# sp-uhh/guided-vae-nmf

Hardware: AMD Instinct MI355X
Metric: STFT-frames/sec through VAE-NMF reconstruct loop; SI-SDR parity vs ref (higher is better)
Workload: dtype bf16; 1 GPU; 64-utterance batch per GPU, M1 reconstruct, 512-pt STFT (F=257, 501 frames/utt), NMF rank 8, 100 EM iters, MH 60/30 per E-step + 105/75 Wiener chain; utterances_total=64, utterances_rank0=64, parallelism=utterance-shard x1 (np.array_split, no collective in the loop)

## Files before the change

### guided-vae-nmf_amd/csrc/chain.hip

```cpp
#include "common.h"

#ifdef VN_STAMP
__device__ long long g_wc_stamp[32];
#define WC_STAMP_DECL long long _t_prev = (long long)__builtin_amdgcn_s_memtime(); long long _st_acc[8] = {0, 0, 0, 0, 0, 0, 0, 0}; int _st_cnt[8] = {0, 0, 0, 0, 0, 0, 0, 0};
#define WC_STAMP(slot) do { long long _t = (long long)__builtin_amdgcn_s_memtime(); _st_acc[slot] += _t - _t_prev; _st_cnt[slot] += 1; _t_prev = _t; } while (0)
#define WC_STAMP_FLUSH do { if (blockIdx.x == 0 && threadIdx.x == 0) { for (int _i = 0; _i < 8; ++_i) { g_wc_stamp[_i] += _st_acc[_i]; g_wc_stamp[16 + _i] += _st_cnt[_i]; } } } while (0)
#else
#define WC_STAMP_DECL
#define WC_STAMP(slot)
#define WC_STAMP_FLUSH
#endif
namespace {

constexpr int WT_FRAMES = 16;
constexpr unsigned WC_OOB = 0xF0000000u;
constexpr int WC_PF = 1;
constexpr int WC_PFL = 2;
constexpr int WC_ST_AUX = 0;

struct WcArgs {
  const __bf16 *w1f, *w2f, *w3f;
  const float *b1, *b2, *b3;
  int NT3;
  int Tm;
  int F, Fs;
  const float *X2, *W, *Ht, *g, *B1, *Vb;
  float *Z, *Zs, *acc_out;
  void* VsS;
  unsigned VsS_bytes;
  int32_t* src;
  int Rs;
  const int32_t *wt_utt, *wt_n0, *wt_cnt;
  int n_wtiles;
  const int32_t* frame_off;
  const uint64_t* utt_seed;
  const float *eps, *u;
  int Kp, NT, n_utts, Rcap, nsamples, burnin, rng_mode, update_Z;
  int n_hi_lds;
  int b1_lds;
  uint32_t call;
  float sd;
  float sd_hi;
  int one_hidden;
};

template <bool SPLIT>
struct WcLds {
  static constexpr int PARTS = SPLIT ? 2 : 1;
  static constexpr int W1 = 0;
  static constexpr int W2 = W1 + NT_H * PARTS * 1024;
  static constexpr int B1 = W2 + NT_H * NK_H * PARTS * 1024;
  static constexpr int B2 = B1 + HID * 4;
  static constexpr int B3 = B2 + HID * 4;
  static constexpr int W3 = B3 + 640 * 4;
  static constexpr int fixed_bytes = W3;
};

typedef __attribute__((ext_vector_type(4))) unsigned u32x4;
typedef __attribute__((ext_vector_type(2))) unsigned u32x2;

typedef __attribute__((ext_vector_type(2))) __bf16 bf16x2;
__device__ __forceinline__ unsigned pk2(float a, float b) { return __builtin_bit_cast(unsigned, bf16x2{(__bf16)a, (__bf16)b}); }
// ... 62 lines not shown
  x2 = xv;
  vb = v;
}

struct WcFrame {
  int utt, nrow;
  bool fvalid;
  bool keeps;
};
__device__ __forceinline__ WcFrame wc_frame(const WcArgs& a, int wt, int c, bool writer) {
  WcFrame fr;
  const int n0 = a.wt_n0[wt], cnt = a.wt_cnt[wt];
  fr.utt = a.wt_utt[wt];
  fr.fvalid = c < cnt;
  fr.keeps = fr.fvalid && writer;
  fr.nrow = n0 + (fr.fvalid ? c : cnt - 1);
  return fr;
}
__device__ __forceinline__ void wc_load_z(const WcRes& R, const WcFrame& fr, int q, float (&z)[8]) {
  const unsigned zo = ((unsigned)fr.nrow * LAT + 4u * (unsigned)q) * 4u;
  const f32x4 lo = __builtin_bit_cast(f32x4, __builtin_amdgcn_raw_buffer_load_b128(R.z_rs, zo, 0, 0));
  const f32x4 hi = __builtin_bit_cast(f32x4, __builtin_amdgcn_raw_buffer_load_b128(R.z_rs, zo + 64u, 0, 0));
#pragma unroll
  for (int t = 0; t < 4; ++t) { z[t] = lo[t]; z[4 + t] = hi[t]; }
}
__device__ __forceinline__ void wc_store_z(const WcArgs& a, const WcRes& R, const WcFrame& fr, unsigned rp_off, const float (&z)[8]) {
  if (a.update_Z) {
    const unsigned zo = fr.keeps ? rp_off : WC_OOB;
    __builtin_amdgcn_raw_buffer_store_b128(__builtin_bit_cast(u32x4, f32x4{z[0], z[1], z[2], z[3]}), R.z_rs, zo, 0, 0);
    __builtin_amdgcn_raw_buffer_store_b128(__builtin_bit_cast(u32x4, f32x4{z[4], z[5], z[6], z[7]}), R.z_rs, zo + 64u, 0, 0);
  }
}

template <int MAXT, bool EXACT, bool SPLIT, bool STORE, int NWAVES, bool LOL, bool HIALL, bool M2, int GT>
__global__ __launch_bounds__(NWAVES * 64, NWAVES / 4) void wchain_kernel(const WcArgs a) {
  extern __shared__ __attribute__((aligned(16))) char smem[];
  using L = WcLds<SPLIT>;
  constexpr int PARTS = L::PARTS;
  using store_t = typename std::conditional<SPLIT, float, __bf16>::type;
  const int NT3 = EXACT ? MAXT : a.NT3;
  const int n_hi = HIALL ? NT3 - GT : a.n_hi_lds;

  {
    const int nthr = NWAVES * 64;
    auto stage = [&](char* dst, const __bf16* srcp, int nblk) {
      for (int e = threadIdx.x; e < nblk * PARTS * 64; e += nthr) {
        const int chunk = e & 63, pb = e >> 6, b = pb / PARTS, part = pb - b * PARTS;
        *reinterpret_cast<f32x4*>(dst + (size_t)e * 16) =
            *reinterpret_cast<const f32x4*>(reinterpret_cast<const char*>(srcp) + ((size_t)(b * 2 + part) * 64 + chunk) * 16);
      }
    };
    stage(smem + L::W1, a.w1f, NT_H);
    stage(smem + L::W2, a.w2f, NT_H * NK_H);
    for (int e = threadIdx.x; e < n_hi * NK_H * 64; e += nthr) {
      const int chunk = e & 63, b = (e >> 6) + GT * NK_H;
      *reinterpret_cast<f32x4*>(smem + L::W3 + (size_t)e * 16) =
          *reinterpret_cast<const f32x4*>(reinterpret_cast<const char*>(a.w3f) + ((size_t)(b * 2) * 64 + chunk) * 16);
    }
    if (SPLIT && LOL)
      for (int e = threadIdx.x; e < NT3 * NK_H * 64; e += nthr) {
        const int chunk = e & 63, b = e >> 6;
        *reinterpret_cast<f32x4*>(smem + L::W3 + (size_t)n_hi * NK_H * 1024 + (size_t)e * 16) =
            *reinterpret_cast<const f32x4*>(reinterpret_cast<const char*>(a.w3f) + ((size_t)(b * 2 + 1) * 64 + chunk) * 16);
      }
    float* b1s = reinterpret_cast<float*>(smem + L::B1);
    float* b2s = reinterpret_cast<float*>(smem + L::B2);
    float* b3s = reinterpret_cast<float*>(smem + L::B3);
    for (int i = threadIdx.x; i < HID; i += nthr) { b1s[i] = a.b1[i]; b2s[i] = a.b2[i]; }
    for (int i = threadIdx.x; i < 16 * NT3; i += nthr) b3s[i] = a.b3[i];
  }
  __syncthreads();

  const int lane = threadIdx.x & 63, q = lane >> 4, c = lane & 15;
  const unsigned l16 = (unsigned)lane * 16u;
  const float* b1l = reinterpret_cast<const float*>(smem + L::B1);
  const float* b2l = reinterpret_cast<const float*>(smem + L::B2);
  const float* b3l = reinterpret_cast<const float*>(smem + L::B3);
  const char* w3lo_lds = smem + L::W3 + (size_t)n_hi * NK_H * 1024;
  const char* w3g = reinterpret_cast<const char*>(a.w3f);
  const int Tm = EXACT ? ((MAXT - 1) & ~1) : a.Tm;
  auto tile_on = [&](int t) { return EXACT || t < NT3; };
  auto tile_on3 = [&](int n, int t) { return n != MAXT || EXACT || t < NT3; };

  const WcRes R = wc_resources<STORE, M2>(a);

  const int wave = __builtin_amdgcn_readfirstlane(threadIdx.x >> 6);
  for (int wt = wave * (int)gridDim.x + (int)blockIdx.x; wt < a.n_wtiles; wt += (int)gridDim.x * NWAVES) {
    const WcFrame fr = wc_frame(a, wt, c, true);
    const int nrow = fr.nrow;
    const float gn = a.g[nrow];
    f32x4 x2[MAXT], vb[MAXT];
    {
      const unsigned rowF = (unsigned)nrow * (unsigned)a.Fs;
      const unsigned uF = (unsigned)fr.utt * (unsigned)a.Fs;
      int qo = q;
      asm volatile("" : "+v"(qo));
      auto bin0o = [&](int t) { return (!SPLIT && t < Tm) ? 32 * (t >> 1) + 8 * qo + 4 * (t & 1) : 16 * t + 4 * qo; };
#pragma unroll
      for (int t = 0; t < MAXT; ++t) {
        x2[t] = f32x4{0, 0, 0, 0};
        vb[t] = f32x4{1, 1, 1, 1};
        if (tile_on(t)) {
          const int f0 = bin0o(t);
          wc_tile_consts(a, R, rowF, uF, nrow, f0, x2[t], vb[t]);
        }
      }
    }
    constexpr bool B1L = M2 && NWAVES == 8;
    f32x4 b1r[(M2 && !B1L) ? NT_H : 1];
    char* b1stash = smem + a.b1_lds + wave * (NT_H * 512) + lane * 8;
    if (M2) {
#pragma unroll
      for (int t = 0; t < NT_H; ++t) {
        const f32x4 v = __builtin_bit_cast(f32x4, __builtin_amdgcn_raw_buffer_load_b128(R.b1in_rs, ((unsigned)nrow * HID + 4u * (unsigned)q) * 4u + 64u * (unsigned)t, 0, 0));
        if (B1L) *reinterpret_cast<u32x2*>(b1stash + t * 512) = u32x2{pk2(v[0], v[1]), pk2(v[2], v[3])};
        else b1r[(M2 && !B1L) ? t : 0] = v;
      }
    }
    float z[8];
    wc_load_z(R, fr, q, z);
    const unsigned fbase = STORE ? (fr.fvalid ? (unsigned)nrow * (unsigned)(a.Rs * a.Fs) * (unsigned)sizeof(store_t) : WC_OOB) : 0u;
    const unsigned zs_off = fr.fvalid ? ((unsigned)nrow * (unsigned)a.Rcap * LAT + 4u * q) * 4u : WC_OOB;
    const unsigned fr_off = (fr.fvalid && q == 0) ? (unsigned)nrow * 4u : WC_OOB;
    const unsigned rp_off = ((unsigned)nrow * LAT + 4u * q) * 4u;
    int cur_src = a.nsamples;
    Xs128 st0, st1;
    if (a.rng_mode == VAENMF_RNG_DEVICE) {
      const uint32_t floc = (uint32_t)(nrow - a.frame_off[fr.utt]);
      int qs = q;
      asm volatile("" : "+v"(qs));
      st0 = xs_seed(a.utt_seed[fr.utt], floc, (uint32_t)qs, a.call);
      st1 = xs_seed(a.utt_seed[fr.utt], floc, (uint32_t)(4 + qs), a.call);
    }

    WC_STAMP_DECL
    auto energy = [&](const float (&zz)[8], int slot, auto dost) -> double {
      constexpr bool DOST = STORE && decltype(dost)::value;
      const unsigned voff = DOST ? fbase + (unsigned)slot * (unsigned)a.Fs * (unsigned)sizeof(store_t) : 0u;
      u32x4 bh[NK_H], bl[NK_H], ch[NK_H], cl[NK_H];
      auto put = [&](u32x4 (&dh)[NK_H], u32x4 (&dl)[NK_H], int t, const f32x4 h) {
        dh[t >> 1][2 * (t & 1)] = pk2(h[0], h[1]);
        dh[t >> 1][2 * (t & 1) + 1] = pk2(h[2], h[3]);
        if (SPLIT) {
          dl[t >> 1][2 * (t & 1)] = pk2(h[0] - bf_lo(dh[t >> 1][2 * (t & 1)]), h[1] - bf_hi(dh[t >> 1][2 * (t & 1)]));
          dl[t >> 1][2 * (t & 1) + 1] = pk2(h[2] - bf_lo(dh[t >> 1][2 * (t & 1) + 1]), h[3] - bf_hi(dh[t >> 1][2 * (t & 1) + 1]));
        }
      };
      auto run_layer = [&](auto nks_c, auto ntiles_c, auto pfl_c, auto frag, auto frag_lo, auto frag_lo_pro, auto bias, auto bop, auto epi) {
        constexpr int NKS = decltype(nks_c)::value, N = decltype(ntiles_c)::value;
        constexpr int PF = WC_PF, NB = PF + 1;
        constexpr int PFL = SPLIT ? decltype(pfl_c)::value : 0, NBL = PFL + 1;
        bf16x8 wh[NB][NKS], wl[NBL][NKS];
        f32x4 acc[2], bq[NB];
#pragma unroll
        for (int p = 0; p < PFL; ++p)
          if (p < N) {
#pragma unroll
            for (int s = 0; s < NKS; ++s) frag_lo_pro(p, s, wl[p % NBL][s]);
          }
#pragma unroll
        for (int p = 0; p < PF; ++p)
          if (p < N) {
#pragma unroll
            for (int s = 0; s < NKS; ++s) frag(p, s, wh[p % NB][s]);
            bq[p % NB] = bias(p);
          }
#pragma unroll
        for (int t = 0; t <= N; ++t) {
          if (SPLIT && t + PFL < N && tile_on3(N, t + PFL)) {
#pragma unroll
            for (int s = 0; s < NKS; ++s) frag_lo(t + PFL, s, wl[(t + PFL) % NBL][s]);
// ... 78 lines not shown
      WC_STAMP(2);
      double e = 0.0;
      f32x2 pl2 = {0.f, 0.f}, px2 = {0.f, 0.f};
      unsigned pk_even0 = 0, pk_even1 = 0;
      run_layer(std::integral_constant<int, NK_H>{}, std::integral_constant<int, MAXT>{}, std::integral_constant<int, (SPLIT && !LOL) ? WC_PFL : WC_PF>{},
                [&](int t, int s, bf16x8& hi) {
                  if (GT > 0 && t < GT) hi = gfr[t < GT ? t : 0][s];
                  else if (HIALL || t - GT < n_hi) hi = *reinterpret_cast<const bf16x8*>(smem + L::W3 + ((t - GT) * NK_H + s) * 1024 + l16);
                  else hi = *reinterpret_cast<const bf16x8*>(w3g + (size_t)((t * NK_H + s) * 2) * 1024 + l16);
                },
                [&](int t, int s, bf16x8& lo) {
                  if (LOL) lo = *reinterpret_cast<const bf16x8*>(w3lo_lds + (t * NK_H + s) * 1024 + l16);
                  else lo = *reinterpret_cast<const bf16x8*>(w3g + (size_t)((t * NK_H + s) * 2 + 1) * 1024 + l16);
                },
                [&](int t, int s, bf16x8& lo) {
                  if (LOL) lo = *reinterpret_cast<const bf16x8*>(w3lo_lds + (t * NK_H + s) * 1024 + l16);
                  else if (t < NHOIST) lo = lo_pre[t < NHOIST ? t : 0][s];
                  else lo = *reinterpret_cast<const bf16x8*>(w3g + (size_t)((t * NK_H + s) * 2 + 1) * 1024 + l16);
                },
                [&](int t) { return *reinterpret_cast<const f32x4*>(b3l + 16 * t + 4 * q); },
                [&](int s, bf16x8& hi, bf16x8& lo) { hi = __builtin_bit_cast(bf16x8, bh[s]); lo = SPLIT ? __builtin_bit_cast(bf16x8, bl[s]) : hi; },
                [&](int t, const f32x4 acc) {
                  f32x4 ev;
#pragma unroll
                  for (int j = 0; j < 4; ++j) ev[j] = fast_exp(acc[j]);
                  {
                    const f32x2 g2 = {gn, gn};
                    const f32x2 v0 = g2 * ev.lo + vb[t].lo, v1 = g2 * ev.hi + vb[t].hi;
                    const f32x2 pp = v0 * v1;
                    pl2 += f32x2{fast_log2(pp[0]), fast_log2(pp[1])};
                    const f32x2 rc = {fast_rcp(pp[0]), fast_rcp(pp[1])};
                    px2 = (x2[t].lo * v1 + x2[t].hi * v0) * rc + px2;
                  }
                  if (DOST) {
                    if (SPLIT) {
                      __builtin_amdgcn_raw_buffer_store_b128(__builtin_bit_cast(u32x4, ev), R.vrs, voff + 16u * q + 64u * t, 0, WC_ST_AUX);
                    } else {
                      const unsigned p0 = pk2(ev[0], ev[1]), p1 = pk2(ev[2], ev[3]);
                      if (t < Tm) {
                        if ((t & 1) == 0) { pk_even0 = p0; pk_even1 = p1; }
                        else __builtin_amdgcn_raw_buffer_store_b128(u32x4{pk_even0, pk_even1, p0, p1}, R.vrs, voff + 16u * q + 64u * (t >> 1), 0, WC_ST_AUX);
                      } else {
                        __builtin_amdgcn_raw_buffer_store_b64(u32x2{p0, p1}, R.vrs, voff + 8u * q + 32u * t, 0, WC_ST_AUX);
                      }
                    }
                  }
                  if ((t & 1) == 1) {
                    e += (double)((pl2[0] + pl2[1]) * LN2_F + (px2[0] + px2[1]));
                    pl2 = px2 = f32x2{0.f, 0.f};
                  }
                });
      e += (double)((pl2[0] + pl2[1]) * LN2_F + (px2[0] + px2[1]));
      WC_STAMP(3);
      return sum_rows4_d(e);
    };

    double Ecur = 0.0;
    __builtin_amdgcn_s_waitcnt(0x0F70);
    const int n_it = vn_chain_passes<STORE>(a.nsamples, a.burnin);
    for (int it = -1; it < n_it; ++it) {
      asm volatile("" ::: "memory");
      const VnChainPass ps = vn_chain_pass<STORE>(it, a.nsamples, a.burnin);
      const bool re = ps.re, step = ps.step;
      const int m = ps.m, slot = ps.slot;
      float zp[8];
      float lu = 0.f;
      if (step) {
// ... 22 lines not shown
      }
      WC_STAMP(0);
      double Ep;
      if (STORE && slot >= 0) Ep = energy(zp, slot, std::true_type{});
      else Ep = energy(zp, slot, std::false_type{});
      WC_STAMP(5);
      if (re) continue;
      float pr = 0.f;
#pragma unroll
      for (int j = 0; j < 8; ++j) pr += z[j] * z[j] - zp[j] * zp[j];
      pr = sum_rows4(pr);
      lu = sum_rows4(lu);
      WC_STAMP(6);
      const float accp = (float)(Ecur - Ep) + 0.5f * pr;
      const bool ok = m < 0 || lu < accp;
      if (a.acc_out && m >= 0) __builtin_amdgcn_raw_buffer_store_b32(__builtin_bit_cast(unsigned, accp), R.acc_rs, fr_off + (unsigned)m * (unsigned)a.NT * 4u, 0, 0);
#pragma unroll
      for (int j = 0; j < 8; ++j) z[j] = ok ? zp[j] : z[j];
      Ecur = ok ? Ep : Ecur;
      WC_STAMP(7);
      if (m >= a.burnin) {
        const unsigned r = (unsigned)(m - a.burnin);
        if (STORE) {
          cur_src = ok ? (int)r : cur_src;
          __builtin_amdgcn_raw_buffer_store_b32((unsigned)cur_src, R.src_rs, fr_off + r * (unsigned)a.NT * 4u, 0, 0);
        }
        const unsigned zo = zs_off + r * (LAT * 4u);
        __builtin_amdgcn_raw_buffer_store_b128(__builtin_bit_cast(u32x4, f32x4{z[0], z[1], z[2], z[3]}), R.zs_rs, zo, 0, 0);
        __builtin_amdgcn_raw_buffer_store_b128(__builtin_bit_cast(u32x4, f32x4{z[4], z[5], z[6], z[7]}), R.zs_rs, zo + 64u, 0, 0);
      }
      WC_STAMP(4);
    }
    WC_STAMP_FLUSH;
    wc_store_z(a, R, fr, rp_off, z);
  }
}


template <int MAXT, bool STORE, bool M2>
__global__ __launch_bounds__(256, 1) void wchain4_kernel(const WcArgs a) {
  extern __shared__ __attribute__((aligned(16))) char smem[];
  constexpr int NP = (MAXT - 1) / 2;
  constexpr int PPW = NP / 4, NOWN = 2 * PPW + 1;
  constexpr bool B1BF = MAXT == 17;
  static_assert(NP % 4 == 0, "pairs must split over four wavefronts");
  u32x4* xh1 = reinterpret_cast<u32x4*>(smem);
  u32x4* xh2 = xh1 + 4 * 64;
  float* exl = reinterpret_cast<float*>(xh2 + 4 * 64);

  const int lane = threadIdx.x & 63, q = lane >> 4, c = lane & 15;
  const unsigned l16 = (unsigned)lane * 16u;
  const int wave = __builtin_amdgcn_readfirstlane(threadIdx.x >> 6);
  auto tile_of = [&](int i) { return i < 2 * PPW ? 2 * (wave + 4 * (i >> 1)) + (i & 1) : MAXT - 1; };
  auto own = [&](int i) { return i < 2 * PPW || wave == 0; };

  bf16x8 w1r[2], w2r[2][NK_H], w3r[NOWN][NK_H];
  f32x4 bias1[2], bias2[2], bias3[NOWN];
  {
    const char* w1g = reinterpret_cast<const char*>(a.w1f);
    const char* w2g = reinterpret_cast<const char*>(a.w2f);
    const char* w3g = reinterpret_cast<const char*>(a.w3f);
#pragma unroll
    for (int i = 0; i < 2; ++i) {
      const int t = 2 * wave + i;
      w1r[i] = *reinterpret_cast<const bf16x8*>(w1g + (size_t)(t * 2) * 1024 + l16);
#pragma unroll
      for (int s = 0; s < NK_H; ++s) w2r[i][s] = *reinterpret_cast<const bf16x8*>(w2g + (size_t)((t * NK_H + s) * 2) * 1024 + l16);
      bias1[i] = *reinterpret_cast<const f32x4*>(a.b1 + 16 * t + 4 * q);
      bias2[i] = *reinterpret_cast<const f32x4*>(a.b2 + 16 * t + 4 * q);
    }
#pragma unroll
    for (int i = 0; i < NOWN; ++i) {
      const int t = tile_of(i);
#pragma unroll
      for (int s = 0; s < NK_H; ++s) w3r[i][s] = *reinterpret_cast<const bf16x8*>(w3g + (size_t)((t * NK_H + s) * 2) * 1024 + l16);
      bias3[i] = *reinterpret_cast<const f32x4*>(a.b3 + 16 * t + 4 * q);
    }
  }

  const WcRes R = wc_resources<STORE, M2>(a);

  for (int wt = blockIdx.x; wt < a.n_wtiles; wt += (int)gridDim.x) {
    const WcFrame fr = wc_frame(a, wt, c, wave == 0);
    const int nrow = fr.nrow;
    const float gn = a.g[nrow];
    f32x4 x2[NOWN], vb[NOWN];
    {
      const unsigned rowF = (unsigned)nrow * (unsigned)a.Fs, uF = (unsigned)fr.utt * (unsigned)a.Fs;
#pragma unroll
      for (int i = 0; i < NOWN; ++i) {
        x2[i] = f32x4{0, 0, 0, 0};
        vb[i] = f32x4{1, 1, 1, 1};
        if (own(i)) {
          const int t = tile_of(i);
          const int f0 = t < MAXT - 1 ? 32 * (t >> 1) + 8 * q + 4 * (t & 1) : 16 * t + 4 * q;
          wc_tile_consts(a, R, rowF, uF, nrow, f0, x2[i], vb[i]);
        }
      }
    }
    f32x4 b1r[2];
    b1r[0] = bias1[0]; b1r[1] = bias1[1];
    if (M2) {
#pragma unroll
      for (int i = 0; i < 2; ++i) {
        const f32x4 v = __builtin_bit_cast(f32x4, __builtin_amdgcn_raw_buffer_load_b128(R.b1in_rs, ((unsigned)nrow * HID + 4u * (unsigned)q) * 4u + 64u * (unsigned)(2 * wave + i), 0, 0));
        if (B1BF) {
          const unsigned w0 = pk2(v[0], v[1]), w1 = pk2(v[2], v[3]);
          b1r[i] = f32x4{bf_lo(w0), bf_hi(w0), bf_lo(w1), bf_hi(w1)};
        } else b1r[i] = v;
      }
    }
    float z[8];
    wc_load_z(R, fr, q, z);
    const unsigned fbase = STORE ? (fr.fvalid ? (unsigned)nrow * (unsigned)(a.Rs * a.Fs) * 2u : WC_OOB) : 0u;
    const unsigned zs_off = fr.keeps ? ((unsigned)nrow * (unsigned)a.Rcap * LAT + 4u * q) * 4u : WC_OOB;
    const unsigned fr_off = (fr.keeps && q == 0) ? (unsigned)nrow * 4u : WC_OOB;
    const unsigned rp_off = ((unsigned)nrow * LAT + 4u * q) * 4u;
    int cur_src = a.nsamples;
    Xs128 st0, st1;
    if (a.rng_mode == VAENMF_RNG_DEVICE) {
      const uint32_t floc = (uint32_t)(nrow - a.frame_off[fr.utt]);
      st0 = xs_seed(a.utt_seed[fr.utt], floc, (uint32_t)q, a.call);
      st1 = xs_seed(a.utt_seed[fr.utt], floc, (uint32_t)(4 + q), a.call);
    }

    auto energy = [&](const float (&zz)[8], int slot, auto dost) -> double {
      constexpr bool DOST = STORE && decltype(dost)::value;
      const unsigned voff = DOST ? fbase + (unsigned)slot * (unsigned)a.Fs * 2u : 0u;
      u32x4 bh[NK_H], ch[NK_H];
      u32x4 mine;
      auto put2 = [&](int i, const f32x4 h) { mine[2 * i] = pk2(h[0], h[1]); mine[2 * i + 1] = pk2(h[2], h[3]); };
      auto exchange = [&](u32x4* xh, u32x4 (&dst)[NK_H]) {
        xh[wave * 64 + lane] = mine;
        __syncthreads();
#pragma unroll
        for (int s2 = 0; s2 < NK_H; ++s2) dst[s2] = xh[s2 * 64 + lane];
      };
      {
        const bf16x8 zin = __builtin_bit_cast(bf16x8, u32x4{pk2(zz[0], zz[1]), pk2(zz[2], zz[3]), pk2(zz[4], zz[5]), pk2(zz[6], zz[7])});
        f32x4 ac[2];
#pragma unroll
        for (int i = 0; i < 2; ++i) ac[i] = __builtin_amdgcn_mfma_f32_16x16x32_bf16(w1r[i], zin, b1r[i], 0, 0, 0);
#pragma unroll
        for (int i = 0; i < 2; ++i) put2(i, tanh4(ac[i]));
      }
      exchange(xh1, ch);
      if (a.one_hidden) {
#pragma unroll
        for (int s = 0; s < NK_H; ++s) bh[s] = ch[s];
      } else {
        f32x4 ac[2];
#pragma unroll
        for (int i = 0; i < 2; ++i) {
          ac[i] = bias2[i];
#pragma unroll
          for (int s = 0; s < NK_H; ++s) ac[i] = __builtin_amdgcn_mfma_f32_16x16x32_bf16(w2r[i][s], __builtin_bit_cast(bf16x8, ch[s]), ac[i], 0, 0, 0);
        }
#pragma unroll
        for (int i = 0; i < 2; ++i) put2(i, tanh4(ac[i]));
        exchange(xh2, bh);
      }
      f32x2 pl2 = {0.f, 0.f}, px2 = {0.f, 0.f};
      float pv[PPW + 1];
#pragma unroll
      for (int j = 0; j <= PPW; ++j) pv[j] = 0.f;
      unsigned pk_even0 = 0, pk_even1 = 0;
      auto mm3 = [&](int i) {
        f32x4 ac = bias3[i];
#pragma unroll
        for (int s = 0; s < NK_H; ++s) ac = __builtin_amdgcn_mfma_f32_16x16x32_bf16(w3r[i][s], __builtin_bit_cast(bf16x8, bh[s]), ac, 0, 0, 0);
        return ac;
      };
      auto epi = [&](int i, const f32x4 acc) {
        f32x4 ev;
#pragma unroll
        for (int j = 0; j < 4; ++j) ev[j] = fast_exp(acc[j]);
        {
          const f32x2 g2 = {gn, gn};
          const f32x2 v0 = g2 * ev.lo + vb[i].lo, v1 = g2 * ev.hi + vb[i].hi;
          const f32x2 pp = v0 * v1;
          pl2 += f32x2{fast_log2(pp[0]), fast_log2(pp[1])};
          const f32x2 rc = {fast_rcp(pp[0]), fast_rcp(pp[1])};
          px2 = (x2[i].lo * v1 + x2[i].hi * v0) * rc + px2;
        }
        if (DOST) {
          const unsigned p0 = pk2(ev[0], ev[1]), p1 = pk2(ev[2], ev[3]);
          const unsigned t = (unsigned)tile_of(i);
          if (i < 2 * PPW) {
            if ((i & 1) == 0) { pk_even0 = p0; pk_even1 = p1; }
            else __builtin_amdgcn_raw_buffer_store_b128(u32x4{pk_even0, pk_even1, p0, p1}, R.vrs, voff + 16u * q + 64u * (t >> 1), 0, WC_ST_AUX);
          } else {
            __builtin_amdgcn_raw_buffer_store_b64(u32x2{p0, p1}, R.vrs, voff + 8u * q + 32u * t, 0, WC_ST_AUX);
          }
        }
        if ((i & 1) == 1 || i == 2 * PPW) {
          pv[i >> 1] = (pl2[0] + pl2[1]) * LN2_F + (px2[0] + px2[1]);
          pl2 = px2 = f32x2{0.f, 0.f};
        }
      };
      {
        f32x4 acn = mm3(0);
#pragma unroll
        for (int i = 0; i < NOWN; ++i) {
          const f32x4 acc = acn;
          if (i + 1 < NOWN && own(i + 1)) acn = mm3(i + 1);
          if (own(i)) epi(i, acc);
        }
      }
      float* ex = exl + lane;
#pragma unroll
      for (int j = 0; j < PPW; ++j) ex[(wave + 4 * j) * 64] = pv[j];
      if (wave == 0) ex[NP * 64] = pv[PPW];
      __syncthreads();
      double e = 0.0;
#pragma unroll
      for (int p = 0; p <= NP; ++p) e += (double)ex[p * 64];
      return sum_rows4_d(e);
    };

    double Ecur = 0.0;
    __builtin_amdgcn_s_waitcnt(0x0F70);
    const int n_it = vn_chain_passes<STORE>(a.nsamples, a.burnin);
    for (int it = -1; it < n_it; ++it) {
// ... 22 lines not shown
          for (int t = 0; t < 8; ++t) asm volatile("" : "+v"(zp[t]));
          asm volatile("" : "+v"(lu));
        }
      } else {
#pragma unroll
        for (int t = 0; t < 8; ++t) zp[t] = z[t];
      }
      double Ep;
      if (STORE && slot >= 0) Ep = energy(zp, slot, std::true_type{});
      else Ep = energy(zp, slot, std::false_type{});
      if (re) continue;
      float pr = 0.f;
#pragma unroll
      for (int j = 0; j < 8; ++j) pr += z[j] * z[j] - zp[j] * zp[j];
      pr = sum_rows4(pr);
      lu = sum_rows4(lu);
      const float accp = (float)(Ecur - Ep) + 0.5f * pr;
      const bool ok = m < 0 || lu < accp;
      if (a.acc_out && m >= 0) __builtin_amdgcn_raw_buffer_store_b32(__builtin_bit_cast(unsigned, accp), R.acc_rs, fr_off + (unsigned)m * (unsigned)a.NT * 4u, 0, 0);
#pragma unroll
      for (int j = 0; j < 8; ++j) z[j] = ok ? zp[j] : z[j];
      Ecur = ok ? Ep : Ecur;
      if (m >= a.burnin) {
        const unsigned r = (unsigned)(m - a.burnin);
        if (STORE) {
          cur_src = ok ? (int)r : cur_src;
          __builtin_amdgcn_raw_buffer_store_b32((unsigned)cur_src, R.src_rs, fr_off + r * (unsigned)a.NT * 4u, 0, 0);
        }
        const unsigned zo = zs_off + r * (LAT * 4u);
        __builtin_amdgcn_raw_buffer_store_b128(__builtin_bit_cast(u32x4, f32x4{z[0], z[1], z[2], z[3]}), R.zs_rs, zo, 0, 0);
        __builtin_amdgcn_raw_buffer_store_b128(__builtin_bit_cast(u32x4, f32x4{z[4], z[5], z[6], z[7]}), R.zs_rs, zo + 64u, 0, 0);
      }
    }
    wc_store_z(a, R, fr, rp_off, z);
  }
}

}

namespace {

template <typename Go>
int wc_by_m2_store(const WcArgs& a, Go&& go) {
  if (a.B1) return a.VsS ? go(std::true_type{}, std::true_type{}) : go(std::true_type{}, std::false_type{});
  return a.VsS ? go(std::false_type{}, std::true_type{}) : go(std::false_type{}, std::false_type{});
}
template <int MAXT, bool EXACT, bool SPLIT, int NW1, bool LOL, int GT = 0>
int wc_launch_s(const WcArgs& a, int nwt, int n_sms, size_t lds, hipStream_t st) {
  int grid = nwt;
  if (grid > n_sms) grid = n_sms;
  const int cap = vn_switches().grid_cap;
  if (cap > 0 && cap < grid) grid = cap;
  return wc_by_m2_store(a, [&](auto m2, auto store) -> int {
    auto* fn = wchain_kernel<MAXT, EXACT, SPLIT, decltype(store)::value, NW1, LOL, true, decltype(m2)::value, GT>;
    if (int e = vn_ensure_dyn_lds((const void*)fn, VN_LDS_LIMIT)) return e;
    hipLaunchKernelGGL(fn, dim3(grid), dim3(NW1 * 64), lds, st, a);
    return 0;
  });
}
template <int MAXT>
int wc_launch4(const WcArgs& a, hipStream_t st) {
  const size_t lds4 = 2 * 4 * 64 * 16 + 20 * 64 * 4;
  return wc_by_m2_store(a, [&](auto m2, auto store) -> int {
    hipLaunchKernelGGL((wchain4_kernel<MAXT, decltype(store)::value, decltype(m2)::value>), dim3(a.n_wtiles), dim3(256), lds4, st, a);
    return 0;
  });
}

}

bool vn_wchain_supported(const vaenmf_plan* p) {
  if (p->NT3c > 17 && !(p->NT3c == 33 && p->cfg.precision == VAENMF_PREC_BF16)) return false;
  return !vn_switches().team_chain;
}

extern "C" int vaenmf_wchain_addressable(int64_t NT, int32_t Rcap, int32_t steps, int32_t Fs, int32_t Kp, int32_t n_utt, int32_t replay) {
  const uint64_t lim = 0xE0000000ull;
  const uint64_t nt = (uint64_t)(NT > 0 ? NT : 0), S = (uint64_t)(steps > 0 ? steps : 0);
  if (nt * (uint64_t)Rcap * LAT * 4 >= lim) return 0;
  if (nt * (uint64_t)Fs * 4 >= lim) return 0;
  if (nt * (uint64_t)HID * 4 >= lim) return 0;
  if ((uint64_t)n_utt * (uint64_t)Fs * (uint64_t)Kp * 4 >= lim) return 0;
  if (nt * (uint64_t)Kp * 4 >= lim) return 0;
  if (nt * S * 4 >= lim) return 0;
  if (replay && nt * S * LAT * 4 >= lim) return 0;
  return 1;
}
bool vn_wchain_fits(const vaenmf_plan* p, const VnChainCall& cc) {
  return vaenmf_wchain_addressable(p->NT, cc.Rcap, cc.nsamples + cc.burnin, p->Fs, p->Kp, p->n_utt, cc.eps != nullptr) != 0;
}

int vn_launch_wchain(vaenmf_plan* p, const VnChainCall& cc, hipStream_t st) {
  VN_REQUIRE(vn_wchain_fits(p, cc), "wave chain: a buffer of this batch (%d frames) passes the kernel's 32-bit byte offsets", p->NT);
  const bool split = p->cfg.precision == VAENMF_PREC_BF16X3;
  WcArgs a = {};
  a.w1f = p->w1f; a.w2f = p->w2f; a.w3f = p->w3c; a.b1 = p->b1; a.b2 = p->b2; a.b3 = p->b3c;
  a.NT3 = p->NT3c; a.Tm = split ? 0 : ((p->NT3c - 1) & ~1); a.F = p->cfg.F; a.Fs = p->Fs;
  a.X2 = cc.X2; a.W = cc.W; a.Ht = cc.Ht; a.g = cc.g; a.B1 = cc.B1; a.Vb = p->Vb_ext;
  a.Z = cc.Z; a.Zs = cc.Zs; a.acc_out = cc.acc_out;
  a.VsS = cc.VsS; a.VsS_bytes = (unsigned)cc.VsS_bytes; a.src = cc.src; a.Rs = cc.Rs;
  a.wt_utt = p->d_wt_utt; a.wt_n0 = p->d_wt_n0; a.wt_cnt = p->d_wt_cnt; a.n_wtiles = p->n_wtiles;
  a.frame_off = p->d_frame_off; a.utt_seed = p->d_utt_seed; a.eps = cc.eps; a.u = cc.u;
  a.Kp = p->Kp; a.NT = p->NT; a.n_utts = p->n_utt; a.Rcap = cc.Rcap; a.nsamples = cc.nsamples; a.burnin = cc.burnin;
  a.rng_mode = cc.rng_mode; a.update_Z = cc.update_Z; a.call = cc.call; a.sd = cc.sd; a.sd_hi = cc.sd_hi; a.one_hidden = cc.one_hidden;
  a.n_hi_lds = p->NT3c;
  const size_t fixed = split ? WcLds<true>::fixed_bytes : WcLds<false>::fixed_bytes;
  constexpr int GT33 = 4;
  const size_t w3hi = (size_t)(p->NT3c == 33 ? p->NT3c - GT33 : p->NT3c) * NK_H * 1024;
  const bool lol = split && p->NT3c <= 5;
  constexpr int NW_BF16 = 8, NW_X3 = 4;
  const int nwaves = (split || p->NT3c == 33) ? 4 : NW_BF16;
  a.b1_lds = (int)(fixed + w3hi * (lol ? 2 : 1));
  const size_t lds = (size_t)a.b1_lds + ((cc.B1 && nwaves == 8) ? (size_t)nwaves * NT_H * 512 : 0);
  VN_REQUIRE(lds <= (size_t)VN_LDS_LIMIT, "wave chain: %zu bytes of LDS needed", lds);
  if (!split && (p->NT3c == 17 || p->NT3c == 33) && p->n_wtiles <= p->n_sms && vn_switches().wchain4) {
    const int rc4 = p->NT3c == 17 ? wc_launch4<17>(a, st) : wc_launch4<33>(a, st);
    if (rc4) return rc4;
    VN_CHECK_HIP(hipGetLastError());
    p->last_chain_kernel = 2;
    return 0;
  }
  int rc;
  if (p->NT3c == 33)     rc = wc_launch_s<33, true, false, 4, false, GT33>(a, p->n_wtiles, p->n_sms, lds, st);
  else if (p->NT3c == 17) rc = split ? wc_launch_s<17, true, true, NW_X3, false>(a, p->n_wtiles, p->n_sms, lds, st) : wc_launch_s<17, true, false, NW_BF16, false>(a, p->n_wtiles, p->n_sms, lds, st);
  else if (p->NT3c == 5) rc = split ? wc_launch_s<5, true, true, NW_X3, true>(a, p->n_wtiles, p->n_sms, lds, st)   : wc_launch_s<5, true, false, NW_BF16, false>(a, p->n_wtiles, p->n_sms, lds, st);
  else if (p->NT3c < 5)  rc = split ? wc_launch_s<5, false, true, NW_X3, true>(a, p->n_wtiles, p->n_sms, lds, st)  : wc_launch_s<5, false, false, NW_BF16, false>(a, p->n_wtiles, p->n_sms, lds, st);
  else                   rc = split ? wc_launch_s<17, false, true, NW_X3, false>(a, p->n_wtiles, p->n_sms, lds, st) : wc_launch_s<17, false, false, NW_BF16, false>(a, p->n_wtiles, p->n_sms, lds, st);
  if (rc) return rc;
  VN_CHECK_HIP(hipGetLastError());
  p->last_chain_kernel = 1;
  return 0;
}

#ifdef VN_STAMP
extern "C" int vaenmf_debug_stamps_wc(long long* out32, int reset) {
  long long h[32];
  if (hipMemcpyFromSymbol(h, HIP_SYMBOL(g_wc_stamp), sizeof(h)) != hipSuccess) return -2;
  for (int i = 0; i < 32; ++i) out32[i] = h[i];
  if (reset) { long long z[32] = {0}; (void)hipMemcpyToSymbol(HIP_SYMBOL(g_wc_stamp), z, sizeof(z)); }
  return 0;
}
#endif
```

### guided-vae-nmf_amd/csrc/common.h

```cpp
#pragma once
#include <hip/hip_runtime.h>
#include <stdint.h>
#include <string>
#include <type_traits>
#include <vector>
#include "../../include/vaenmf.h"

typedef __attribute__((ext_vector_type(8))) __bf16 bf16x8;
typedef __attribute__((ext_vector_type(4))) __bf16 bf16x4;
typedef __attribute__((ext_vector_type(4))) float f32x4;

void vaenmf_set_error(const char* fmt, ...);
#define VN_CHECK_HIP(expr)                                                         \
  do {                                                                             \
    hipError_t _e = (expr);                                                        \
    if (_e != hipSuccess) {                                                        \
      vaenmf_set_error("%s failed: %s (%s:%d)", #expr, hipGetErrorString(_e), __FILE__, __LINE__); \
      return -2;                                                                   \
    }                                                                              \
  } while (0)
#define VN_REQUIRE(cond, ...)                \
  do {                                       \
    if (!(cond)) {                           \
      vaenmf_set_error(__VA_ARGS__);         \
      return -1;                             \
    }                                        \
  } while (0)

constexpr int VN_COST_CHUNK = 25;
constexpr int MAX_TILE_FRAMES = 64;
constexpr int LAT = 32;
constexpr int HID = 128;
constexpr int NK_H = HID / 32;
constexpr int NT_H = HID / 16;
constexpr int VN_LDS_LIMIT = 160 * 1024;

struct VnEmGraphs {
  using Key = std::vector<uint64_t>;
  struct Graph {
    Key key; hipGraphExec_t exec; uint64_t used;
    int chain_kernel, w_fused;
  };
  hipStream_t cap_stream = nullptr;
  std::vector<Graph> cache;
  std::vector<Key> seen;
  uint64_t tick = 0;
  bool off = false;
  int last = 0;
  Graph* find(const Key& key);
  bool first_seen(const Key& key);
  Graph* insert(const Key& key, hipGraphExec_t exec, int chain_kernel, int w_fused);
  void release();
};

struct vaenmf_plan {
  vaenmf_config cfg;
  int Fs, Kp, NT3;
  int Fm;
  float* w3n;
  int geom;
  int nwaves;
  int tile_frames;
  __bf16 *w1f, *w2f, *w3f;
  float *b1, *b2, *b3;
  float* w1y;
  int Dy;
  int Lz;
  bool wide = false;
  int Lp = LAT;
  bool one_hidden;
  bool have_weights;
  const float* Vb_ext;
  int n_utt, NT, n_tiles;
  int32_t *d_frame_off;
  int32_t *d_tile_utt, *d_tile_n0, *d_tile_cnt;
  int32_t *d_frame_utt;
  int32_t *d_frame_loc;
  __bf16* w3c;
  float* b3c;
  int NT3c;
  int32_t *d_wt_utt, *d_wt_n0, *d_wt_cnt;
  int n_wtiles;
  int32_t *d_t64_n0 = nullptr, *d_t64_cnt = nullptr, *d_t64_first = nullptr, *d_t64_g0 = nullptr;
  int n_t64 = 0;
  float* wpart64 = nullptr;
  size_t wpart16_groups = 0;
  float* wpart16 = nullptr;
  int last_chain_kernel = 0;
  int last_w_fused = 0;
  int Rcap_store;
  int last_m_step_path;
  uint64_t* d_utt_seed;
  std::vector<int32_t> h_frame_off;
  float *A1, *P;
  float* normW;
  float* wpart;
  double* cost_frames;
  bool store_on;
  void* VsS;
  int32_t* src;
  size_t VsS_cap, src_cap;
  int store_R, store_Rs;
  int n_sms;
  bool prof_on;
  std::vector<hipEvent_t> prof_ev;
  std::vector<int> prof_kind;
  size_t prof_used;
  VnEmGraphs graphs;
  static constexpr int SEED_RING = 8;
  uint64_t* h_seed_ring = nullptr;
  hipEvent_t seed_ev[SEED_RING] = {};
  bool seed_ev_used[SEED_RING] = {};
  int seed_pos = 0;
};

struct VnChainCall {
  const float *X2, *W, *Ht, *g, *B1;
  float *Z, *Zs, *acc_out;
  const float *eps, *u;
  void* VsS; size_t VsS_bytes; int32_t* src; int Rs;
  int Rcap, nsamples, burnin, rng_mode, update_Z;
  uint32_t call;
  float sd;
  float sd_hi;
  int one_hidden;
};

struct VnSwitches {
  bool wchain4;
  bool team_chain;
  bool wfused;
  bool wgroup;
  int wfused_grid;
  int grid_cap;
  bool keep_zs;
};

VnSwitches vn_switches();
int vn_ensure_dyn_lds(const void* fn, int bytes);
extern long long g_vn_dev_allocs;
bool vn_wchain_supported(const vaenmf_plan* p);
bool vn_wchain_fits(const vaenmf_plan* p, const VnChainCall& cc);
int vn_launch_wchain(vaenmf_plan* p, const VnChainCall& cc, hipStream_t st);
int vn_launch_tchain(vaenmf_plan* p, const VnChainCall& cc, hipStream_t st);
int vn_launch_widechain(vaenmf_plan* p, const VnChainCall& cc, hipStream_t st);
int vn_launch_wide_rng_fill(vaenmf_plan* p, uint32_t call, int S, float* eps_out, float* u_out, hipStream_t st);
int vn_launch_w_update(const vaenmf_plan* p, float* W, const float* Ht, hipStream_t st);
int vn_launch_w_update_tiles(const vaenmf_plan* p, float* W, hipStream_t st, bool groups);
int vn_launch_cost_reduce(const vaenmf_plan* p, const double* cost_frames, size_t stride, int n_it, int R, double* cost, int niter,
                          int it0, hipStream_t st);

inline int check_bound(const vaenmf_plan* p) {
  VN_REQUIRE(p != nullptr, "null plan");
  VN_REQUIRE(p->have_weights, "decoder weights not set (vaenmf_set_decoder_weights)");
  VN_REQUIRE(p->NT > 0, "no batch bound (vaenmf_bind_batch)");
  return 0;
}

enum { VN_K_CHAIN = 0, VN_K_WSTATS = 1, VN_K_WUPDATE = 2, VN_K_HG = 3, VN_K_WF = 4, VN_K_NKINDS = 5 };
struct ProfScope {
  vaenmf_plan* p; hipStream_t st; size_t idx; bool on;
  ProfScope(vaenmf_plan* p_, int kind, hipStream_t st_) : p(p_), st(st_), idx(0), on(false) {
    if (p && p->prof_on && p->prof_used + 2 <= p->prof_ev.size()) {
      on = true; idx = p->prof_used; p->prof_used += 2; p->prof_kind[idx / 2] = kind;
      (void)hipEventRecord(p->prof_ev[idx], st);
    }
  }
  ~ProfScope() { if (on) (void)hipEventRecord(p->prof_ev[idx + 1], st); }
};

#if defined(__HIPCC__)
__device__ __forceinline__ float fast_tanh(float xs) {
  float e = __builtin_amdgcn_exp2f(xs);
  return 1.0f - 2.0f * __builtin_amdgcn_rcpf(e + 1.0f);
}
// ... 137 lines not shown
```

### guided-vae-nmf_amd/csrc/driver.hip

```cpp
#include "common.h"
#include <cstring>

extern "C" int vaenmf_mh_chain(vaenmf_plan* p, const float* X2, const float* W, const float* Ht, const float* g,
                               float* Z, int32_t update_Z, const float* B1, float* Zs, int32_t Rcap, int32_t nsamples,
                               int32_t burnin, float var_rw, const vaenmf_rng* rng, float* acc_out, void* stream) {
  if (int e = check_bound(p)) return e;
  VN_REQUIRE(rng != nullptr, "rng is null");
  VN_REQUIRE(nsamples >= 1 && burnin >= 0 && nsamples <= Rcap, "bad sample counts (nsamples=%d burnin=%d Rcap=%d)", nsamples, burnin, Rcap);
  VN_REQUIRE(rng->mode == VAENMF_RNG_DEVICE || (rng->eps && rng->u), "replay mode needs eps and u buffers");
  hipStream_t st = (hipStream_t)stream;
  const bool split = p->cfg.precision == VAENMF_PREC_BF16X3;
  VnChainCall cc = {};
  cc.X2 = X2; cc.W = W; cc.Ht = Ht; cc.g = g; cc.B1 = B1; cc.Z = Z; cc.Zs = Zs; cc.acc_out = acc_out;
  cc.eps = rng->eps; cc.u = rng->u;
  cc.Rcap = Rcap; cc.nsamples = nsamples; cc.burnin = burnin; cc.rng_mode = rng->mode; cc.update_Z = update_Z;
  cc.call = rng->call; cc.sd = sqrtf(var_rw); cc.sd_hi = p->Lz > 16 ? cc.sd : 0.f; cc.one_hidden = p->one_hidden ? 1 : 0;
  p->store_R = p->store_Rs = 0;
  if (p->store_on) {
    const int Rs = nsamples + 1;
    const size_t esz = split ? sizeof(float) : sizeof(__bf16);
    const size_t need_v = (size_t)(p->NT + 1) * Rs * p->Fs * esz, need_s = (size_t)p->NT * Rs;
    VN_REQUIRE(need_v < 0xE0000000ull, "sample store: %d frames x %d slots x %d bins exceeds the 32-bit byte offsets of "
               "the chain kernel; bind a smaller batch or switch the store off", p->NT, Rs, p->Fs);
    VN_REQUIRE(need_v <= p->VsS_cap && need_s <= p->src_cap, "sample store too small for %d frames x %d samples: call "
               "vaenmf_sample_store(plan, max_samples) after vaenmf_bind_batch (no allocation happens in vaenmf_mh_chain)", p->NT, nsamples);
    cc.VsS = p->VsS; cc.VsS_bytes = need_v; cc.src = p->src; cc.Rs = Rs;
  }
  const bool use_wchain = !p->wide && vn_wchain_supported(p) && vn_wchain_fits(p, cc);
  VN_REQUIRE(p->wide || use_wchain || Zs != nullptr, "vaenmf_mh_chain: Zs may be NULL only where the wave-private chain kernels run (vaenmf_wchain_addressable)");
  {
    ProfScope ps(p, VN_K_CHAIN, st);
    if (int e = p->wide ? vn_launch_widechain(p, cc, st) : use_wchain ? vn_launch_wchain(p, cc, st) : vn_launch_tchain(p, cc, st)) return e;
  }
  if (p->store_on) { p->store_R = nsamples; p->store_Rs = nsamples + 1; }
  return 0;
}

extern "C" int vaenmf_sample_store(vaenmf_plan* p, int32_t max_samples) {
  VN_REQUIRE(p != nullptr, "null plan");
  VN_REQUIRE(max_samples >= 0, "max_samples = %d", max_samples);
  p->store_R = p->store_Rs = 0;
  p->store_on = max_samples > 0;
  if (!p->store_on) return 0;
  const size_t esz = p->cfg.precision == VAENMF_PREC_BF16X3 ? sizeof(float) : sizeof(__bf16);
  const size_t frames = (size_t)(p->NT > 0 ? p->NT : p->cfg.max_frames) + 1, Rs = (size_t)max_samples + 1;
  size_t need_v = frames * Rs * p->Fs * esz, need_s = frames * Rs;
  if (need_v >= 0xE0000000ull) need_v = 0xE0000000ull - 16;
  if (need_v > p->VsS_cap) {
    if (p->VsS) VN_CHECK_HIP(hipFree(p->VsS));
    p->VsS = nullptr; p->VsS_cap = 0;
    VN_CHECK_HIP(hipMalloc(&p->VsS, need_v));
    ++g_vn_dev_allocs;
    p->VsS_cap = need_v;
  }
  if (need_s > p->src_cap) {
    if (p->src) VN_CHECK_HIP(hipFree(p->src));
    p->src = nullptr; p->src_cap = 0;
    VN_CHECK_HIP(hipMalloc(&p->src, need_s * sizeof(int32_t)));
    ++g_vn_dev_allocs;
    p->src_cap = need_s;
  }
  p->Rcap_store = max_samples;
  return 0;
}

namespace {
template <typename ST>
__global__ void store_gather_kernel(const ST* __restrict__ VsS, const int32_t* __restrict__ src, int NT, int R, int Rs, int Fs,
                                    float* __restrict__ out) {
  const int n = blockIdx.x / R, r = blockIdx.x - n * R;
  const ST* row = VsS + ((size_t)n * Rs + src[(size_t)r * NT + n]) * Fs;
  for (int f = threadIdx.x; f < Fs; f += blockDim.x) out[((size_t)n * R + r) * Fs + f] = (float)row[f];
}
}

extern "C" int vaenmf_sample_store_gather(vaenmf_plan* p, float* Vs_out, void* stream) {
  VN_REQUIRE(p != nullptr && p->store_R > 0, "the sample store is empty (vaenmf_sample_store(plan, 1), then vaenmf_mh_chain)");
  VN_REQUIRE(Vs_out != nullptr, "null output");
  if (p->cfg.precision == VAENMF_PREC_BF16X3)
    hipLaunchKernelGGL(store_gather_kernel<float>, dim3((unsigned)(p->NT * p->store_R)), dim3(64), 0, (hipStream_t)stream,
                       reinterpret_cast<const float*>(p->VsS), p->src, p->NT, p->store_R, p->store_Rs, p->Fs, Vs_out);
  else
    hipLaunchKernelGGL(store_gather_kernel<__bf16>, dim3((unsigned)(p->NT * p->store_R)), dim3(64), 0, (hipStream_t)stream,
                       reinterpret_cast<const __bf16*>(p->VsS), p->src, p->NT, p->store_R, p->store_Rs, p->Fs, Vs_out);
  VN_CHECK_HIP(hipGetLastError());
  return 0;
}

extern "C" int vaenmf_set_noise_psd(vaenmf_plan* p, const float* Vb) {
  VN_REQUIRE(p != nullptr, "null plan");
  p->Vb_ext = Vb;
  return 0;
}

namespace {
constexpr size_t MAX_GRAPHS = 4, MAX_SEEN = 8;

struct EmCall {
  const float* X2; float *W, *Ht, *g, *Z; const float* B1; float* Zs;
  int32_t Rcap, niter, nsE, biE, nsWF, biWF; float var_rw;
  const float* X; float *S_hat, *N_hat; double* cost;
};

VnEmGraphs::Key em_graph_key(const vaenmf_plan* p, const EmCall& c, bool stored, const VnSwitches& sw) {
  auto u64 = [](const void* q) { return (uint64_t)(uintptr_t)q; };
  uint32_t vbits;
  memcpy(&vbits, &c.var_rw, 4);
  uint64_t fo_hash = 1469598103934665603ull;
  for (int32_t v : p->h_frame_off) { fo_hash ^= (uint64_t)(uint32_t)v; fo_hash *= 1099511628211ull; }
  return {fo_hash,
      u64(c.X2), u64(c.W), u64(c.Ht), u64(c.g), u64(c.Z), u64(c.B1), u64(c.Zs), u64(c.X), u64(c.S_hat), u64(c.N_hat), u64(c.cost),
      (uint64_t)c.Rcap, (uint64_t)c.niter, (uint64_t)c.nsE, (uint64_t)c.biE, (uint64_t)c.nsWF, (uint64_t)c.biWF, (uint64_t)vbits, (uint64_t)stored,
      (uint64_t)p->NT, (uint64_t)p->n_utt, (uint64_t)p->n_wtiles, (uint64_t)p->n_tiles, u64(p->VsS), u64(p->src), u64(p->Vb_ext),
      (uint64_t)p->VsS_cap, (uint64_t)p->Rcap_store, u64(p->w1f), u64(p->w2f), u64(p->w3f), u64(p->w3c), u64(p->b3c), u64(p->b1),
      u64(p->d_wt_utt), u64(p->d_wt_n0), u64(p->d_wt_cnt), u64(p->d_frame_off), u64(p->d_frame_utt), u64(p->d_frame_loc), u64(p->d_tile_utt),
      u64(p->d_tile_n0), u64(p->d_tile_cnt), u64(p->d_utt_seed), u64(p->A1), u64(p->P), u64(p->normW), u64(p->wpart), u64(p->cost_frames), u64(p->w3n), u64(p->w1y), u64(p->b2), u64(p->b3),
      u64(p->wpart64), u64(p->wpart16), u64(p->d_t64_n0), u64(p->d_t64_cnt), u64(p->d_t64_first), u64(p->d_t64_g0), (uint64_t)p->n_t64,
      (uint64_t)p->cfg.precision, (uint64_t)p->cfg.K, (uint64_t)p->cfg.F,
      (uint64_t)sw.wchain4, (uint64_t)sw.team_chain, (uint64_t)sw.wfused, (uint64_t)sw.wgroup, (uint64_t)(uint32_t)sw.wfused_grid,
      (uint64_t)(uint32_t)sw.grid_cap,
      (uint64_t)sw.keep_zs};
}
}

VnEmGraphs::Graph* VnEmGraphs::find(const Key& key) {
  for (auto& gph : cache)
    if (gph.key == key) return &gph;
  return nullptr;
}

bool VnEmGraphs::first_seen(const Key& key) {
  for (auto& k : seen) if (k == key) return false;
  if (seen.size() >= MAX_SEEN) seen.erase(seen.begin());
  seen.push_back(key);
  return true;
}

VnEmGraphs::Graph* VnEmGraphs::insert(const Key& key, hipGraphExec_t exec, int chain_kernel, int w_fused) {
  if (cache.size() >= MAX_GRAPHS) {
    size_t lru = 0;
    for (size_t i = 1; i < cache.size(); ++i) if (cache[i].used < cache[lru].used) lru = i;
    (void)hipGraphExecDestroy(cache[lru].exec);
    cache.erase(cache.begin() + lru);
  }
  cache.push_back({key, exec, 0, chain_kernel, w_fused});
  return &cache.back();
}

void VnEmGraphs::release() {
  for (auto& gph : cache) if (gph.exec) (void)hipGraphExecDestroy(gph.exec);
  cache.clear();
  if (cap_stream) (void)hipStreamDestroy(cap_stream);
  cap_stream = nullptr;
}

static int em_run_body(vaenmf_plan* p, const EmCall& c, bool stored, void* stream) {
  hipStream_t st = (hipStream_t)stream;
  vaenmf_rng rng = {VAENMF_RNG_DEVICE, 0, nullptr, nullptr};
  const size_t cstride = (size_t)p->cfg.max_frames;
  float* Zs_e = (stored && !vn_switches().keep_zs &&
                 (p->wide || (vn_wchain_supported(p) &&
                              vaenmf_wchain_addressable(p->NT, c.Rcap, c.nsE + c.biE, p->Fs, p->Kp, p->n_utt, 0)))) ? nullptr : c.Zs;
  for (int it = 0; it < c.niter; ++it) {
    rng.call = (uint32_t)it;
    double* cf = p->cost_frames + (size_t)(it % VN_COST_CHUNK) * cstride;
    if (int e = vaenmf_mh_chain(p, c.X2, c.W, c.Ht, c.g, c.Z, 1, c.B1, Zs_e, c.Rcap, c.nsE, c.biE, c.var_rw, &rng, nullptr, stream)) return e;
    if (int e = stored ? vaenmf_m_step_stored(p, c.X2, c.W, c.Ht, c.g, cf, stream)
                       : vaenmf_m_step(p, c.X2, c.W, c.Ht, c.g, c.Zs, c.Rcap, c.nsE, c.B1, cf, stream)) return e;
    if (c.cost && ((it + 1) % VN_COST_CHUNK == 0 || it + 1 == c.niter)) {
      const int it0 = it - it % VN_COST_CHUNK;
      if (int e2 = vn_launch_cost_reduce(p, p->cost_frames, cstride, it - it0 + 1, c.nsE, c.cost, c.niter, it0, st)) return e2;
    }
  }
  rng.call = (uint32_t)c.niter;
  if (int e = vaenmf_mh_chain(p, c.X2, c.W, c.Ht, c.g, c.Z, 0, c.B1, c.Zs, c.Rcap, c.nsWF, c.biWF, c.var_rw, &rng, nullptr, stream)) return e;
  if (stored) return vaenmf_wiener_stored(p, c.W, c.Ht, c.g, c.X, c.S_hat, c.N_hat, nullptr, nullptr, stream);
  return vaenmf_wiener(p, c.X2, c.W, c.Ht, c.g, c.Zs, c.Rcap, c.nsWF, c.B1, c.X, c.S_hat, c.N_hat, nullptr, nullptr, stream);
}

static int em_graph_launch(vaenmf_plan* p, VnEmGraphs::Graph& gph, const EmCall& c, bool stored, hipStream_t st) {
  VN_CHECK_HIP(hipGraphLaunch(gph.exec, st));
  gph.used = ++p->graphs.tick;
  if (stored) { p->store_R = c.nsWF; p->store_Rs = c.nsWF + 1; }
  p->last_chain_kernel = gph.chain_kernel;
  p->last_w_fused = gph.w_fused;
  p->graphs.last = 1;
  return 0;
}

static hipGraphExec_t em_graph_capture(vaenmf_plan* p, const EmCall& c, bool stored) {
  VnEmGraphs& G = p->graphs;
  auto fail = [&]() { (void)hipGetLastError(); G.off = true; return (hipGraphExec_t) nullptr; };
  if (!G.cap_stream && hipStreamCreateWithFlags(&G.cap_stream, hipStreamNonBlocking) != hipSuccess) return fail();
  if (hipStreamBeginCapture(G.cap_stream, hipStreamCaptureModeThreadLocal) != hipSuccess) return fail();
  hipGraph_t graph = nullptr;
  const int rc = em_run_body(p, c, stored, (void*)G.cap_stream);
  const hipError_t ec = hipStreamEndCapture(G.cap_stream, &graph);
  hipGraphExec_t exec = nullptr;
  const bool ok = rc == 0 && ec == hipSuccess && graph && hipGraphInstantiate(&exec, graph, nullptr, nullptr, 0) == hipSuccess && exec;
  if (graph) (void)hipGraphDestroy(graph);
  return ok ? exec : fail();
}

extern "C" int vaenmf_em_run(vaenmf_plan* p, const float* X2, float* W, float* Ht, float* g, float* Z, const float* B1,
                             float* Zs, int32_t Rcap, int32_t niter, int32_t nsE, int32_t biE, int32_t nsWF, int32_t biWF,
                             float var_rw, const float* X, float* S_hat, float* N_hat, double* cost, void* stream) {
  if (int e = check_bound(p)) return e;
  VN_REQUIRE(nsE <= Rcap && nsWF <= Rcap, "Rcap=%d too small for nsE=%d / nsWF=%d", Rcap, nsE, nsWF);
  const EmCall c = {X2, W, Ht, g, Z, B1, Zs, Rcap, niter, nsE, biE, nsWF, biWF, var_rw, X, S_hat, N_hat, cost};
  const size_t esz = p->cfg.precision == VAENMF_PREC_BF16X3 ? sizeof(float) : sizeof(__bf16);
  auto fits = [&](int ns) { return (size_t)(p->NT + 1) * (ns + 1) * p->Fs * esz < 0xE0000000ull; };
  const bool want = p->store_on, stored = want && fits(nsE) && fits(nsWF);
  VN_REQUIRE(!p->wide || want, "vaenmf_em_run on a wide decoder plan streams the sample store: switch it on with vaenmf_sample_store first");
  VN_REQUIRE(!p->wide || stored, "vaenmf_em_run on a wide decoder plan: the sample store of %d frames passes the 32-bit offsets of the "
             "streaming kernels and there is no decoding path for wide decoders; bind a smaller batch", p->NT);
  p->store_on = stored;
  p->last_m_step_path = stored ? 1 : 2;
  struct Restore { vaenmf_plan* p; bool v; ~Restore() { p->store_on = v; } } restore{p, want};
  auto eager = [&]() { return em_run_body(p, c, stored, stream); };

  static const bool graphs_on = []() { const char* e = getenv("VAENMF_GRAPH"); return !(e && e[0] == '0'); }();
  VnEmGraphs& G = p->graphs;
  G.last = 0;
  if (!graphs_on || G.off || p->prof_on) return eager();
  const VnEmGraphs::Key key = em_graph_key(p, c, stored, vn_switches());
  if (VnEmGraphs::Graph* gph = G.find(key)) return em_graph_launch(p, *gph, c, stored, (hipStream_t)stream);
  if (G.first_seen(key)) return eager();
  const hipGraphExec_t exec = em_graph_capture(p, c, stored);
  if (!exec) return eager();
  return em_graph_launch(p, *G.insert(key, exec, p->last_chain_kernel, p->last_w_fused), c, stored, (hipStream_t)stream);
}
```

### guided-vae-nmf_amd/csrc/engine.hip

```cpp
#include "common.h"

namespace {

constexpr int TEAM_COLS = 32;

struct DecW {
  const __bf16 *w1f, *w2f, *w3f;
  const float *b1, *b2, *b3;
  const float* w3n;
  int NT3;
  int F;
  int Fm;
  int Lz;
  int one_hidden;
};

template <int NTEAM, bool SPLIT>
struct LdsMap {
  static constexpr int PARTS = SPLIT ? 2 : 1;
  static constexpr bool ALIAS = SPLIT;
  static constexpr int ACT = 2 * NK_H * PARTS * 1024;
  static constexpr int ACT_TEAM = ALIAS ? ACT : 2 * ACT;
  static constexpr int W1B = NT_H * 1 * PARTS * 1024;
  static constexpr int W2B = NT_H * NK_H * PARTS * 1024;
// ... 251 lines not shown
  d.nyq = dw.Fm != dw.F;
  d.nyqbuf = reinterpret_cast<float*>(smem + M::nyq) + d.team * 8 * 2 * 16;
#pragma unroll
  for (int ti = 0; ti < NT_H / NW; ++ti)
    d.wn[ti] = d.nyq ? *reinterpret_cast<const f32x4*>(dw.w3n + 16 * (d.w + NW * ti) + 4 * ((threadIdx.x & 63) >> 4)) : f32x4{0, 0, 0, 0};
  stage_weights<M::PARTS>(smem + M::w1, dw.w1f, NT_H);
  stage_weights<M::PARTS>(smem + M::w2, dw.w2f, NT_H * NK_H);
  if (W3LDS) stage_weights<M::PARTS>(smem + w3_lds_off, dw.w3f, dw.NT3 * NK_H);
  float* b2 = reinterpret_cast<float*>(smem + M::b2);
  float* b3 = reinterpret_cast<float*>(smem + M::b3);
  for (int i = threadIdx.x; i < HID; i += blockDim.x) b2[i] = dw.b2[i];
  for (int i = threadIdx.x; i < Fs; i += blockDim.x) b3[i] = dw.b3[i];
  return d;
}

__device__ __forceinline__ double shfl_xor_d(double v, int m) { return __shfl_xor(v, m, 64); }

#ifdef VN_STAMP
__device__ long long* g_stamp_buf = nullptr;
__device__ long long g_stamp_store[64];
#define VN_STAMP_DECL long long _t_prev = (long long)__builtin_amdgcn_s_memtime(); const bool _st_on = blockIdx.x == 0 && threadIdx.x == 0;
#define VN_STAMP_AT(slot) do { long long _t = (long long)__builtin_amdgcn_s_memtime(); if (_st_on) { g_stamp_store[slot] += _t - _t_prev; g_stamp_store[32 + slot] += 1; } _t_prev = _t; } while (0)
#else
#define VN_STAMP_DECL
#define VN_STAMP_AT(slot)
#endif

struct ChainArgs {
  DecW dw;
  const float *X2, *W, *Ht, *g, *B1;
  const float* Vb;
  float *Z, *Zs, *acc_out;
  void* VsS;
  int32_t* src;
  int Rs;
  const int32_t *tile_utt, *tile_n0, *tile_cnt, *frame_off;
  const uint64_t* utt_seed;
  const float *eps, *u;
  int Fs, Kp, NT, Rcap, nsamples, burnin, rng_mode, update_Z;
  int w3_lds_off;
  uint32_t call;
  float sd;
};

struct ChainX {
  float eps[TEAM_COLS][LAT];
  float u[TEAM_COLS];
  double epart[2][8][TEAM_COLS];
};

template <int NW, int NTEAM, int MT, bool SPLIT, bool W3LDS, bool STORE>
__global__ __launch_bounds__(NW * NTEAM * 64) void mh_chain_kernel(const ChainArgs a) {
  constexpr int MAXT = MT;
  extern __shared__ __attribute__((aligned(16))) char smem[];
  using M = LdsMap<NTEAM, SPLIT>;
  constexpr int TPW = NT_H / NW;
  const DecW& dw = a.dw;
  const Dec<NW, NTEAM, MT, SPLIT, W3LDS> d = dec_setup<NW, NTEAM, MT, SPLIT, W3LDS>(smem, dw, a.w3_lds_off, a.Fs);
  ChainX& L = reinterpret_cast<ChainX*>(smem + M::common_end)[d.team];
  const int lane = threadIdx.x & 63, w = d.w, q = lane >> 4, c = lane & 15;
  const int tile = blockIdx.x;
  const int utt = a.tile_utt[tile];
  const int cnt_all = a.tile_cnt[tile];
  int cnt = cnt_all - TEAM_COLS * d.team;
  cnt = cnt < 0 ? 0 : (cnt > TEAM_COLS ? TEAM_COLS : cnt);
  const bool team_on = cnt > 0;
// ... 44 lines not shown
#pragma unroll
    for (int fg = 0; fg < 2; ++fg) {
      x2n[fg] = a.X2[(size_t)nrow[fg] * a.Fs + dw.F - 1];
      float v = 0.f;
      if (a.Vb) v = a.Vb[(size_t)nrow[fg] * a.Fs + dw.F - 1];
      else
        for (int k = 0; k < a.Kp; ++k) v += a.W[((size_t)utt * a.Fs + dw.F - 1) * a.Kp + k] * a.Ht[(size_t)nrow[fg] * a.Kp + k];
      vbn[fg] = v;
    }
  }
  f32x4 bias1[TPW][2];
#pragma unroll
  for (int ti = 0; ti < TPW; ++ti) {
    const int f0 = 16 * (w + NW * ti) + 4 * q;
#pragma unroll
    for (int fg = 0; fg < 2; ++fg)
      bias1[ti][fg] = a.B1 ? *reinterpret_cast<const f32x4*>(a.B1 + (size_t)nrow[fg] * HID + f0)
                           : *reinterpret_cast<const f32x4*>(dw.b1 + f0);
  }
  float z[2][8];
#pragma unroll
  for (int fg = 0; fg < 2; ++fg) {
    const f32x4 lo = *reinterpret_cast<const f32x4*>(a.Z + (size_t)nrow[fg] * LAT + 4 * q);
    const f32x4 hi = *reinterpret_cast<const f32x4*>(a.Z + (size_t)nrow[fg] * LAT + 16 + 4 * q);
#pragma unroll
    for (int t = 0; t < 4; ++t) { z[fg][t] = lo[t]; z[fg][4 + t] = hi[t]; }
  }
  using store_t = typename std::conditional<SPLIT, float, __bf16>::type;
  uint32_t voff[2] = {0u, 0u};
  int cur_src[2] = {a.nsamples, a.nsamples};
  if (STORE) {
#pragma unroll
    for (int fg = 0; fg < 2; ++fg)
      voff[fg] = ((uint32_t)(fvalid[fg] ? nrow[fg] : a.NT) * (uint32_t)(a.Rs * a.Fs) + 4u * q) * (uint32_t)sizeof(store_t);
  }
  const int sid = threadIdx.x - d.team * NW * 64, sfr = sid >> 3, squad = sid & 7;
  const bool srng = sid < TEAM_COLS * 8;
  const bool sval = srng && team_on && sfr < cnt;
  Xs128 st;
  if (sval && a.rng_mode == VAENMF_RNG_DEVICE)
    st = xs_seed(a.utt_seed[utt], (uint32_t)(n0 - a.frame_off[utt] + sfr), (uint32_t)squad, a.call);
  auto draw = [&](int step) {
    if (!srng) return;
    f32x4 e = {0, 0, 0, 0};
    float uu = 0.5f;
    if (sval) {
      if (a.rng_mode == VAENMF_RNG_DEVICE) {
        e = normal4(st);
        if (squad == 0) uu = uniform01(st);
      } else {
        const size_t row = (size_t)step * a.NT + n0 + sfr;
        e = *reinterpret_cast<const f32x4*>(a.eps + row * LAT + 4 * squad);
        if (squad == 0) uu = a.u[row];
        __builtin_amdgcn_s_waitcnt(0x0F70);
      }
    }
    if (4 * squad >= a.dw.Lz) e = f32x4{0, 0, 0, 0};
    *reinterpret_cast<f32x4*>(&L.eps[sfr][4 * squad]) = e;
    if (squad == 0) L.u[sfr] = uu;
  };

  int ecount = 0;
  const float* b3l = reinterpret_cast<const float*>(smem + M::b3);
  const int S = a.nsamples + a.burnin;
  auto energy = [&](const float (&zz)[2][8], double (&E)[2], int next_step, int slot, auto dost) {
    constexpr bool DOST = STORE && decltype(dost)::value;
    char* const vbase = reinterpret_cast<char*>(a.VsS) + (DOST ? (size_t)slot * a.Fs * sizeof(store_t) : 0);
    bf16x8 zhi[2], zlo[2];
    split8<SPLIT>(zz[0], zhi[0], zlo[0]);
    split8<SPLIT>(zz[1], zhi[1], zlo[1]);
    d.hidden(zhi, zlo, bias1, [&]() { if (next_step < S) draw(next_step); });
    double e[2] = {0.0, 0.0};
    d.template out_layer_tiles<false>(
        [&](int i) { return *reinterpret_cast<const f32x4*>(b3l + 16 * (w + NW * i) + 4 * q); },
        [&](int i, const f32x4 acc0, const f32x4 acc1) {
#pragma unroll
          for (int fg = 0; fg < 2; ++fg) {
            const f32x4 acc = fg == 0 ? acc0 : acc1;
            float pl = 0.f, px = 0.f;
            f32x4 ev;
#pragma unroll
            for (int t = 0; t < 4; ++t) ev[t] = fast_exp(acc[t]);
#pragma unroll
            for (int t = 0; t < 4; t += 2) {
              const float v0 = gn[fg] * ev[t] + vb[i][fg][t];
              const float v1 = gn[fg] * ev[t + 1] + vb[i][fg][t + 1];
              const float pp = v0 * v1;
              pl += fast_log2(pp);
              px += (x2[i][fg][t] * v1 + x2[i][fg][t + 1] * v0) * fast_rcp(pp);
            }
            if (DOST) {
              const char* tb = vbase + 16 * (w + NW * i) * sizeof(store_t);
              if (SPLIT) {
                asm volatile("global_store_dwordx4 %0, %1, %2\n\ts_nop 1" :: "v"(voff[fg]), "v"(ev), "s"(tb) : "memory");
              } else {
                const bf16x4 pk = bf16x4{(__bf16)ev[0], (__bf16)ev[1], (__bf16)ev[2], (__bf16)ev[3]};
                asm volatile("global_store_dwordx2 %0, %1, %2" :: "v"(voff[fg]), "v"(pk), "s"(tb) : "memory");
              }
            }
            e[fg] += (double)(pl * LN2_F + px);
          }
        });
    if (d.nyq) {
      const float bn = b3l[dw.F - 1];
#pragma unroll
      for (int fg = 0; fg < 2; ++fg) {
        const float vs = fast_exp(d.nyq_logit(fg, bn));
        const float vx = gn[fg] * vs + vbn[fg];
        const float term = fast_log(vx) + x2n[fg] * fast_rcp(vx);
        e[fg] += (w == 0 && q == 0) ? (double)term : 0.0;
        if (DOST && w == 2 && q == 0) {
          store_t* dst = reinterpret_cast<store_t*>(vbase + (size_t)dw.Fm * sizeof(store_t) + voff[fg]);
          if (SPLIT) {
            *reinterpret_cast<f32x4*>(dst) = f32x4{vs, 0.f, 0.f, 0.f};
#pragma unroll
            for (int j = 1; j < 4; ++j) *reinterpret_cast<f32x4*>(dst + 4 * j) = f32x4{0.f, 0.f, 0.f, 0.f};
          } else {
            bf16x8 t8;
#pragma unroll
            for (int j = 0; j < 8; ++j) t8[j] = (__bf16)0.f;
            bf16x8 h8 = t8;
            h8[0] = (__bf16)vs;
            *reinterpret_cast<bf16x8*>(dst) = h8;
            *reinterpret_cast<bf16x8*>(dst + 8) = t8;
          }
        }
      }
    }
    const int par = ecount & 1;
    ++ecount;
#pragma unroll
    for (int fg = 0; fg < 2; ++fg) {
      e[fg] = sum_rows4_d(e[fg]);
      if (q == 0) L.epart[par][w][16 * fg + c] = e[fg];
    }
    d.team_sync();
#pragma unroll
    for (int fg = 0; fg < 2; ++fg) {
      double s = 0.0;
#pragma unroll
      for (int ww = 0; ww < NW; ++ww) s += L.epart[par][ww][16 * fg + c];
      E[fg] = s;
    }
// ... 704 lines not shown
    default: return launch_decode_one<NW, NTEAM, MT, SPLIT, MODE, 32>(a, grid, lds, st);
  }
}
template <int MODE>
int launch_decode(const vaenmf_plan* p, const DecodeArgs& a, hipStream_t st) {
  const int want = p->n_sms * 2;
  int grid = a.n_tiles < want ? a.n_tiles : want;
  const int cap = vn_switches().grid_cap;
  if (cap > 0 && cap < grid) grid = cap;
  const bool split = p->cfg.precision == VAENMF_PREC_BF16X3;
  const int Kp = (MODE == MODE_STORE) ? 8 : p->Kp;
  switch (p->geom) {
    case 0: return split ? launch_decode_kp<4, 2, 5, true, MODE>(a, Kp, grid, st) : launch_decode_kp<4, 2, 5, false, MODE>(a, Kp, grid, st);
    case 3: return split ? launch_decode_kp<4, 2, 4, true, MODE>(a, Kp, grid, st) : launch_decode_kp<4, 2, 4, false, MODE>(a, Kp, grid, st);
    case 4: return split ? launch_decode_kp<8, 1, 4, true, MODE>(a, Kp, grid, st) : launch_decode_kp<8, 1, 4, false, MODE>(a, Kp, grid, st);
    default: return split ? launch_decode_kp<8, 1, 5, true, MODE>(a, Kp, grid, st) : launch_decode_kp<8, 1, 5, false, MODE>(a, Kp, grid, st);
  }
}

DecodeArgs base_decode_args(const vaenmf_plan* p, const float* Zs, int Rcap, int R, const float* B1) {
  DecodeArgs a = {};
  a.dw = make_decw(p);
  a.Zs = Zs; a.B1 = B1; a.tile_utt = p->d_tile_utt; a.tile_n0 = p->d_tile_n0; a.tile_cnt = p->d_tile_cnt; a.n_tiles = p->n_tiles;
  a.Fs = p->Fs; a.K = p->cfg.K; a.NT = p->NT; a.Rcap = Rcap; a.R = R; a.Vb = p->Vb_ext;
  return a;
}

}

int vn_launch_tchain(vaenmf_plan* p, const VnChainCall& cc, hipStream_t st) {
  ChainArgs a = {};
  a.dw = make_decw(p);
  a.X2 = cc.X2; a.W = cc.W; a.Ht = cc.Ht; a.g = cc.g; a.B1 = cc.B1; a.Z = cc.Z; a.Zs = cc.Zs; a.acc_out = cc.acc_out; a.Vb = p->Vb_ext;
  a.VsS = cc.VsS; a.src = cc.src; a.Rs = cc.Rs;
  a.tile_utt = p->d_tile_utt; a.tile_n0 = p->d_tile_n0; a.tile_cnt = p->d_tile_cnt; a.frame_off = p->d_frame_off;
  a.utt_seed = p->d_utt_seed; a.eps = cc.eps; a.u = cc.u;
  a.Fs = p->Fs; a.Kp = p->Kp; a.NT = p->NT; a.Rcap = cc.Rcap; a.nsamples = cc.nsamples; a.burnin = cc.burnin;
  a.rng_mode = cc.rng_mode; a.call = cc.call; a.sd = cc.sd; a.update_Z = cc.update_Z;
  const bool split = p->cfg.precision == VAENMF_PREC_BF16X3;
  int lrc = 0;
  switch (p->geom) {
    case 0: lrc = split ? launch_chain<4, 2, 5, true>(a, p->n_tiles, st) : launch_chain<4, 2, 5, false>(a, p->n_tiles, st); break;
    case 3: lrc = split ? launch_chain<4, 2, 4, true>(a, p->n_tiles, st) : launch_chain<4, 2, 4, false>(a, p->n_tiles, st); break;
    case 4: lrc = split ? launch_chain<8, 1, 4, true>(a, p->n_tiles, st) : launch_chain<8, 1, 4, false>(a, p->n_tiles, st); break;
    default: lrc = split ? launch_chain<8, 1, 5, true>(a, p->n_tiles, st) : launch_chain<8, 1, 5, false>(a, p->n_tiles, st); break;
  }
  if (lrc) return lrc;
  VN_CHECK_HIP(hipGetLastError());
  p->last_chain_kernel = 0;
  return 0;
}

extern "C" int vaenmf_rng_fill(vaenmf_plan* p, uint32_t call, int32_t S, float* eps_out, float* u_out, void* stream) {
  if (int e = check_bound(p)) return e;
  if (p->wide) return vn_launch_wide_rng_fill(p, call, S, eps_out, u_out, (hipStream_t)stream);
  hipLaunchKernelGGL(rng_fill_kernel, dim3(p->n_tiles), dim3(8 * p->tile_frames), 0, (hipStream_t)stream, p->d_tile_utt, p->d_tile_n0,
                     p->d_tile_cnt, p->d_frame_off, p->d_utt_seed, call, S, p->NT, eps_out, u_out);
  VN_CHECK_HIP(hipGetLastError());
  return 0;
}

extern "C" int vaenmf_decode(vaenmf_plan* p, const float* Zs, int32_t Rcap, int32_t R, const float* B1, float* Vs_out, void* stream) {
  if (int e = check_bound(p)) return e;
  VN_REQUIRE(!p->wide, "%s: a wide decoder plan (z_dim > 32 or a hidden layer of 256 units) has no decoding kernels; run the chain with the sample "
             "store on (vaenmf_sample_store) and use vaenmf_m_step_stored / vaenmf_wiener_stored (vaenmf_sample_store_gather for the variances)", "vaenmf_decode");
  VN_REQUIRE(R >= 1 && R <= Rcap, "bad R=%d (Rcap=%d)", R, Rcap);
  DecodeArgs a = base_decode_args(p, Zs, Rcap, R, B1);
// ... 54 lines not shown
```

### guided-vae-nmf_amd/csrc/plan.hip

```cpp
#include <stdarg.h>
#include <stdio.h>
#include <string.h>
#include <math.h>
#include <stdlib.h>
#include <mutex>
#include <set>
#include <utility>
#include "common.h"
#include <algorithm>

static thread_local char g_err[512] = "";

int vn_ensure_dyn_lds(const void* fn, int bytes) {
  static std::mutex mu;
  static std::set<std::pair<int, const void*>> done;
  int dev = 0;
  VN_CHECK_HIP(hipGetDevice(&dev));
  std::lock_guard<std::mutex> lock(mu);
  if (done.count({dev, fn})) return 0;
  VN_CHECK_HIP(hipFuncSetAttribute(fn, hipFuncAttributeMaxDynamicSharedMemorySize, bytes));
  done.insert({dev, fn});
  return 0;
}

VnSwitches vn_switches() {
  auto env = [](const char* name) { const char* e = getenv(name); return e ? e : ""; };
  VnSwitches s;
  s.wchain4 = env("VAENMF_WCHAIN4")[0] != '0';
  s.team_chain = env("VAENMF_TEAM_CHAIN")[0] == '1';
  s.wfused = env("VAENMF_WFUSED")[0] != '0';
  s.wgroup = env("VAENMF_WGROUP")[0] != '0';
  s.wfused_grid = atoi(env("VAENMF_WFUSED_GRID"));
  s.grid_cap = atoi(env("VAENMF_GRID_CAP"));
  s.keep_zs = env("VAENMF_KEEP_ZS")[0] == '1';
  return s;
}

void vaenmf_set_error(const char* fmt, ...) {
  va_list ap;
  va_start(ap, fmt);
  vsnprintf(g_err, sizeof(g_err), fmt, ap);
  va_end(ap);
}
extern "C" const char* vaenmf_last_error(void) { return g_err; }

long long g_vn_dev_allocs = 0;

namespace {

uint16_t bf16_rne(float v) {
  uint32_t u;
  memcpy(&u, &v, 4);
  if ((u & 0x7F800000u) == 0x7F800000u && (u & 0x007FFFFFu)) return (uint16_t)((u >> 16) | 0x40);
  u += 0x7FFFu + ((u >> 16) & 1u);
  return (uint16_t)(u >> 16);
}
float bf16_to_f(uint16_t h) {
  uint32_t u = (uint32_t)h << 16;
  float v;
  memcpy(&v, &u, 4);
  return v;
}

std::vector<uint16_t> pack_weights(const float* W, int out, int in, int ldw, int ntiles, int nk) {
  std::vector<uint16_t> f((size_t)ntiles * nk * 2 * 64 * 8, 0);
  for (int t = 0; t < ntiles; ++t)
    for (int s = 0; s < nk; ++s)
// ... 34 lines not shown
  VN_REQUIRE(cfg->F >= 1 && cfg->F <= 640, "F=%d out of range (1..640)", cfg->F);
  VN_REQUIRE(cfg->K >= 1 && cfg->K <= 32, "NMF rank K=%d out of range (1..32)", cfg->K);
  VN_REQUIRE(cfg->max_frames >= 1 && cfg->max_utts >= 1, "bad capacities");
  VN_REQUIRE(cfg->precision == VAENMF_PREC_BF16X3 || cfg->precision == VAENMF_PREC_BF16, "bad precision");
  vaenmf_plan* p = new vaenmf_plan();
  memset((void*)&p->cfg, 0, sizeof(p->cfg));
  p->cfg = *cfg;
  p->Fs = (cfg->F + 15) / 16 * 16;
  p->Fm = (cfg->F % 16 == 1 && cfg->F > 16) ? cfg->F - 1 : cfg->F;
  p->NT3 = (p->Fm + 15) / 16;
  p->Kp = cfg->K <= 8 ? 8 : (cfg->K <= 16 ? 16 : 32);
  {
    const char* g = getenv("VAENMF_GEOM");
    int geom = p->NT3 == 16 ? 3 : (p->NT3 <= 20 ? 0 : (p->NT3 == 32 ? 4 : 2));
    if (g && g[0] == '2') geom = p->NT3 == 32 ? 4 : 2;
    p->geom = geom;
    p->nwaves = (geom == 0 || geom == 3) ? 4 : 8;
    p->tile_frames = (geom == 0 || geom == 3) ? 64 : 32;
  }
  p->NT3c = (cfg->F + 15) / 16;
  p->w1f = p->w2f = p->w3f = p->w3c = nullptr;
  p->b1 = p->b2 = p->b3 = p->w1y = p->w3n = p->b3c = nullptr;
  p->d_wt_utt = p->d_wt_n0 = p->d_wt_cnt = nullptr;
  p->n_wtiles = 0; p->Rcap_store = 0; p->last_m_step_path = 0;
  p->Dy = 0;
  p->Lz = cfg->L;
  p->one_hidden = cfg->H2 == 0;
  p->wide = cfg->L > LAT || cfg->H1 != HID || cfg->H2 > HID;
  p->Lp = p->wide ? 128 : LAT;
  const size_t H1 = cfg->H1, H2 = cfg->H2 ? cfg->H2 : HID, Hlast = cfg->H2 ? cfg->H2 : cfg->H1;
  const size_t nk1 = p->Lp / 32, nt3 = p->wide ? p->Fs / 16 : p->NT3;
  p->have_weights = false;
  p->Vb_ext = nullptr;
  p->store_on = false; p->VsS = nullptr; p->src = nullptr; p->VsS_cap = p->src_cap = 0; p->store_R = p->store_Rs = 0;
  p->n_utt = p->NT = p->n_tiles = 0;
  p->prof_on = false;
  p->prof_used = 0;
  int dev = 0;
  hipDeviceProp_t prop;
  VN_CHECK_HIP(hipGetDevice(&dev));
  VN_CHECK_HIP(hipGetDeviceProperties(&prop, dev));
  p->n_sms = prop.multiProcessorCount;
  const size_t NTc = cfg->max_frames, Uc = cfg->max_utts;
  const size_t max_tiles = NTc / 32 + Uc + 1;
  int e = 0;
  e |= dev_alloc(&p->w1f, (H1 / 16) * nk1 * 2 * 64 * 8);
  e |= dev_alloc(&p->w2f, (H2 / 16) * (H1 / 32) * 2 * 64 * 8);
  e |= dev_alloc(&p->w3f, nt3 * (Hlast / 32) * 2 * 64 * 8);
  e |= dev_alloc(&p->b1, H1);
  e |= dev_alloc(&p->b2, H2);
  e |= dev_alloc(&p->b3, p->Fs);
  e |= dev_alloc(&p->w3n, HID);
  e |= dev_alloc(&p->w3c, (size_t)p->NT3c * (HID / 32) * 2 * 64 * 8);
  e |= dev_alloc(&p->b3c, (size_t)p->NT3c * 16);
  const size_t max_wtiles = NTc / 16 + Uc + 1;
  e |= dev_alloc(&p->d_wt_utt, max_wtiles);
  e |= dev_alloc(&p->d_wt_n0, max_wtiles);
  e |= dev_alloc(&p->d_wt_cnt, max_wtiles);
  e |= dev_alloc(&p->d_frame_off, Uc + 1);
  e |= dev_alloc(&p->d_tile_utt, max_tiles);
  e |= dev_alloc(&p->d_tile_n0, max_tiles);
  e |= dev_alloc(&p->d_tile_cnt, max_tiles);
  e |= dev_alloc(&p->d_frame_utt, NTc);
  e |= dev_alloc(&p->d_frame_loc, NTc);
  e |= dev_alloc(&p->d_utt_seed, Uc);
  e |= dev_alloc(&p->A1, NTc * p->Fs);
  e |= dev_alloc(&p->P, NTc * p->Fs);
// ... 15 lines not shown
  return 0;
}

extern "C" void vaenmf_plan_destroy(vaenmf_plan* p) {
  if (!p) return;
  void* ptrs[] = {p->w1f, p->w2f, p->w3f, p->b1, p->b2, p->b3, p->w3n, p->w1y, p->d_frame_off, p->d_tile_utt, p->d_tile_n0,
                  p->d_tile_cnt, p->d_frame_utt, p->d_frame_loc, p->d_utt_seed, p->A1, p->P, p->normW, p->wpart, p->cost_frames,
                  p->VsS, p->src, p->w3c, p->b3c, p->d_wt_utt, p->d_wt_n0, p->d_wt_cnt, p->d_t64_n0, p->d_t64_cnt, p->d_t64_first, p->d_t64_g0,
                  p->wpart64, p->wpart16};
  for (void* q : ptrs)
    if (q) (void)hipFree(q);
  for (hipEvent_t e : p->prof_ev) (void)hipEventDestroy(e);
  p->graphs.release();
  if (p->h_seed_ring) (void)hipHostFree(p->h_seed_ring);
  for (int i = 0; i < vaenmf_plan::SEED_RING; ++i) if (p->seed_ev[i]) (void)hipEventDestroy(p->seed_ev[i]);
  delete p;
}

extern "C" int vaenmf_plan_query(const vaenmf_plan* p, int32_t what) {
  if (!p) return -1;
  switch (what) {
    case VAENMF_Q_FS: return p->Fs;
    case VAENMF_Q_KP: return p->Kp;
    case VAENMF_Q_TILES: return p->n_tiles;
    case VAENMF_Q_NT: return p->NT;
    case VAENMF_Q_NUTT: return p->n_utt;
    case VAENMF_Q_MSTEP_PATH: return p->last_m_step_path;
    case VAENMF_Q_WTILES: return p->n_wtiles;
    case VAENMF_Q_EM_GRAPH: return p->graphs.last;
    case VAENMF_Q_DEV_ALLOCS: return (int)g_vn_dev_allocs;
    case VAENMF_Q_W_FUSED: return p->last_w_fused;
    case VAENMF_Q_CHAIN_KERNEL: return p->last_chain_kernel;
    case VAENMF_Q_LP: return p->Lp;
    default: return -1;
  }
}

static int set_weights_wide(vaenmf_plan* p, const float* W1, int in1, const float* b1, const float* W2, const float* b2,
                            const float* W3, const float* b3) {
  const int Lz = p->Lz, H1 = p->cfg.H1, H2 = p->cfg.H2, HL = H2 ? H2 : H1, F = p->cfg.F, Dy = in1 - Lz;
  const double C2 = 2.0 * 1.4426950408889634, C1 = 1.4426950408889634;
  auto scaled = [](const float* src, size_t n, double c) {
    std::vector<float> v(n);
    for (size_t i = 0; i < n; ++i) v[i] = (float)((double)src[i] * c);
    return v;
  };
  const std::vector<float> W1s = scaled(W1, (size_t)H1 * in1, C2), b1s = scaled(b1, H1, C2);
  const std::vector<float> W3s = scaled(W3, (size_t)F * HL, C1), b3s = scaled(b3, F, C1);
  int e = 0;
  const std::vector<uint16_t> f1 = pack_weights(W1s.data(), H1, Lz, in1, H1 / 16, p->Lp / 32);
  e |= upload((uint16_t*)p->w1f, f1.data(), f1.size());
  e |= upload(p->b1, b1s.data(), (size_t)H1);
  if (!p->one_hidden) {
    const std::vector<float> W2s = scaled(W2, (size_t)H2 * H1, C2), b2s = scaled(b2, H2, C2);
    const std::vector<uint16_t> f2 = pack_weights(W2s.data(), H2, H1, H1, H2 / 16, H1 / 32);
    e |= upload((uint16_t*)p->w2f, f2.data(), f2.size());
    e |= upload(p->b2, b2s.data(), (size_t)H2);
  }
  const std::vector<uint16_t> f3 = pack_weights(W3s.data(), F, HL, HL, p->Fs / 16, HL / 32);
  std::vector<float> b3p(p->Fs, -200.f);
  memcpy(b3p.data(), b3s.data(), sizeof(float) * F);
  e |= upload((uint16_t*)p->w3f, f3.data(), f3.size());
  e |= upload(p->b3, b3p.data(), b3p.size());
  if (p->w1y) { (void)hipFree(p->w1y); p->w1y = nullptr; }
  p->Dy = Dy;
  if (Dy > 0) {
// ... 204 lines not shown
```

### guided-vae-nmf_amd/csrc/stream.hip

```cpp
#include "common.h"

namespace {

typedef __attribute__((ext_vector_type(4))) unsigned u32x4;
typedef __attribute__((ext_vector_type(2))) unsigned u32x2;

constexpr int ST_WAVES = 4;
constexpr int ROW_AUX = 2;

struct StreamArgs {
  const void* VsS;
  const int32_t* src;
  const float *X2, *W, *normW, *Vb, *X;
  float *Ht, *g, *A1, *P, *S_hat, *N_hat, *WFs, *WFn;
  double* cost_frames;
  const int32_t* frame_utt;
  int NT, R, Rs, F, Fm, Fs, K;
  int gains_only;
  int store_f32;
  int w_blk_lds;
  int n_sms;
  const int32_t *t64_n0, *t64_cnt;
  int n_t64;
  float* wpart64;
};

__device__ __forceinline__ float wave_sum(float v) { return sum_rows4(sum_row16(v)); }
__device__ __forceinline__ float vn_uniform(float v) { return __builtin_bit_cast(float, __builtin_amdgcn_readfirstlane(__builtin_bit_cast(int, v))); }
__device__ __forceinline__ float read_lane(const float& v, int l) { return __builtin_bit_cast(float, __builtin_amdgcn_readlane(__builtin_bit_cast(int, v), l)); }

template <int NCH, int KP, typename ST, bool TAIL = false>
struct FrameCtx {
  const StreamArgs& a;
  int lane;
  bool cv[NCH];
  int f0[NCH];
  int nb[NCH];
  unsigned fo[NCH];
  bool has_x;
  static constexpr bool WPRIV = KP <= 8;
  float* wl;
  float wx;
  float nw;
  int wutt, blk_utt, xutt;
  bool in_lds;
  __device__ FrameCtx(const StreamArgs& a_, float* wl_) : a(a_), wl(wl_) {
    lane = threadIdx.x & 63;
#pragma unroll
    for (int c = 0; c < NCH; ++c) {
      f0[c] = 256 * c + 4 * lane; cv[c] = f0[c] < a.Fm; fo[c] = cv[c] ? (unsigned)f0[c] : 0u;
      nb[c] = TAIL ? a.Fm - f0[c] : 0;
    }
    has_x = a.F != a.Fm;
    wutt = -1;
    blk_utt = -1;
    xutt = -1;
    wx = 0.f;
    nw = 1.f;
    in_lds = false;
  }
  __device__ __forceinline__ bool ok(int c, int t) const { return TAIL ? t < nb[c] : cv[c]; }
  __device__ __forceinline__ void pad_bins(f32x4 (&v)[NCH], float pad) const {
    if constexpr (TAIL) {
#pragma unroll
      for (int c = 0; c < NCH; ++c)
#pragma unroll
        for (int t = 1; t < 4; ++t) v[c][t] = ok(c, t) ? v[c][t] : pad;
    }
  }
  __device__ __forceinline__ float nwk(int k) const { return read_lane(nw, k); }
  __device__ __forceinline__ float wxk(int k) const { return read_lane(wx, k); }
  __device__ __forceinline__ void stage_block_w() {
    if (WPRIV || !a.w_blk_lds) return;
    const int wpb = blockDim.x >> 6, nw = gridDim.x * wpb, per = (a.NT + nw - 1) / nw;
    const int n_first = blockIdx.x * wpb * per;
    if (n_first < a.NT) {
      blk_utt = a.frame_utt[n_first];
      const f32x4* src = reinterpret_cast<const f32x4*>(a.W + (size_t)blk_utt * a.Fs * KP);
      for (int e = threadIdx.x; e < a.Fs * KP / 4; e += blockDim.x) put_t(e, src[e]);
    }
    __syncthreads();
  }
  __device__ __forceinline__ void set_utt(int utt, const float* normW = nullptr) {
    if (utt != xutt) {
      xutt = utt;
      unsigned lo = (unsigned)lane;
      asm volatile("" : "+v"(lo));
      const unsigned lk = lo < (unsigned)KP ? lo : 0u;
      wx = (has_x && lo < (unsigned)KP) ? (a.W + ((size_t)utt * a.Fs + a.F - 1) * KP)[lk] : 0.f;
      if (normW) nw = lo < (unsigned)KP ? (normW + (size_t)utt * KP)[lk] : 1.f;
      __builtin_amdgcn_s_waitcnt(0x0F70);
    }
    if (!WPRIV) { in_lds = utt == blk_utt; return; }
// ... 119 lines not shown
  __device__ __forceinline__ void store_row(float* dst, const f32x4 (&v)[NCH], float vx) const {
#pragma unroll
    for (int c = 0; c < NCH; ++c)
      if (cv[c]) *reinterpret_cast<f32x4*>(dst + fo[c]) = v[c];
    if (a.Fm + lane < a.Fs) dst[a.Fm + lane] = (lane == 0 && has_x) ? vx : 0.f;
  }
};

typedef float f32x2 __attribute__((ext_vector_type(2)));
__device__ __forceinline__ f32x2 rcp2(const f32x2 x) { return f32x2{fast_rcp(x[0]), fast_rcp(x[1])}; }
__device__ __forceinline__ f32x2 log2_2(const f32x2 x) { return f32x2{fast_log2(x[0]), fast_log2(x[1])}; }
__device__ __forceinline__ void wstat_term(const f32x4 v, const f32x4 vb, const f32x2 g2, f32x4& a1, f32x4& a2) {
  const f32x2 q0 = rcp2(g2 * v.lo + vb.lo), q1 = rcp2(g2 * v.hi + vb.hi);
  a1.lo += q0; a1.hi += q1;
  a2.lo = q0 * q0 + a2.lo; a2.hi = q1 * q1 + a2.hi;
}

constexpr int row_batch_rows(int elt, int nch, int div) { return (elt == 2 ? 32 : 16) / nch / div; }
template <int NCH, typename ST, int DIV = 1, int RT = 0, int RBX = 0>
struct RowBatch {
  static constexpr int RB = RBX > 0 ? RBX : row_batch_rows((int)sizeof(ST), NCH, DIV);
  static_assert(RT <= RB, "RT");
  __device__ __forceinline__ bool on(int r) const { return RT > 0 ? r < RT : r < nr; }
  using raw_t = typename std::conditional<sizeof(ST) == 4, f32x4, bf16x4>::type;
  raw_t raw[RB][NCH];
  unsigned xbits;
  int nr;
  template <typename FC>
  static __device__ __forceinline__ int load_slots(const FC& fc, const int32_t* scol, int r0, int R) {
    const int nr_ = R - r0 < RB ? R - r0 : RB;
    return *reinterpret_cast<const int32_t*>(reinterpret_cast<const char*>(scol) + (unsigned)(r0 + (fc.lane < nr_ ? fc.lane : 0)) * (unsigned)fc.a.NT * 4u);
  }
  template <typename FC>
  __device__ __forceinline__ void load_rows(const FC& fc, const ST* base, int sl, int r0, int R) {
    nr = RT > 0 ? RT : (R - r0 < RB ? R - r0 : RB);
#pragma unroll
    for (int r = 0; r < RB; ++r)
      if (r == 0 || on(r)) {
        const ST* row = base + (size_t)__builtin_amdgcn_readlane(sl, r) * fc.a.Fs;
#pragma unroll
        for (int c = 0; c < NCH; ++c) raw[r][c] = __builtin_nontemporal_load(reinterpret_cast<const raw_t*>(row + fc.fo[c]));
      }
    if (fc.has_x) {
      if constexpr (sizeof(ST) == 2) xbits = reinterpret_cast<const unsigned short*>(base)[(size_t)sl * fc.a.Fs + fc.a.F - 1];
      else xbits = reinterpret_cast<const unsigned*>(base)[(size_t)sl * fc.a.Fs + fc.a.F - 1];
    } else xbits = 0u;
  }
  template <typename FC>
  __device__ __forceinline__ void load(const FC& fc, const ST* base, const int32_t* scol, int r0, int R) {
    load_rows(fc, base, load_slots(fc, scol, r0, R), r0, R);
  }
  template <typename FC>
  __device__ __forceinline__ void load_rows_buf(const FC& fc, __amdgpu_buffer_rsrc_t rs, unsigned frame_off, int sl, int R, int r0 = 0) {
    nr = RT > 0 ? RT : (R - r0 < RB ? R - r0 : RB);
    const unsigned rowb = (unsigned)fc.a.Fs * (unsigned)sizeof(ST);
    if (fc.has_x) {
      const unsigned o = frame_off + (unsigned)sl * rowb + (unsigned)(fc.a.F - 1) * (unsigned)sizeof(ST);
      if constexpr (sizeof(ST) == 2) xbits = (unsigned)__builtin_amdgcn_raw_buffer_load_b16(rs, o, 0, 0);
      else xbits = (unsigned)__builtin_amdgcn_raw_buffer_load_b32(rs, o, 0, 0);
    } else xbits = 0u;
#pragma unroll
    for (int r = 0; r < RB; ++r)
      if (r == 0 || on(r)) {
        const unsigned so = frame_off + (unsigned)__builtin_amdgcn_readlane(sl, r) * rowb;
#pragma unroll
        for (int c = 0; c < NCH; ++c) {
          const unsigned vo = (unsigned)(fc.cv[c] ? fc.f0[c] : 0) * (unsigned)sizeof(ST);
          if constexpr (sizeof(ST) == 2) raw[r][c] = __builtin_bit_cast(raw_t, __builtin_amdgcn_raw_buffer_load_b64(rs, vo, so, 0));
          else raw[r][c] = __builtin_bit_cast(raw_t, __builtin_amdgcn_raw_buffer_load_b128(rs, vo, so, 0));
        }
      }
  }
  template <typename FN>
  __device__ __forceinline__ void for_rows(FN f) const {
    constexpr int CH = 1;
#pragma unroll
    for (int r0 = 0; r0 < RB; r0 += CH) {
      if (RT > 0 ? r0 + CH <= RT : r0 + CH <= nr) {
#pragma unroll
        for (int r = r0; r < r0 + CH && r < RB; ++r) f(r);
      } else {
#pragma unroll
        for (int r = r0; r < r0 + CH && r < RB; ++r)
          if (on(r)) f(r);
      }
    }
  }
  __device__ __forceinline__ float x() const {
    if constexpr (sizeof(ST) == 2) return __builtin_bit_cast(float, xbits << 16);
    else return __builtin_bit_cast(float, xbits);
// ... 2 lines not shown
#pragma unroll
    for (int r = 0; r < RB; ++r)
#pragma unroll
      for (int c = 0; c < NCH; ++c) asm volatile("" : "+v"(raw[r][c]));
  }
  __device__ __forceinline__ void get(int r, f32x4 (&v)[NCH]) const {
#pragma unroll
    for (int c = 0; c < NCH; ++c) v[c] = f32x4{(float)raw[r][c][0], (float)raw[r][c][1], (float)raw[r][c][2], (float)raw[r][c][3]};
  }
  template <typename FC>
  __device__ __forceinline__ float xmask(const FC& fc) const { return (fc.has_x && fc.lane < nr) ? 1.f : 0.f; }
};

__device__ __forceinline__ void wave_frames(int NT, int& n_beg, int& n_end) {
  const int wpb = blockDim.x >> 6;
  const int gw = blockIdx.x * wpb + (threadIdx.x >> 6), nw = gridDim.x * wpb;
  const int per = (NT + nw - 1) / nw;
  n_beg = __builtin_amdgcn_readfirstlane(gw * per);
  n_end = n_beg + per < NT ? n_beg + per : NT;
}

template <int NCH, int KP, typename ST>
__global__ __launch_bounds__(256, (KP <= 8 && NCH == 1) ? ST_WAVES : 2) void wstats_stream_kernel(const StreamArgs a) {
  extern __shared__ __attribute__((aligned(16))) float wlds[];
  FrameCtx<NCH, KP, ST> fc(a, wlds + (KP <= 8 ? (size_t)(threadIdx.x >> 6) * a.Fs * KP : 0));
  fc.stage_block_w();
  using RBt = RowBatch<NCH, ST>;
  int n_beg, n_end;
  wave_frames(a.NT, n_beg, n_end);
  using Half = RowBatch<NCH, ST, 2>;
  constexpr int HB = Half::RB;
  if (a.R <= 2 * HB) {
    Half h0, h1;
    auto base_of = [&](int n) { return reinterpret_cast<const ST*>(a.VsS) + (size_t)n * a.Rs * a.Fs; };
    const int R0 = a.R < HB ? a.R : HB;
    if (n_beg < n_end) {
      h0.load(fc, base_of(n_beg), a.src + n_beg, 0, R0);
      if (a.R > HB) h1.load(fc, base_of(n_beg), a.src + n_beg, HB, a.R); else h1.nr = 0, h1.xbits = 0u;
    }
    for (int n = n_beg; n < n_end; ++n) {
      const int utt = a.frame_utt[n];
      fc.set_utt(utt);
      const float gn = a.g[n];
      float h[KP];
#pragma unroll
      for (int k = 0; k < KP; k += 4) {
        const f32x4 hv = *reinterpret_cast<const f32x4*>(a.Ht + (size_t)n * KP + k);
#pragma unroll
        for (int t = 0; t < 4; ++t) h[k + t] = vn_uniform(hv[t]);
      }
      f32x4 vb[NCH], x2[NCH], a1[NCH], a2[NCH];
      float vbx, x2x, a1x = 0.f, a2x = 0.f;
      fc.noise_var(utt, h, vb, vbx);
      fc.load_x2(n, x2, x2x);
#pragma unroll
      for (int c = 0; c < NCH; ++c) a1[c] = a2[c] = f32x4{0.f, 0.f, 0.f, 0.f};
      auto consume = [&](const Half& hb) {
#pragma unroll
        for (int r = 0; r < HB; ++r)
          if (r < hb.nr) {
            f32x4 v[NCH];
            hb.get(r, v);
#pragma unroll
            for (int c = 0; c < NCH; ++c) {
              const f32x2 g2 = {gn, gn};
              const f32x2 q0 = rcp2(g2 * v[c].lo + vb[c].lo), q1 = rcp2(g2 * v[c].hi + vb[c].hi);
              a1[c].lo += q0; a1[c].hi += q1;
              a2[c].lo = q0 * q0 + a2[c].lo; a2[c].hi = q1 * q1 + a2[c].hi;
            }
          }
        const float q = fast_rcp(gn * hb.x() + vbx) * hb.xmask(fc);
        a1x += wave_sum(q);
        a2x += wave_sum(q * q);
      };
      consume(h0);
      if (n + 1 < n_end) h0.load(fc, base_of(n + 1), a.src + n + 1, 0, R0);
      if (a.R > HB) {
        consume(h1);
        if (n + 1 < n_end) h1.load(fc, base_of(n + 1), a.src + n + 1, HB, a.R);
      }
#pragma unroll
      for (int c = 0; c < NCH; ++c)
#pragma unroll
        for (int t = 0; t < 4; ++t) a2[c][t] *= x2[c][t];
      fc.store_row(a.A1 + (size_t)n * a.Fs, a1, a1x);
      fc.store_row(a.P + (size_t)n * a.Fs, a2, a2x * x2x);
    }
    return;
  }
  for (int n = n_beg; n < n_end; ++n) {
    const ST* base = reinterpret_cast<const ST*>(a.VsS) + (size_t)n * a.Rs * a.Fs;
    const int32_t* srow = a.src + n;
    RBt rb;
    rb.load(fc, base, srow, 0, a.R);
    const int utt = a.frame_utt[n];
    fc.set_utt(utt);
    const float gn = a.g[n];
    float h[KP];
#pragma unroll
    for (int k = 0; k < KP; k += 4) {
      const f32x4 hv = *reinterpret_cast<const f32x4*>(a.Ht + (size_t)n * KP + k);
#pragma unroll
      for (int t = 0; t < 4; ++t) h[k + t] = vn_uniform(hv[t]);
    }
    f32x4 vb[NCH], x2[NCH], a1[NCH], a2[NCH];
    float vbx, x2x, a1x = 0.f, a2x = 0.f;
    fc.noise_var(utt, h, vb, vbx);
    fc.load_x2(n, x2, x2x);
#pragma unroll
    for (int c = 0; c < NCH; ++c) a1[c] = a2[c] = f32x4{0.f, 0.f, 0.f, 0.f};
    for (int r0 = 0; r0 < a.R; r0 += RBt::RB) {
      if (r0 > 0) rb.load(fc, base, srow, r0, a.R);
#pragma unroll
      for (int r = 0; r < RBt::RB; ++r)
        if (r < rb.nr) {
          f32x4 v[NCH];
          rb.get(r, v);
#pragma unroll
          for (int c = 0; c < NCH; ++c) {
            const f32x2 g2 = {gn, gn};
            const f32x2 q0 = rcp2(g2 * v[c].lo + vb[c].lo), q1 = rcp2(g2 * v[c].hi + vb[c].hi);
            a1[c].lo += q0; a1[c].hi += q1;
            a2[c].lo = q0 * q0 + a2[c].lo; a2[c].hi = q1 * q1 + a2[c].hi;
          }
        }
      const float q = fast_rcp(gn * rb.x() + vbx) * rb.xmask(fc);
      a1x += wave_sum(q);
      a2x += wave_sum(q * q);
    }
#pragma unroll
    for (int c = 0; c < NCH; ++c)
#pragma unroll
      for (int t = 0; t < 4; ++t) a2[c][t] *= x2[c][t];
    fc.store_row(a.A1 + (size_t)n * a.Fs, a1, a1x);
    fc.store_row(a.P + (size_t)n * a.Fs, a2, a2x * x2x);
  }
}

template <int NCH, int KP, typename ST, int RT = 0, bool TAIL = false>
__global__ __launch_bounds__(256, (KP <= 8 && NCH == 1 && sizeof(ST) == 2) ? ST_WAVES : 2) void hg_stream_kernel(const StreamArgs a) {
  extern __shared__ __attribute__((aligned(16))) float wlds[];
  FrameCtx<NCH, KP, ST, TAIL> fc(a, wlds + (KP <= 8 ? (size_t)(threadIdx.x >> 6) * a.Fs * KP : 0));
  fc.stage_block_w();
  using RBt = RowBatch<NCH, ST, 1, RT, ((sizeof(ST) == 2 && NCH == 2 && KP <= 16) || (sizeof(ST) == 4 && NCH == 1 && KP <= 8)) ? 32 : 0>;
  int n_beg, n_end;
  wave_frames(a.NT, n_beg, n_end);
  const bool one = a.R <= RBt::RB;
  for (int n = n_beg; n < n_end; ++n) {
    const ST* base = reinterpret_cast<const ST*>(a.VsS) + (size_t)n * a.Rs * a.Fs;
    const int32_t* srow = a.src + n;
    RBt rb;
    const int utt = a.frame_utt[n];
    const float gn = a.g[n];
    const int sl = RBt::load_slots(fc, srow, 0, a.R);
    f32x4 vb[NCH], x2[NCH];
    float vbx, x2x;
    fc.load_x2(n, x2, x2x);
    float hs[KP];
    if (a.gains_only) {
      fc.ext_var(n, vb, vbx);
    } else {
#pragma unroll
      for (int k = 0; k < KP; k += 4) {
        const f32x4 hv = *reinterpret_cast<const f32x4*>(a.Ht + (size_t)n * KP + k);
#pragma unroll
        for (int t = 0; t < 4; ++t) hs[k + t] = hv[t];
      }
    }
    fc.set_utt(utt, a.gains_only ? nullptr : a.normW);
    rb.load_rows(fc, base, sl, 0, a.R);
    const f32x2 gn2 = {gn, gn};
    if (!a.gains_only) {
#pragma unroll
      for (int k = 0; k < KP; ++k) hs[k] = vn_uniform(hs[k] * fc.nwk(k));
      fc.noise_var(utt, hs, vb, vbx);
      f32x4 a1[NCH], a2[NCH];
      float a1x = 0.f, a2x = 0.f;
#pragma unroll
      for (int c = 0; c < NCH; ++c) a1[c] = a2[c] = f32x4{0.f, 0.f, 0.f, 0.f};
      for (int r0 = 0; r0 < a.R; r0 += RBt::RB) {
        if (r0 > 0) rb.load(fc, base, srow, r0, a.R);
        auto row1 = [&](int r) {
          f32x4 v[NCH];
          rb.get(r, v);
#pragma unroll
          for (int c = 0; c < NCH; ++c) wstat_term(v[c], vb[c], gn2, a1[c], a2[c]);
        };
        rb.for_rows(row1);
        const float q = fast_rcp(gn * rb.x() + vbx) * rb.xmask(fc);
        a1x += wave_sum(q);
        a2x += wave_sum(q * q);
      }
#pragma unroll
      for (int c = 0; c < NCH; ++c)
#pragma unroll
        for (int t = 0; t < 4; ++t) {
          a2[c][t] = fc.ok(c, t) ? a2[c][t] * x2[c][t] : 0.f;
          a1[c][t] = fc.ok(c, t) ? a1[c][t] : 0.f;
        }
      const bool lead = fc.lane == 0 && fc.has_x;
      a2x = lead ? a2x * x2x : 0.f;
      a1x = lead ? a1x : 0.f;
      float hn[KP];
#pragma unroll
      for (int k = 0; k < KP; ++k) {
        float nu, de;
        fc.w_dot(utt, k, a2, a1, a2x, a1x, nu, de);
        nu = wave_sum(nu);
        de = wave_sum(de);
        hn[k] = vn_uniform(k < a.K ? hs[k] * __builtin_amdgcn_sqrtf(nu * fast_rcp(de)) : 0.f);
      }
      if (fc.lane == 0) {
#pragma unroll
        for (int k = 0; k < KP; k += 4)
          *reinterpret_cast<f32x4*>(a.Ht + (size_t)n * KP + k) = f32x4{hn[k], hn[k + 1], hn[k + 2], hn[k + 3]};
      }
      fc.noise_var(utt, hn, vb, vbx);
    }
    float nu = 0.f, de = 0.f;
    if (one) rb.repack();
    {
      f32x4 ng[NCH], dg[NCH];
      float ngx = 0.f, dgx = 0.f;
#pragma unroll
      for (int c = 0; c < NCH; ++c) ng[c] = dg[c] = f32x4{0.f, 0.f, 0.f, 0.f};
      for (int r0 = 0; r0 < a.R; r0 += RBt::RB) {
        if (!one) rb.load(fc, base, srow, r0, a.R);
        auto row2 = [&](int r) {
          f32x4 v[NCH];
          rb.get(r, v);
#pragma unroll
          for (int c = 0; c < NCH; ++c) {
            const f32x2 q0 = rcp2(gn2 * v[c].lo + vb[c].lo), q1 = rcp2(gn2 * v[c].hi + vb[c].hi);
            const f32x2 vq0 = v[c].lo * q0, vq1 = v[c].hi * q1;
            dg[c].lo += vq0; dg[c].hi += vq1;
            ng[c].lo = vq0 * q0 + ng[c].lo; ng[c].hi = vq1 * q1 + ng[c].hi;
          }
        };
        rb.for_rows(row2);
        const float q = fast_rcp(gn * rb.x() + vbx), vq = rb.x() * q * rb.xmask(fc);
        dgx += wave_sum(vq);
        ngx += wave_sum(vq * q);
      }
#pragma unroll
      for (int c = 0; c < NCH; ++c)
        if (fc.cv[c]) {
#pragma unroll
          for (int t = 0; t < 4; ++t)
            if (!TAIL || fc.ok(c, t)) { nu += x2[c][t] * ng[c][t]; de += dg[c][t]; }
        }
      if (fc.lane == 0 && fc.has_x) { nu += x2x * ngx; de += dgx; }
      nu = wave_sum(nu);
      de = wave_sum(de);
    }
    const float gnew = gn * __builtin_amdgcn_sqrtf(nu * fast_rcp(de));
    if (fc.lane == 0) a.g[n] = gnew;
    const f32x2 gw2 = {gnew, gnew};
    if (one) rb.repack();
    f32x4 cl[NCH], cx[NCH];
    float clx = 0.f, cxx = 0.f;
#pragma unroll
    for (int c = 0; c < NCH; ++c) cl[c] = cx[c] = f32x4{0.f, 0.f, 0.f, 0.f};
    for (int r0 = 0; r0 < a.R; r0 += RBt::RB) {
      if (!one) rb.load(fc, base, srow, r0, a.R);
#pragma unroll
      for (int r = 0; r < RBt::RB; r += 2) {
        if (rb.on(r + 1)) {
          f32x4 v0[NCH], v1[NCH];
          rb.get(r, v0);
          rb.get(r + 1, v1);
#pragma unroll
          for (int c = 0; c < NCH; ++c) {
            const f32x2 xa0 = gw2 * v0[c].lo + vb[c].lo, xa1 = gw2 * v1[c].lo + vb[c].lo;
            const f32x2 xb0 = gw2 * v0[c].hi + vb[c].hi, xb1 = gw2 * v1[c].hi + vb[c].hi;
            const f32x2 pa = xa0 * xa1, pb = xb0 * xb1;
            cl[c].lo += log2_2(pa); cl[c].hi += log2_2(pb);
            cx[c].lo = (xa0 + xa1) * rcp2(pa) + cx[c].lo; cx[c].hi = (xb0 + xb1) * rcp2(pb) + cx[c].hi;
          }
        } else if (rb.on(r)) {
          f32x4 v0[NCH];
          rb.get(r, v0);
#pragma unroll
          for (int c = 0; c < NCH; ++c) {
            const f32x2 xa = gw2 * v0[c].lo + vb[c].lo, xb = gw2 * v0[c].hi + vb[c].hi;
            cl[c].lo += log2_2(xa); cl[c].hi += log2_2(xb);
            cx[c].lo += rcp2(xa); cx[c].hi += rcp2(xb);
          }
        }
      }
      const float xm = rb.xmask(fc), x0 = gnew * rb.x() + vbx;
      clx += wave_sum(fast_log2(x0) * xm);
      cxx += wave_sum(fast_rcp(x0) * xm);
    }
    float cs = 0.f;
#pragma unroll
    for (int c = 0; c < NCH; ++c)
      if (fc.cv[c]) {
#pragma unroll
        for (int t = 0; t < 4; ++t)
          if (!TAIL || fc.ok(c, t)) cs += cl[c][t] * LN2_F + x2[c][t] * cx[c][t];
      }
    if (fc.lane == 0 && fc.has_x) cs += clx * LN2_F + x2x * cxx;
    const double cd = sum_rows4_d((double)sum_row16(cs));
    if (fc.lane == 0) a.cost_frames[n] = cd;
  }
}

template <int NCH, int KP, typename ST, bool TAIL = false>
__global__ __launch_bounds__(256, (KP <= 8 && NCH == 1) ? ST_WAVES : 2) void wf_stream_kernel(const StreamArgs a) {
  extern __shared__ __attribute__((aligned(16))) float wlds[];
  FrameCtx<NCH, KP, ST, TAIL> fc(a, wlds + (KP <= 8 ? (size_t)(threadIdx.x >> 6) * a.Fs * KP : 0));
  fc.stage_block_w();
  using RBt = RowBatch<NCH, ST>;
  int n_beg, n_end;
  wave_frames(a.NT, n_beg, n_end);
  const float invR = 1.0f / (float)a.R;
  for (int n = n_beg; n < n_end; ++n) {
    const ST* base = reinterpret_cast<const ST*>(a.VsS) + (size_t)n * a.Rs * a.Fs;
    const int32_t* srow = a.src + n;
    RBt rb;
    rb.load(fc, base, srow, 0, a.R);
    const int utt = a.frame_utt[n];
    fc.set_utt(utt);
    const float gn = a.g[n];
    f32x4 vb[NCH];
    float vbx;
    if (a.Vb) {
      fc.ext_var(n, vb, vbx);
    } else {
      float h[KP];
#pragma unroll
      for (int k = 0; k < KP; k += 4) {
        const f32x4 hv = *reinterpret_cast<const f32x4*>(a.Ht + (size_t)n * KP + k);
#pragma unroll
        for (int t = 0; t < 4; ++t) h[k + t] = vn_uniform(hv[t]);
      }
      fc.noise_var(utt, h, vb, vbx);
    }
    f32x4 ws[NCH], wn[NCH];
    float wsx = 0.f, wnx = 0.f;
#pragma unroll
    for (int c = 0; c < NCH; ++c) ws[c] = wn[c] = f32x4{0.f, 0.f, 0.f, 0.f};
    for (int r0 = 0; r0 < a.R; r0 += RBt::RB) {
      if (r0 > 0) rb.load(fc, base, srow, r0, a.R);
#pragma unroll
      for (int r = 0; r < RBt::RB; ++r)
        if (r < rb.nr) {
          f32x4 v[NCH];
          rb.get(r, v);
#pragma unroll
          for (int c = 0; c < NCH; ++c) {
            const f32x2 g2 = {gn, gn};
            const f32x2 s0 = g2 * v[c].lo, s1 = g2 * v[c].hi;
            const f32x2 q0 = rcp2(s0 + vb[c].lo), q1 = rcp2(s1 + vb[c].hi);
            ws[c].lo = s0 * q0 + ws[c].lo; ws[c].hi = s1 * q1 + ws[c].hi;
            wn[c].lo = vb[c].lo * q0 + wn[c].lo; wn[c].hi = vb[c].hi * q1 + wn[c].hi;
          }
        }
      const float sc = gn * rb.x(), q = fast_rcp(sc + vbx) * rb.xmask(fc);
      wsx += wave_sum(sc * q);
      wnx += wave_sum(vbx * q);
    }
#pragma unroll
    for (int c = 0; c < NCH; ++c)
      if (fc.cv[c]) {
        const size_t o = (size_t)n * a.Fs + fc.f0[c];
#pragma unroll
        for (int t = 0; t < 4; ++t) {
          const float ms = (!TAIL || fc.ok(c, t)) ? ws[c][t] * invR : 0.f, mn = (!TAIL || fc.ok(c, t)) ? wn[c][t] * invR : 0.f;
          const float xr = a.X[2 * (o + t)], xi = a.X[2 * (o + t) + 1];
          a.S_hat[2 * (o + t)] = ms * xr;  a.S_hat[2 * (o + t) + 1] = ms * xi;
          a.N_hat[2 * (o + t)] = mn * xr;  a.N_hat[2 * (o + t) + 1] = mn * xi;
          if (a.WFs) a.WFs[o + t] = ms;
          if (a.WFn) a.WFn[o + t] = mn;
        }
      }
    if (a.Fm + fc.lane < a.Fs) {
// ... 1 lines not shown
      const bool lead = fc.lane == 0 && fc.has_x;
      const float ms = lead ? wsx * invR : 0.f, mn = lead ? wnx * invR : 0.f;
      const float xr = a.X[2 * o], xi = a.X[2 * o + 1];
      a.S_hat[2 * o] = ms * xr;  a.S_hat[2 * o + 1] = ms * xi;
      a.N_hat[2 * o] = mn * xr;  a.N_hat[2 * o + 1] = mn * xi;
      if (a.WFs) a.WFs[o] = ms;
      if (a.WFn) a.WFn[o] = mn;
    }
  }
}

template <int NCH, int KP>
struct FrameSmall {
  f32x4 x2[NCH];
  float x2x, g;
  float hl;
  int utt;
  __device__ __forceinline__ void get_h(float (&h)[KP]) const {
#pragma unroll
    for (int k = 0; k < KP; ++k) h[k] = read_lane(hl, k);
  }
};

template <int NCH, int KP, typename ST, int RT>
__global__ __launch_bounds__(256, 2) void wstats_stream2_kernel(const StreamArgs a) {
  extern __shared__ __attribute__((aligned(16))) float wlds[];
  FrameCtx<NCH, KP, ST> fc(a, wlds + (KP <= 8 ? (size_t)(threadIdx.x >> 6) * a.Fs * KP : 0));
  fc.stage_block_w();
  using RBt = RowBatch<NCH, ST, 1, RT>;
  using FS = FrameSmall<NCH, KP>;
  int n_beg, n_end;
  wave_frames(a.NT, n_beg, n_end);
  if (n_beg >= n_end) return;
  __amdgpu_buffer_rsrc_t vrs = __builtin_amdgcn_make_buffer_rsrc(const_cast<void*>(a.VsS), 0, (int)((unsigned)a.NT * (unsigned)(a.Rs * a.Fs) * (unsigned)sizeof(ST)), 0x00020000);
  auto request = [&](int n, RBt& rb, FS& s, int sl) {
    s.utt = a.frame_utt[n];
    s.g = a.g[n];
    s.hl = a.Ht[(size_t)n * KP + (fc.lane < KP ? fc.lane : 0)];
    fc.load_x2(n, s.x2, s.x2x);
    rb.load_rows_buf(fc, vrs, (unsigned)n * (unsigned)(a.Rs * a.Fs) * (unsigned)sizeof(ST), sl, a.R);
  };
  auto compute = [&](int n, RBt& rb, const FS& s) {
    fc.set_utt(s.utt);
    f32x4 vb[NCH], a1[NCH], a2[NCH];
    float vbx, a1x = 0.f, a2x = 0.f;
    float h[KP];
    s.get_h(h);
    fc.noise_var(s.utt, h, vb, vbx);
#pragma unroll
    for (int c = 0; c < NCH; ++c) a1[c] = a2[c] = f32x4{0.f, 0.f, 0.f, 0.f};
#pragma unroll
    for (int r = 0; r < RBt::RB; ++r) {
      constexpr int ROWGRP = 6;
      if (RT > 0 && (r % ROWGRP) == 0) __builtin_amdgcn_sched_barrier(0);
      if (rb.on(r)) {
        f32x4 v[NCH];
        rb.get(r, v);
#pragma unroll
        for (int c = 0; c < NCH; ++c) wstat_term(v[c], vb[c], f32x2{s.g, s.g}, a1[c], a2[c]);
      }
    }
    const float q = fast_rcp(s.g * rb.x() + vbx) * rb.xmask(fc);
    a1x = wave_sum(q);
    a2x = wave_sum(q * q);
#pragma unroll
    for (int c = 0; c < NCH; ++c)
#pragma unroll
      for (int t = 0; t < 4; ++t) a2[c][t] *= s.x2[c][t];
    fc.store_row(a.A1 + (size_t)n * a.Fs, a1, a1x);
    fc.store_row(a.P + (size_t)n * a.Fs, a2, a2x * s.x2x);
  };
  auto slots = [&](int n) { return n < n_end ? RBt::load_slots(fc, a.src + n, 0, a.R) : 0; };
  RBt rbA, rbB;
  FS sA, sB;
  int sl1 = slots(n_beg + 1);
  request(n_beg, rbA, sA, slots(n_beg));
  for (int n = n_beg; n < n_end; n += 2) {
    int sl2 = 0, sl3 = 0;
    if (n + 1 < n_end) { request(n + 1, rbB, sB, sl1); sl2 = slots(n + 2); }
    compute(n, rbA, sA);
    if (n + 1 < n_end) {
      if (n + 2 < n_end) { request(n + 2, rbA, sA, sl2); sl3 = slots(n + 3); }
      compute(n + 1, rbB, sB);
    }
    sl1 = sl3;
  }
}

template <int KP>
struct RotSmall {
  f32x4 x2;
  float pk;
  __device__ __forceinline__ float lane_f(int l) const { return read_lane(pk, l); }
  __device__ __forceinline__ int utt() const { return __builtin_amdgcn_readlane(__builtin_bit_cast(int, pk), KP); }
  __device__ __forceinline__ float g() const { return lane_f(KP + 1); }
  __device__ __forceinline__ float x2x() const { return lane_f(KP + 2); }
};

template <int KP, int RT>
struct RotCtx {
  using FC = FrameCtx<1, KP, __bf16>;
  const StreamArgs& a;
  const FC& fc;
  __amdgpu_buffer_rsrc_t vrs;
  unsigned rowb, frameb, voff, xvoff;
  const char* pk_base;
  unsigned pk_stride;
  bf16x4 raw[2][RT];
  unsigned xb[2];
  __device__ RotCtx(const StreamArgs& a_, const FC& fc_) : a(a_), fc(fc_) {
    vrs = __builtin_amdgcn_make_buffer_rsrc(const_cast<void*>(a.VsS), 0, (int)((unsigned)a.NT * (unsigned)(a.Rs * a.Fs) * 2u), 0x00020000);
    rowb = (unsigned)a.Fs * 2u;
    frameb = (unsigned)a.Rs * rowb;
    voff = (unsigned)(fc.cv[0] ? fc.f0[0] : 0) * 2u;
    xvoff = (unsigned)(a.F - 1) * 2u;
    xb[0] = xb[1] = 0u;
    const int l = fc.lane;
    if (l == KP) { pk_base = reinterpret_cast<const char*>(a.frame_utt); pk_stride = 4u; }
    else if (l == KP + 1) { pk_base = reinterpret_cast<const char*>(a.g); pk_stride = 4u; }
    else if (l == KP + 2 && fc.has_x) { pk_base = reinterpret_cast<const char*>(a.X2 + a.F - 1); pk_stride = (unsigned)a.Fs * 4u; }
    else if (a.Ht) { pk_base = reinterpret_cast<const char*>(a.Ht + (l < KP ? l : 0)); pk_stride = (unsigned)KP * 4u; }
    else { pk_base = reinterpret_cast<const char*>(a.g); pk_stride = 4u; }
  }
  __device__ __forceinline__ int slots(int n) const {
    return *reinterpret_cast<const int32_t*>(reinterpret_cast<const char*>(a.src + n) + (unsigned)(fc.lane < RT ? fc.lane : 0) * (unsigned)a.NT * 4u);
  }
  __device__ __forceinline__ void req_small(int n, RotSmall<KP>& s) const {
    s.pk = *reinterpret_cast<const float*>(pk_base + (size_t)n * pk_stride);
    f32x4 x2v[1];
    float unused;
    fc.load_x2(n, x2v, unused);
    s.x2 = x2v[0];
  }
  template <int S>
  __device__ __forceinline__ void req_row(int n, int sl, int r, float after, unsigned vbase) {
    const unsigned so = (unsigned)n * frameb + (unsigned)__builtin_amdgcn_readlane(sl, r) * rowb;
    unsigned vo = vbase;
    asm volatile("" : "+v"(vo) : "v"(after));
    raw[S][r] = __builtin_bit_cast(bf16x4, __builtin_amdgcn_raw_buffer_load_b64(vrs, vo, so, ROW_AUX));
  }
  template <int S>
  __device__ __forceinline__ void req_x(int n, int sl, bool on) {
    if (fc.has_x) xb[S] = (unsigned)__builtin_amdgcn_raw_buffer_load_b16(vrs, on ? (unsigned)sl * rowb + xvoff : 0xF0000000u, (unsigned)n * frameb, 0);
  }
  template <int S>
  __device__ __forceinline__ f32x4 row(int r) const {
    return f32x4{(float)raw[S][r][0], (float)raw[S][r][1], (float)raw[S][r][2], (float)raw[S][r][3]};
  }
  template <int S>
  __device__ __forceinline__ float x() const { return __builtin_bit_cast(float, xb[S] << 16); }
  __device__ __forceinline__ float xmask() const { return (fc.has_x && fc.lane < RT) ? 1.f : 0.f; }
};

template <int KP>
__device__ __forceinline__ void rot_h(float hl, float (&h)[KP]) {
#pragma unroll
  for (int k = 0; k < KP; ++k) h[k] = read_lane(hl, k);
}

constexpr int WF_TILE = 64, WF_WFR = 16;
template <int KP>
__host__ __device__ constexpr int wf_acc_floats() { return 2 * KP * 256 + 128; }
template <int KP, int RT>
__global__ __launch_bounds__(256, 2) void wstats_fused_kernel(const StreamArgs a) {
  extern __shared__ __attribute__((aligned(16))) float wlds[];
  const int wave = __builtin_amdgcn_readfirstlane(threadIdx.x >> 6);
  FrameCtx<1, KP, __bf16> fc(a, wlds);
  float* acc_all = wlds + (size_t)a.Fs * KP;
  float* acc = acc_all + (size_t)wave * wf_acc_floats<KP>();
  RotCtx<KP, RT> rc(a, fc);
  const unsigned l4 = (unsigned)fc.lane * 4u;
  for (int tile = blockIdx.x; tile < a.n_t64; tile += gridDim.x) {
    const int t_n0 = a.t64_n0[tile], t_cnt = a.t64_cnt[tile];
    const int utt = a.frame_utt[t_n0];
    __syncthreads();
    if (utt != fc.wutt) {
// ... 98 lines not shown
}

template <int KP, int RT, typename ST>
__global__ __launch_bounds__(256, 2) void wstats_group_kernel(const StreamArgs a, const int32_t* __restrict__ wt_n0,
                                                              const int32_t* __restrict__ wt_cnt, int n_groups, float* __restrict__ part16) {
  extern __shared__ __attribute__((aligned(16))) float wlds[];
  const int wave = __builtin_amdgcn_readfirstlane(threadIdx.x >> 6);
  FrameCtx<1, KP, ST> fc(a, wlds);
  float* acc = wlds + (size_t)a.Fs * KP;
  using RBt = RowBatch<1, ST, 1, RT, (sizeof(ST) == 4 ? 32 : 0)>;
  const unsigned l4 = (unsigned)fc.lane * 4u;
  for (int grp = blockIdx.x; grp < n_groups; grp += gridDim.x) {
    const int g_n0 = wt_n0[grp], g_cnt = wt_cnt[grp];
    const int utt = a.frame_utt[g_n0];
    __syncthreads();
    if (utt != fc.wutt) {
      const f32x4* src = reinterpret_cast<const f32x4*>(a.W + (size_t)utt * a.Fs * KP);
      for (int e = threadIdx.x; e < a.Fs * KP / 4; e += 256) fc.put_t(e, src[e]);
      fc.wutt = utt;
    }
    for (int sidx = wave; sidx < 2 * KP; sidx += 4) *reinterpret_cast<f32x4*>(acc + sidx * 256 + l4) = f32x4{0.f, 0.f, 0.f, 0.f};
    if (wave == 0) { acc[2 * KP * 256 + fc.lane] = 0.f; acc[2 * KP * 256 + 64 + fc.lane] = 0.f; }
    __syncthreads();
    const int n_beg = g_n0 + 4 * wave;
    const int n_end = n_beg + 4 < g_n0 + g_cnt ? n_beg + 4 : g_n0 + g_cnt;
    f32x4 A1[4], A2[4];
    float a1xs[4], pxs[4], hls[4];
#pragma unroll
    for (int i = 0; i < 4; ++i) {
      A1[i] = A2[i] = f32x4{0.f, 0.f, 0.f, 0.f};
      a1xs[i] = pxs[i] = hls[i] = 0.f;
      const int n = n_beg + i;
      if (n < n_end) {
        const ST* base = reinterpret_cast<const ST*>(a.VsS) + (size_t)n * a.Rs * a.Fs;
        const int sl = RBt::load_slots(fc, a.src + n, 0, RT);
        const float gn = a.g[n];
        f32x4 x2[1];
        float x2x;
        fc.load_x2(n, x2, x2x);
        float h[KP];
#pragma unroll
        for (int k = 0; k < KP; k += 4) {
          const f32x4 hv = *reinterpret_cast<const f32x4*>(a.Ht + (size_t)n * KP + k);
#pragma unroll
          for (int t = 0; t < 4; ++t) h[k + t] = vn_uniform(hv[t]);
        }
        hls[i] = fc.lane < KP ? a.Ht[(size_t)n * KP + (fc.lane < KP ? fc.lane : 0)] : 0.f;
        fc.set_utt(utt);
        RBt rb;
        rb.load_rows(fc, base, sl, 0, RT);
        f32x4 vb[1], a1, a2;
        float vbx;
        fc.noise_var(utt, h, vb, vbx);
        a1 = a2 = f32x4{0.f, 0.f, 0.f, 0.f};
        const f32x2 g2 = {gn, gn};
        auto row1 = [&](int r) {
          f32x4 v[1];
          rb.get(r, v);
          wstat_term(v[0], vb[0], g2, a1, a2);
        };
        rb.for_rows(row1);
        const float q = fast_rcp(gn * rb.x() + vbx) * rb.xmask(fc);
        const float a1x = wave_sum(q), a2x = wave_sum(q * q);
        a2 *= x2[0];
        A1[i] = a1; A2[i] = a2;
        a1xs[i] = a1x;
        pxs[i] = a2x * x2x;
      }
    }
    for (int r = 0; r < 4; ++r) {
      if (wave == r) {
#pragma unroll
        for (int i = 0; i < 4; ++i)
          if (n_beg + i < n_end) {
            float h[KP];
            rot_h<KP>(hls[i], h);
            const f32x4 a1 = A1[i], a2 = A2[i];
#pragma unroll
            for (int k0 = 0; k0 < KP; k0 += 4) {
              f32x4 nv[4], dv[4];
#pragma unroll
              for (int t = 0; t < 4; ++t) {
                nv[t] = *reinterpret_cast<const f32x4*>(acc + (2 * (k0 + t)) * 256 + l4);
// ... 3 lines not shown
              for (int t = 0; t < 4; ++t) {
                const f32x4 hh = {h[k0 + t], h[k0 + t], h[k0 + t], h[k0 + t]};
                *reinterpret_cast<f32x4*>(acc + (2 * (k0 + t)) * 256 + l4) = __builtin_elementwise_fma(a2, hh, nv[t]);
                *reinterpret_cast<f32x4*>(acc + (2 * (k0 + t) + 1) * 256 + l4) = __builtin_elementwise_fma(a1, hh, dv[t]);
              }
            }
            const float hl = hls[i];
            float numx = acc[2 * KP * 256 + fc.lane], denx = acc[2 * KP * 256 + 64 + fc.lane];
            numx = __builtin_fmaf(pxs[i], hl, numx);
            denx = __builtin_fmaf(a1xs[i], hl, denx);
            acc[2 * KP * 256 + fc.lane] = numx;
            acc[2 * KP * 256 + 64 + fc.lane] = denx;
          }
      }
      __syncthreads();
    }
    float* dst = part16 + (size_t)grp * 2 * KP * a.Fs;
    for (int sidx = wave; sidx < 2 * KP; sidx += 4) {
      const f32x4 v = *reinterpret_cast<const f32x4*>(acc + sidx * 256 + l4);
      if (fc.cv[0]) *reinterpret_cast<f32x4*>(dst + (size_t)sidx * a.Fs + fc.f0[0]) = v;
    }
    if (wave == 0 && fc.has_x && fc.lane < KP) {
      dst[(size_t)(2 * fc.lane) * a.Fs + a.F - 1] = acc[2 * KP * 256 + fc.lane];
      dst[(size_t)(2 * fc.lane + 1) * a.Fs + a.F - 1] = acc[2 * KP * 256 + 64 + fc.lane];
    }
  }
}

StreamArgs base_args(const vaenmf_plan* p) {
  StreamArgs a = {};
  a.VsS = p->VsS; a.src = p->src; a.frame_utt = p->d_frame_utt; a.Vb = p->Vb_ext;
  a.store_f32 = p->cfg.precision == VAENMF_PREC_BF16X3;
  a.n_sms = p->n_sms;
  a.NT = p->NT; a.R = p->store_R; a.Rs = p->store_Rs; a.F = p->cfg.F; a.Fm = p->Fm; a.Fs = p->Fs; a.K = p->cfg.K;
  return a;
}

enum { SK_WSTATS, SK_HG, SK_WF };
enum { W_TWO_KERNELS = 0, W_FUSED = 1, W_GROUP = 2 };

struct StreamForm {
  int nch, kp;
  bool f32;
  bool tail;
  int hg_rt;
  bool pipelined;
  int w_path;
};

StreamForm stream_form(const vaenmf_plan* p, const StreamArgs& a) {
  StreamForm f = {};
  const int nch = (p->Fm + 255) / 256;
  f.nch = nch <= 1 ? 1 : (nch == 2 ? 2 : 3);
  f.kp = (p->Kp == 8 || p->Kp == 16) ? p->Kp : 32;
  f.f32 = a.store_f32 != 0;
  f.tail = (a.Fm & 3) != 0;
  const bool small = f.nch == 1 && f.kp == 8;
  if (!f.tail && ((small && (a.R == 30 || a.R == 10)) || (f.nch == 2 && !f.f32 && f.kp == 16 && a.R == 30))) f.hg_rt = a.R;
  f.pipelined = small && a.R <= row_batch_rows(f.f32 ? 4 : 2, 1, 1);
  f.w_path = W_TWO_KERNELS;
  if (!f.f32 && p->Kp == 8 && nch == 1 && (a.R == 30 || a.R == 10) && !a.gains_only && vn_switches().wfused)
    f.w_path = (p->wpart16 && p->n_wtiles <= p->n_sms && vn_switches().wgroup) ? W_GROUP : W_FUSED;
  return f;
}

template <int V> using ic = std::integral_constant<int, V>;
// ... 117 lines not shown
```

### guided-vae-nmf_amd/csrc/wide.hip

```cpp
#include "common.h"

namespace {

constexpr int WD_LP = 128;
constexpr int WD_MAXT = 10;

struct WideArgs {
  const __bf16 *w1f, *w2f, *w3f;
  const float *b1, *b2, *b3;
  int NT1, NT2, NT3;
  int NK1, NK2, NK3;
  int H1, Lz, F, Fs, Kp, NT;
  const float *X2, *W, *Ht, *g, *B1, *Vb;
  float *Z, *Zs, *acc_out;
  void* VsS; int32_t* src; int Rs;
  const int32_t *wt_utt, *wt_n0, *wt_cnt, *frame_off;
  const uint64_t* utt_seed;
  const float *eps, *u;
  int Rcap, nsamples, burnin, rng_mode, update_Z;
  uint32_t call;
  float sd;
};

template <bool SPLIT>
__device__ __forceinline__ void wd_split8(const float (&z)[8], bf16x8& hi, bf16x8& lo) {
#pragma unroll
  for (int j = 0; j < 8; ++j) {
    const __bf16 h = (__bf16)z[j];
    hi[j] = h;
    lo[j] = SPLIT ? (__bf16)(z[j] - (float)h) : (__bf16)0.f;
  }
}

template <bool SPLIT, bool STORE>
__global__ __launch_bounds__(256) void widechain_kernel(const WideArgs a) {
  constexpr int PARTS = SPLIT ? 2 : 1;
  using store_t = typename std::conditional<SPLIT, float, __bf16>::type;
  __shared__ __attribute__((aligned(16))) char zimg[4 * PARTS * 1024];
  __shared__ __attribute__((aligned(16))) char act1[8 * PARTS * 1024];
  __shared__ __attribute__((aligned(16))) char act2[8 * PARTS * 1024];
  __shared__ double epart[4][16];
  __shared__ float ppart[4][16];
  __shared__ float ush[16];

  const int lane = threadIdx.x & 63, q = lane >> 4, c = lane & 15;
  const int w = __builtin_amdgcn_readfirstlane(threadIdx.x >> 6);
  const unsigned lane16 = lane * 16;
  const int tile = blockIdx.x;
// ... 93 lines not shown
#pragma unroll
    for (int i = 0; i < 4; ++i) {
      const int t = w + 4 * i;
      if (t < a.NT1) {
        f32x4 acc = bias1[i];
        for (int s = 0; s < a.NK1; ++s) {
          bf16x8 whi, wlo, ahi, alo;
          wfrag(a.w1f, t, 4, s, whi, wlo);
          afrag(zimg, s, ahi, alo);
          acc = mma3<SPLIT>(whi, wlo, ahi, alo, acc);
        }
        store_act(act1, t, acc);
      }
    }
    __syncthreads();
    if (a.NT2 > 0) {
#pragma unroll
      for (int i = 0; i < 4; ++i) {
        const int t = w + 4 * i;
        if (t < a.NT2) {
          f32x4 acc = bias2[i];
          for (int s = 0; s < a.NK2; ++s) {
            bf16x8 whi, wlo, ahi, alo;
            wfrag(a.w2f, t, a.NK2, s, whi, wlo);
            afrag(act1, s, ahi, alo);
            acc = mma3<SPLIT>(whi, wlo, ahi, alo, acc);
          }
          store_act(act2, t, acc);
        }
      }
      __syncthreads();
    }
    const char* last = a.NT2 > 0 ? act2 : act1;
    char* const vrow = DOST ? reinterpret_cast<char*>(a.VsS) + ((size_t)nrow * a.Rs + slot) * a.Fs * sizeof(store_t) : nullptr;
    double e = 0.0;
#pragma unroll
    for (int i = 0; i < WD_MAXT; ++i) {
      const int t = w + 4 * i;
      if (t < a.NT3) {
        f32x4 acc = *reinterpret_cast<const f32x4*>(a.b3 + 16 * t + 4 * q);
        for (int s = 0; s < a.NK3; ++s) {
          bf16x8 whi, wlo, ahi, alo;
          wfrag(a.w3f, t, a.NK3, s, whi, wlo);
          afrag(last, s, ahi, alo);
          acc = mma3<SPLIT>(whi, wlo, ahi, alo, acc);
        }
        f32x4 ev;
        float pl = 0.f, px = 0.f;
#pragma unroll
        for (int k = 0; k < 4; ++k) {
          ev[k] = fast_exp(acc[k]);
          const float vx = gn * ev[k] + vb[i][k];
          pl += fast_log2(vx);
          px += x2[i][k] * fast_rcp(vx);
        }
        if (DOST && fvalid) {
          store_t* dst = reinterpret_cast<store_t*>(vrow) + 16 * t + 4 * q;
          if (SPLIT) *reinterpret_cast<f32x4*>(dst) = ev;
          else *reinterpret_cast<bf16x4*>(dst) = bf16x4{(__bf16)ev[0], (__bf16)ev[1], (__bf16)ev[2], (__bf16)ev[3]};
        }
        e += (double)(pl * LN2_F + px);
      }
    }
    e = sum_rows4_d(e);
    pr = sum_rows4(pr);
    if (q == 0) { epart[w][c] = e; ppart[w][c] = pr; }
    if (ulane) ush[c] = uu;
    __syncthreads();
    E = ((epart[0][c] + epart[1][c]) + epart[2][c]) + epart[3][c];
    P = ((ppart[0][c] + ppart[1][c]) + ppart[2][c]) + ppart[3][c];
    U = ush[c];
  };

  double Ecur = 0.0;
  int cur_src = a.nsamples;
  const int n_it = vn_chain_passes<STORE>(a.nsamples, a.burnin);
  for (int it = -1; it < n_it; ++it) {
    const VnChainPass ps = vn_chain_pass<STORE>(it, a.nsamples, a.burnin);
    const bool re = ps.re, step = ps.step;
    const int m = ps.m, slot = ps.slot;
    float e8[8] = {0, 0, 0, 0, 0, 0, 0, 0}, uu = 1.f;
    if (step) {
      f32x4 e0 = {0, 0, 0, 0}, e1 = {0, 0, 0, 0};
      if (a.rng_mode == VAENMF_RNG_DEVICE) {
        if (on0) e0 = normal4(st0);
        if (on1) e1 = normal4(st1);
        if (ulane) uu = uniform01(st0);
      } else {
        const size_t row = (size_t)m * a.NT + nrow;
// ... 39 lines not shown
    *reinterpret_cast<f32x4*>(dst + l0) = f32x4{z[0], z[1], z[2], z[3]};
    *reinterpret_cast<f32x4*>(dst + l1) = f32x4{z[4], z[5], z[6], z[7]};
  }
}

__global__ void wide_rng_fill_kernel(const int32_t* wt_utt, const int32_t* wt_n0, const int32_t* wt_cnt, const int32_t* frame_off,
                                     const uint64_t* utt_seed, uint32_t call, int S, int NT, float* eps_out, float* u_out) {
  const int tile = blockIdx.x, sfr = threadIdx.x >> 5, squad = threadIdx.x & 31;
  const int utt = wt_utt[tile], n0 = wt_n0[tile], cnt = wt_cnt[tile];
  if (sfr >= cnt) return;
  Xs128 st = xs_seed(utt_seed[utt], (uint32_t)(n0 - frame_off[utt] + sfr), (uint32_t)squad, call);
  for (int s = 0; s < S; ++s) {
    const f32x4 e = normal4(st);
    const size_t row = (size_t)s * NT + n0 + sfr;
    *reinterpret_cast<f32x4*>(eps_out + row * WD_LP + 4 * squad) = e;
    if (squad == 0) u_out[row] = uniform01(st);
  }
}

}

int vn_launch_widechain(vaenmf_plan* p, const VnChainCall& cc, hipStream_t st) {
  VN_REQUIRE(p->wide, "vn_launch_widechain: not a wide plan");
  WideArgs a = {};
  a.w1f = p->w1f; a.w2f = p->w2f; a.w3f = p->w3f; a.b1 = p->b1; a.b2 = p->b2; a.b3 = p->b3;
  a.H1 = p->cfg.H1; a.Lz = p->Lz;
  a.NT1 = a.H1 / 16; a.NT2 = p->cfg.H2 / 16; a.NT3 = p->Fs / 16;
  a.NK1 = (p->Lz + 31) / 32; a.NK2 = a.H1 / 32; a.NK3 = (p->one_hidden ? a.H1 : p->cfg.H2) / 32;
  VN_REQUIRE(a.NT3 <= 4 * WD_MAXT && a.NT1 <= 16 && a.NT2 <= 16 && a.NK2 <= 8 && a.NK3 <= 8 && a.NK1 <= 4 && p->Lp == WD_LP,
             "wide chain: shape outside the kernel's tiles");
  a.F = p->cfg.F; a.Fs = p->Fs; a.Kp = p->Kp; a.NT = p->NT;
  a.X2 = cc.X2; a.W = cc.W; a.Ht = cc.Ht; a.g = cc.g; a.B1 = cc.B1; a.Vb = p->Vb_ext;
  a.Z = cc.Z; a.Zs = cc.Zs; a.acc_out = cc.acc_out;
  a.VsS = cc.VsS; a.src = cc.src; a.Rs = cc.Rs;
  a.wt_utt = p->d_wt_utt; a.wt_n0 = p->d_wt_n0; a.wt_cnt = p->d_wt_cnt; a.frame_off = p->d_frame_off;
  a.utt_seed = p->d_utt_seed; a.eps = cc.eps; a.u = cc.u;
  a.Rcap = cc.Rcap; a.nsamples = cc.nsamples; a.burnin = cc.burnin; a.rng_mode = cc.rng_mode; a.update_Z = cc.update_Z;
  a.call = cc.call; a.sd = cc.sd;
  const bool split = p->cfg.precision == VAENMF_PREC_BF16X3;
  const dim3 grid(p->n_wtiles), blk(256);
  if (split) {
    if (a.VsS) hipLaunchKernelGGL((widechain_kernel<true, true>), grid, blk, 0, st, a);
    else hipLaunchKernelGGL((widechain_kernel<true, false>), grid, blk, 0, st, a);
  } else {
    if (a.VsS) hipLaunchKernelGGL((widechain_kernel<false, true>), grid, blk, 0, st, a);
    else hipLaunchKernelGGL((widechain_kernel<false, false>), grid, blk, 0, st, a);
  }
  VN_CHECK_HIP(hipGetLastError());
  p->last_chain_kernel = 3;
  return 0;
}

int vn_launch_wide_rng_fill(vaenmf_plan* p, uint32_t call, int S, float* eps_out, float* u_out, hipStream_t st) {
  hipLaunchKernelGGL(wide_rng_fill_kernel, dim3(p->n_wtiles), dim3(16 * 32), 0, st, p->d_wt_utt, p->d_wt_n0, p->d_wt_cnt,
                     p->d_frame_off, p->d_utt_seed, call, S, p->NT, eps_out, u_out);
  VN_CHECK_HIP(hipGetLastError());
  return 0;
}
```

### guided-vae-nmf_amd/vaenmf/_lib.py

```python
import ctypes as C
import os

_HERE = os.path.dirname(os.path.abspath(__file__))
LIB_PATH = os.environ.get("VAENMF_LIB") or os.path.join(_HERE, "libvaenmf.so")

PREC_BF16X3, PREC_BF16 = 0, 1
RNG_REPLAY, RNG_DEVICE = 0, 1
Q_FS, Q_KP, Q_TILES, Q_NT, Q_NUTT, Q_MSTEP_PATH, Q_WTILES, Q_EM_GRAPH, Q_DEV_ALLOCS, Q_W_FUSED, Q_CHAIN_KERNEL, Q_LP = 0, 1, 2, 3, 4, 5, 6, 7, 8, 9, 10, 11
ACT_NONE, ACT_TANH, ACT_RELU, ACT_SIGMOID, ACT_STEP = 0, 1, 2, 3, 4
LABEL_IBM, LABEL_VAD = 0, 1


class Config(C.Structure):
    _fields_ = [("F", C.c_int32), ("K", C.c_int32), ("L", C.c_int32), ("H1", C.c_int32), ("H2", C.c_int32),
                ("max_frames", C.c_int32), ("max_utts", C.c_int32), ("precision", C.c_int32)]


class Rng(C.Structure):
    _fields_ = [("mode", C.c_int32), ("call", C.c_uint32), ("eps", C.c_void_p), ("u", C.c_void_p)]


PAD_REFLECT, PAD_CONSTANT = 0, 1


class StftOpts(C.Structure):
    _fields_ = [("nfft", C.c_int32), ("hop", C.c_int32), ("center", C.c_int32), ("pad_mode", C.c_int32),
                ("window", C.c_void_p)]


_P, _I, _I64, _F, _D = C.c_void_p, C.c_int32, C.c_int64, C.c_float, C.c_double
SIGNATURES = {
    "vaenmf_last_error": (C.c_char_p, []),
    "vaenmf_plan_create": (_I, [C.POINTER(Config), C.POINTER(_P)]),
    "vaenmf_plan_destroy": (None, [_P]),
    "vaenmf_plan_query": (_I, [_P, _I]),
    "vaenmf_set_decoder_weights": (_I, [_P, _P, _I, _P, _P, _P, _P, _P]),
    "vaenmf_bind_batch": (_I, [_P, _I, _P, _P]),
    "vaenmf_bind_batch_async": (_I, [_P, _I, _P, _P, _P]),
    "vaenmf_set_noise_psd": (_I, [_P, _P]),
    "vaenmf_init_nmf": (_I, [_P, _P, _P, _P, C.c_uint64, _F, _P]),
    "vaenmf_layer1_bias": (_I, [_P, _P, _I, _P, _P]),
    "vaenmf_mh_chain": (_I, [_P, _P, _P, _P, _P, _P, _I, _P, _P, _I, _I, _I, _F, C.POINTER(Rng), _P, _P]),
    "vaenmf_sample_store": (_I, [_P, _I]),
    "vaenmf_sample_store_gather": (_I, [_P, _P, _P]),
    "vaenmf_m_step_stored": (_I, [_P, _P, _P, _P, _P, _P, _P]),
    "vaenmf_wiener_stored": (_I, [_P, _P, _P, _P, _P, _P, _P, _P, _P, _P]),
    "vaenmf_rng_fill": (_I, [_P, C.c_uint32, _I, _P, _P, _P]),
    "vaenmf_decode": (_I, [_P, _P, _I, _I, _P, _P, _P]),
    "vaenmf_m_step": (_I, [_P, _P, _P, _P, _P, _P, _I, _I, _P, _P, _P]),
    "vaenmf_wiener": (_I, [_P, _P, _P, _P, _P, _P, _I, _I, _P, _P, _P, _P, _P, _P, _P]),
    "vaenmf_em_run": (_I, [_P, _P, _P, _P, _P, _P, _P, _P, _I, _I, _I, _I, _I, _I, _F, _P, _P, _P, _P, _P]),
    "vaenmf_dense": (_I, [_P, _I, _I, _I, _P, _P, _I, _I, _P, _I, _P]),
    "vaenmf_power_spec": (_I, [_P, _P, _I64, _P]),
    "vaenmf_stft_geometry": (_I, [_I64, _D, _D, _D, _I, C.POINTER(_I), C.POINTER(_I), C.POINTER(_I), C.POINTER(_I)]),
    "vaenmf_stft_batch_ex": (_I, [_P, _I, _P, _P, _P, _P, C.POINTER(StftOpts), _I, _P, _P]),
    "vaenmf_istft_batch_ex": (_I, [_P, _I, _I, _P, _P, C.POINTER(StftOpts), _I, _P, _P, _P]),
    "vaenmf_resample_ratio": (_I, [_I64, _I64, C.POINTER(_I), C.POINTER(_I)]),
    "vaenmf_resample_length": (_I64, [_I64, _I, _I]),
    "vaenmf_resample_taps": (_I, [_I, _I, _I, _D, _P]),
    "vaenmf_resample_batch": (_I, [_P, _I, _P, _P, _I, _I, _I, _D, _P, _P]),
    "vaenmf_segment_count": (_I, [_I, _P, _I, _I, C.POINTER(_I64), C.POINTER(_I64)]),
    "vaenmf_segment_table": (_I, [_I, _P, _I, _I, _I, _P, _P, _P, _P, _P, _P, _P, _P]),
    "vaenmf_gather_rows": (_I, [_P, _P, _I64, _I, _P, _P]),
    "vaenmf_blend_rows": (_I, [_P, _P, _P, _P, _I64, _I, _P, _P]),
    "vaenmf_lorenz_work_bytes": (_I64, [_I, _I, _I, _I]),
    "vaenmf_lorenz_labels": (_I, [_P, _I, _P, _I, _I, _I, _F, _F, _F, _P, _I, _P, _P, _I64, _P]),
    "vaenmf_wiener_mask": (_I, [_P, _P, _I64, _F, _P, _P]),
    "vaenmf_apply_mask": (_I, [_P, _P, _I, _I, _I, _I, _P, _P]),
    "vaenmf_spp_estimate": (_I, [_P, _I, _I, _P, _I, _D, _D, _D, _D, _I, _P, _P, _I, _P]),
    "vaenmf_spp_noise_given": (_I, [_P, _P, _I64, _D, _P, _P]),
    "vaenmf_gram3_batch": (_I, [_P, _P, _P, _I, _P, _P, _P]),
    "vaenmf_profile_enable": (_I, [_P, _I]),
    "vaenmf_profile_read": (_I, [_P, _P, _P]),
    "vaenmf_wchain_addressable": (_I, [_I64, _I, _I, _I, _I, _I, _I]),
    "vaenmf_hbm_read_probe": (_I, [_P, _I64, _I, _P, C.POINTER(_D), _P]),
}

_lib = None


def lib():
    global _lib
    if _lib is None:
        if not os.path.exists(LIB_PATH):
            raise RuntimeError("libvaenmf.so not found at %s -- build it with "
                               "`python -c 'import __graft_entry__ as g; g.build()'`; "
                               "there is no CPU fallback" % LIB_PATH)
        l = C.CDLL(LIB_PATH)
        for name, (res, args) in SIGNATURES.items():
            fn = getattr(l, name)
            fn.restype = res
            fn.argtypes = args
        _lib = l
    return _lib


class VaenmfError(RuntimeError):
    pass


def check(rc):
    if rc != 0:
        raise VaenmfError("libvaenmf: %s (code %d)" % (lib().vaenmf_last_error().decode(), rc))
```

### include/vaenmf.h

```cpp
#ifndef VAENMF_H
#define VAENMF_H

#include <stdint.h>

#ifdef __cplusplus
extern "C" {
#endif

typedef struct vaenmf_plan vaenmf_plan;

enum { VAENMF_PREC_BF16X3 = 0,
       VAENMF_PREC_BF16   = 1 };

enum { VAENMF_RNG_REPLAY = 0,
       VAENMF_RNG_DEVICE = 1 };

enum { VAENMF_Q_FS = 0, VAENMF_Q_KP = 1, VAENMF_Q_TILES = 2, VAENMF_Q_NT = 3, VAENMF_Q_NUTT = 4,
       VAENMF_Q_MSTEP_PATH = 5,
       VAENMF_Q_WTILES = 6,
       VAENMF_Q_EM_GRAPH = 7,
       VAENMF_Q_W_FUSED = 9,
       VAENMF_Q_CHAIN_KERNEL = 10,
       VAENMF_Q_LP = 11,
       VAENMF_Q_DEV_ALLOCS = 8 };

enum { VAENMF_ACT_NONE = 0, VAENMF_ACT_TANH = 1, VAENMF_ACT_RELU = 2, VAENMF_ACT_SIGMOID = 3,
       VAENMF_ACT_STEP = 4 };

typedef struct {
  int32_t F;
  int32_t K;
  int32_t L;
  int32_t H1, H2;
  int32_t max_frames;
  int32_t max_utts;
  int32_t precision;
} vaenmf_config;

typedef struct {
  int32_t  mode;
  uint32_t call;
  const float* eps;
  const float* u;
} vaenmf_rng;

const char* vaenmf_last_error(void);

int  vaenmf_plan_create(const vaenmf_config* cfg, vaenmf_plan** out);
void vaenmf_plan_destroy(vaenmf_plan* p);
int  vaenmf_plan_query(const vaenmf_plan* p, int32_t what);

int vaenmf_set_decoder_weights(vaenmf_plan* p, const float* W1, int32_t in1, const float* b1,
                               const float* W2, const float* b2, const float* W3, const float* b3);

int vaenmf_bind_batch(vaenmf_plan* p, int32_t n_utt, const int32_t* frame_offsets,
                      const uint64_t* utt_seeds);
// ... 6 lines not shown

int vaenmf_set_noise_psd(vaenmf_plan* p, const float* Vb);

int vaenmf_mh_chain(vaenmf_plan* p, const float* X2, const float* W, const float* Ht, const float* g,
                    float* Z, int32_t update_Z, const float* B1, float* Zs, int32_t Rcap,
                    int32_t nsamples, int32_t burnin, float var_rw,
                    const vaenmf_rng* rng, float* acc_out, void* stream);

int vaenmf_wchain_addressable(int64_t NT, int32_t Rcap, int32_t steps, int32_t Fs, int32_t Kp, int32_t n_utt, int32_t replay);

int vaenmf_rng_fill(vaenmf_plan* p, uint32_t call, int32_t S, float* eps_out, float* u_out, void* stream);

int vaenmf_decode(vaenmf_plan* p, const float* Zs, int32_t Rcap, int32_t R, const float* B1,
                  float* Vs_out, void* stream);

int vaenmf_m_step(vaenmf_plan* p, const float* X2, float* W, float* Ht, float* g,
                  const float* Zs, int32_t Rcap, int32_t R, const float* B1,
                  double* cost_frames, void* stream);

int vaenmf_wiener(vaenmf_plan* p, const float* X2, const float* W, const float* Ht, const float* g,
                  const float* Zs, int32_t Rcap, int32_t R, const float* B1,
                  const float* X, float* S_hat, float* N_hat, float* WFs, float* WFn, void* stream);

int vaenmf_em_run(vaenmf_plan* p, const float* X2, float* W, float* Ht, float* g, float* Z,
                  const float* B1, float* Zs, int32_t Rcap, int32_t niter,
                  int32_t nsE, int32_t biE, int32_t nsWF, int32_t biWF, float var_rw,
                  const float* X, float* S_hat, float* N_hat, double* cost, void* stream);

int vaenmf_dense(const float* X, int32_t M, int32_t in, int32_t ldx, const float* Wt, const float* b,
                 int32_t out, int32_t act, float* Y, int32_t ldy, void* stream);

int vaenmf_sample_store(vaenmf_plan* plan, int32_t max_samples);
int vaenmf_sample_store_gather(vaenmf_plan* plan, float* Vs_out, void* stream);
int vaenmf_m_step_stored(vaenmf_plan* plan, const float* X2, float* W, float* Ht, float* g,
                         double* cost_frames, void* stream);
int vaenmf_wiener_stored(vaenmf_plan* plan, const float* W, const float* Ht, const float* g,
                         const float* X, float* S_hat, float* N_hat, float* WFs, float* WFn,
                         void* stream);

int vaenmf_power_spec(const float* X, float* X2, int64_t n, void* stream);

#define VAENMF_PAD_REFLECT 0
#define VAENMF_PAD_CONSTANT 1
typedef struct vaenmf_stft_opts {
  int32_t nfft;
  int32_t hop;
  int32_t center;
  int32_t pad_mode;
  const double* window;
} vaenmf_stft_opts;
int vaenmf_stft_geometry(int64_t n_samples, double fs, double wlen_sec, double hop_percent,
                         int32_t center, int32_t* nfft, int32_t* hop, int32_t* n_frames,
                         int32_t* n_padded);
int vaenmf_stft_batch_ex(const float* wav, int32_t n_frames_total, const int64_t* sample_offsets,
                         const int32_t* frame_offsets, const int32_t* frame_utt,
                         const int32_t* padded_len, const vaenmf_stft_opts* opts, int32_t Fs,
                         float* X, void* stream);
int vaenmf_istft_batch_ex(const float* S, int32_t n_utt, int32_t n_frames_total,
                          const int64_t* sample_offsets, const int32_t* frame_offsets,
                          const vaenmf_stft_opts* opts, int32_t Fs, float* work,
                          float* wav_out, void* stream);

int vaenmf_resample_ratio(int64_t fs_in, int64_t fs_out, int32_t* up, int32_t* down);
int64_t vaenmf_resample_length(int64_t n_in, int32_t up, int32_t down);
int vaenmf_resample_taps(int32_t up, int32_t down, int32_t zeros, double beta, double* h);
int vaenmf_resample_batch(const float* x, int32_t n_utt, const int64_t* in_offsets, const int64_t* out_offsets,
// ... 42 lines not shown
```

Before: 457,400 frames/s.

## Store sample variances in line-aligned rows with the odd Nyquist bin parked separately

Changes the stored sample-variance layout so each row holds F-1 (256 or 512) bins, which keeps rows aligned to cache lines, and moves the odd last bin into a separate per-frame region. Chain kernels collect that last bin in an LDS park area through cross-lane permutes and flush it once per frame with vector stores. The consumer kernels (M-step and Wiener streaming) and the wide kernel are updated to read the new layout. This is meant to remove misaligned and partial-line stores and loads of the sample store, at the cost of extra LDS, a per-frame flush, and more complex addressing.

```diff
diff --git a/guided-vae-nmf_amd/csrc/chain.hip b/guided-vae-nmf_amd/csrc/chain.hip
--- a/guided-vae-nmf_amd/csrc/chain.hip
+++ b/guided-vae-nmf_amd/csrc/chain.hip
@@ -28,6 +28,8 @@
   float *Z, *Zs, *acc_out;
   void* VsS;
   unsigned VsS_bytes;
+  VnStoreLayout lay;
+  int park_lds;
   int32_t* src;
   int Rs;
   const int32_t *wt_utt, *wt_n0, *wt_cnt;
@@ -156,8 +158,45 @@
   }
 }
 
-template <int MAXT, bool EXACT, bool SPLIT, bool STORE, int NWAVES, bool LOL, bool HIALL, bool M2, int GT>
+__device__ __forceinline__ unsigned wc_lane_here() {
+  unsigned l;
+  asm volatile("v_mbcnt_lo_u32_b32 %0, -1, 0\n\tv_mbcnt_hi_u32_b32 %0, -1, %0" : "=&v"(l));
+  return l;
+}
+__device__ __forceinline__ unsigned wc_or_rows4(unsigned a) {
+  auto r = __builtin_amdgcn_permlane16_swap(a, opaque_copy(a), false, false);
+  unsigned x = r[0], y = r[1];
+  asm volatile("" : "+v"(x), "+v"(y));
+  a = x | y;
+  auto r2 = __builtin_amdgcn_permlane32_swap(a, opaque_copy(a), false, false);
+  x = r2[0]; y = r2[1];
+  asm volatile("" : "+v"(x), "+v"(y));
+  return x | y;
+}
+template <typename store_t>
+__device__ __forceinline__ void wc_park(char* area, unsigned xb, int slot, unsigned bits) {
+  const unsigned l = wc_lane_here();
+  const unsigned v = wc_or_rows4(l < 16u ? bits : 0u);
+  char* dst = area + (l & 15u) * xb + (unsigned)slot * (unsigned)sizeof(store_t);
+  if constexpr (sizeof(store_t) == 4) *reinterpret_cast<unsigned*>(dst) = v;
+  else *reinterpret_cast<unsigned short*>(dst) = (unsigned short)v;
+}
+template <typename store_t>
+__device__ __forceinline__ void wc_flush_odd(const WcArgs& a, __amdgpu_buffer_rsrc_t vrs, const char* area, bool fvalid, int nrow) {
+  __builtin_amdgcn_s_waitcnt(0xC07F);
+  __builtin_amdgcn_wave_barrier();
+  const unsigned xb = a.lay.xframe * (unsigned)sizeof(store_t);
+  const unsigned l = wc_lane_here(), q = l >> 4;
+  const char* park = area + (l & 15u) * xb;
+  const unsigned xo = fvalid ? ((unsigned)a.lay.xbase + (unsigned)nrow * a.lay.xframe) * (unsigned)sizeof(store_t) : WC_OOB;
+  for (unsigned j = 16u * (unsigned)q; j < xb; j += 64u)
+    __builtin_amdgcn_raw_buffer_store_b128(*reinterpret_cast<const u32x4*>(park + j), vrs, xo + j, 0, 0);
+  __builtin_amdgcn_wave_barrier();
+}
+
+template <int MAXT, bool EXACT, bool SPLIT, bool STORE, int NWAVES, bool LOL, bool HIALL, bool M2, int GT, bool ALN = false>
 __global__ __launch_bounds__(NWAVES * 64, NWAVES / 4) void wchain_kernel(const WcArgs a) {
+  static_assert(!ALN || (STORE && EXACT && MAXT == 17), "ALN");
   extern __shared__ __attribute__((aligned(16))) char smem[];
   using L = WcLds<SPLIT>;
   constexpr int PARTS = L::PARTS;
@@ -192,6 +231,9 @@
     float* b3s = reinterpret_cast<float*>(smem + L::B3);
     for (int i = threadIdx.x; i < HID; i += nthr) { b1s[i] = a.b1[i]; b2s[i] = a.b2[i]; }
     for (int i = threadIdx.x; i < 16 * NT3; i += nthr) b3s[i] = a.b3[i];
+    if (ALN)
+      for (unsigned e = threadIdx.x * 16u; e < NWAVES * WT_FRAMES * a.lay.xframe * (unsigned)sizeof(store_t); e += nthr * 16u)
+        *reinterpret_cast<u32x4*>(smem + a.park_lds + e) = u32x4{0u, 0u, 0u, 0u};
   }
   __syncthreads();
 
@@ -243,7 +285,9 @@
     }
     float z[8];
     wc_load_z(R, fr, q, z);
-    const unsigned fbase = STORE ? (fr.fvalid ? (unsigned)nrow * (unsigned)(a.Rs * a.Fs) * (unsigned)sizeof(store_t) : WC_OOB) : 0u;
+    const unsigned fbase = STORE ? (fr.fvalid ? (unsigned)nrow * a.lay.frame * (unsigned)sizeof(store_t) : WC_OOB) : 0u;
+    const unsigned xpark = a.lay.xframe * (unsigned)sizeof(store_t);
+    char* const park = smem + (ALN ? a.park_lds + wave * WT_FRAMES * (int)xpark : 0);
     const unsigned zs_off = fr.fvalid ? ((unsigned)nrow * (unsigned)a.Rcap * LAT + 4u * q) * 4u : WC_OOB;
     const unsigned fr_off = (fr.fvalid && q == 0) ? (unsigned)nrow * 4u : WC_OOB;
     const unsigned rp_off = ((unsigned)nrow * LAT + 4u * q) * 4u;
@@ -260,7 +304,7 @@
     WC_STAMP_DECL
     auto energy = [&](const float (&zz)[8], int slot, auto dost) -> double {
       constexpr bool DOST = STORE && decltype(dost)::value;
-      const unsigned voff = DOST ? fbase + (unsigned)slot * (unsigned)a.Fs * (unsigned)sizeof(store_t) : 0u;
+      const unsigned voff = DOST ? fbase + (unsigned)slot * a.lay.row * (unsigned)sizeof(store_t) : 0u;
       u32x4 bh[NK_H], bl[NK_H], ch[NK_H], cl[NK_H];
       auto put = [&](u32x4 (&dh)[NK_H], u32x4 (&dl)[NK_H], int t, const f32x4 h) {
         dh[t >> 1][2 * (t & 1)] = pk2(h[0], h[1]);
@@ -405,7 +449,9 @@
                     const f32x2 rc = {fast_rcp(pp[0]), fast_rcp(pp[1])};
                     px2 = (x2[t].lo * v1 + x2[t].hi * v0) * rc + px2;
                   }
-                  if (DOST) {
+                  if (DOST && ALN && t == MAXT - 1) {
+                    wc_park<store_t>(park, xpark, slot, SPLIT ? __builtin_bit_cast(unsigned, ev[0]) : (pk2(ev[0], ev[1]) & 0xFFFFu));
+                  } else if (DOST) {
                     if (SPLIT) {
                       __builtin_amdgcn_raw_buffer_store_b128(__builtin_bit_cast(u32x4, ev), R.vrs, voff + 16u * q + 64u * t, 0, WC_ST_AUX);
                     } else {
@@ -494,13 +540,15 @@
       WC_STAMP(4);
     }
     WC_STAMP_FLUSH;
+    if (ALN) wc_flush_odd<store_t>(a, R.vrs, park, fr.fvalid, nrow);
     wc_store_z(a, R, fr, rp_off, z);
   }
 }
 
 
-template <int MAXT, bool STORE, bool M2>
+template <int MAXT, bool STORE, bool M2, bool ALN = false>
 __global__ __launch_bounds__(256, 1) void wchain4_kernel(const WcArgs a) {
+  static_assert(!ALN || STORE, "ALN");
   extern __shared__ __attribute__((aligned(16))) char smem[];
   constexpr int NP = (MAXT - 1) / 2;
   constexpr int PPW = NP / 4, NOWN = 2 * PPW + 1;
@@ -541,6 +589,11 @@
   }
 
   const WcRes R = wc_resources<STORE, M2>(a);
+  char* const park = smem + (ALN ? a.park_lds : 0);
+  const unsigned xpark = a.lay.xframe * 2u;
+  if (ALN && wave == 0)
+    for (unsigned e = (unsigned)lane * 16u; e < WT_FRAMES * a.lay.xframe * 2u; e += 1024u)
+      *reinterpret_cast<u32x4*>(smem + a.park_lds + e) = u32x4{0u, 0u, 0u, 0u};
 
   for (int wt = blockIdx.x; wt < a.n_wtiles; wt += (int)gridDim.x) {
     const WcFrame fr = wc_frame(a, wt, c, wave == 0);
@@ -574,7 +627,7 @@
     }
     float z[8];
     wc_load_z(R, fr, q, z);
-    const unsigned fbase = STORE ? (fr.fvalid ? (unsigned)nrow * (unsigned)(a.Rs * a.Fs) * 2u : WC_OOB) : 0u;
+    const unsigned fbase = STORE ? (fr.fvalid ? (unsigned)nrow * a.lay.frame * 2u : WC_OOB) : 0u;
     const unsigned zs_off = fr.keeps ? ((unsigned)nrow * (unsigned)a.Rcap * LAT + 4u * q) * 4u : WC_OOB;
     const unsigned fr_off = (fr.keeps && q == 0) ? (unsigned)nrow * 4u : WC_OOB;
     const unsigned rp_off = ((unsigned)nrow * LAT + 4u * q) * 4u;
@@ -588,7 +641,7 @@
 
     auto energy = [&](const float (&zz)[8], int slot, auto dost) -> double {
       constexpr bool DOST = STORE && decltype(dost)::value;
-      const unsigned voff = DOST ? fbase + (unsigned)slot * (unsigned)a.Fs * 2u : 0u;
+      const unsigned voff = DOST ? fbase + (unsigned)slot * a.lay.row * 2u : 0u;
       u32x4 bh[NK_H], ch[NK_H];
       u32x4 mine;
       auto put2 = [&](int i, const f32x4 h) { mine[2 * i] = pk2(h[0], h[1]); mine[2 * i + 1] = pk2(h[2], h[3]); };
@@ -651,6 +704,8 @@
           if (i < 2 * PPW) {
             if ((i & 1) == 0) { pk_even0 = p0; pk_even1 = p1; }
             else __builtin_amdgcn_raw_buffer_store_b128(u32x4{pk_even0, pk_even1, p0, p1}, R.vrs, voff + 16u * q + 64u * (t >> 1), 0, WC_ST_AUX);
+          } else if (ALN) {
+            wc_park<__bf16>(park, xpark, slot, p0 & 0xFFFFu);
           } else {
             __builtin_amdgcn_raw_buffer_store_b64(u32x2{p0, p1}, R.vrs, voff + 8u * q + 32u * t, 0, WC_ST_AUX);
           }
@@ -739,6 +794,7 @@
         __builtin_amdgcn_raw_buffer_store_b128(__builtin_bit_cast(u32x4, f32x4{z[4], z[5], z[6], z[7]}), R.zs_rs, zo + 64u, 0, 0);
       }
     }
+    if (ALN && wave == 0) wc_flush_odd<__bf16>(a, R.vrs, park, fr.fvalid, nrow);
     wc_store_z(a, R, fr, rp_off, z);
   }
 }
@@ -752,6 +808,23 @@
   if (a.B1) return a.VsS ? go(std::true_type{}, std::true_type{}) : go(std::true_type{}, std::false_type{});
   return a.VsS ? go(std::false_type{}, std::true_type{}) : go(std::false_type{}, std::false_type{});
 }
+constexpr int WC_GT33 = 4;
+
+struct WcLdsPlan { int nwaves; bool lol; size_t b1_lds, park_lds, total; };
+WcLdsPlan wc_lds_plan(const vaenmf_plan* p, bool m2, size_t xframe_bytes) {
+  const bool split = p->cfg.precision == VAENMF_PREC_BF16X3;
+  WcLdsPlan l;
+  const size_t fixed = split ? WcLds<true>::fixed_bytes : WcLds<false>::fixed_bytes;
+  const int gt = p->NT3c == 33 ? WC_GT33 : 0;
+  const size_t w3hi = (size_t)(p->NT3c - gt) * NK_H * 1024;
+  l.lol = split && p->NT3c <= 5;
+  l.nwaves = (split || p->NT3c == 33) ? 4 : 8;
+  l.b1_lds = fixed + w3hi * (l.lol ? 2 : 1);
+  l.park_lds = l.b1_lds + ((m2 && l.nwaves == 8) ? (size_t)l.nwaves * NT_H * 512 : 0);
+  l.total = l.park_lds + (size_t)l.nwaves * WT_FRAMES * xframe_bytes;
+  return l;
+}
+
 template <int MAXT, bool EXACT, bool SPLIT, int NW1, bool LOL, int GT = 0>
 int wc_launch_s(const WcArgs& a, int nwt, int n_sms, size_t lds, hipStream_t st) {
   int grid = nwt;
@@ -759,16 +832,29 @@
   const int cap = vn_switches().grid_cap;
   if (cap > 0 && cap < grid) grid = cap;
   return wc_by_m2_store(a, [&](auto m2, auto store) -> int {
-    auto* fn = wchain_kernel<MAXT, EXACT, SPLIT, decltype(store)::value, NW1, LOL, true, decltype(m2)::value, GT>;
-    if (int e = vn_ensure_dyn_lds((const void*)fn, VN_LDS_LIMIT)) return e;
-    hipLaunchKernelGGL(fn, dim3(grid), dim3(NW1 * 64), lds, st, a);
-    return 0;
+    auto go = [&](auto* fn) -> int {
+      if (int e = vn_ensure_dyn_lds((const void*)fn, VN_LDS_LIMIT)) return e;
+      hipLaunchKernelGGL(fn, dim3(grid), dim3(NW1 * 64), lds, st, a);
+      return 0;
+    };
+    if constexpr (decltype(store)::value && EXACT && MAXT == 17) {
+      if (a.lay.aligned) return go(wchain_kernel<MAXT, EXACT, SPLIT, true, NW1, LOL, true, decltype(m2)::value, GT, true>);
+    }
+    return go(wchain_kernel<MAXT, EXACT, SPLIT, decltype(store)::value, NW1, LOL, true, decltype(m2)::value, GT>);
   });
 }
 template <int MAXT>
-int wc_launch4(const WcArgs& a, hipStream_t st) {
+int wc_launch4(WcArgs a, hipStream_t st) {
   const size_t lds4 = 2 * 4 * 64 * 16 + 20 * 64 * 4;
   return wc_by_m2_store(a, [&](auto m2, auto store) -> int {
+    if constexpr (decltype(store)::value) {
+      if (a.lay.aligned) {
+        a.park_lds = (int)lds4;
+        hipLaunchKernelGGL((wchain4_kernel<MAXT, true, decltype(m2)::value, true>), dim3(a.n_wtiles), dim3(256),
+                           lds4 + (size_t)WT_FRAMES * a.lay.xframe * 2, st, a);
+        return 0;
+      }
+    }
     hipLaunchKernelGGL((wchain4_kernel<MAXT, decltype(store)::value, decltype(m2)::value>), dim3(a.n_wtiles), dim3(256), lds4, st, a);
     return 0;
   });
@@ -793,6 +879,17 @@
   if (replay && nt * S * LAT * 4 >= lim) return 0;
   return 1;
 }
+static bool wc_runs_wchain4(const vaenmf_plan* p) {
+  return p->cfg.precision != VAENMF_PREC_BF16X3 && (p->NT3c == 17 || p->NT3c == 33) && p->n_wtiles <= p->n_sms && vn_switches().wchain4;
+}
+bool vn_wchain_park_fits(const vaenmf_plan* p, int Rs, bool m2) {
+  if (p->NT3c != 17 && p->NT3c != 33) return true;
+  if (wc_runs_wchain4(p)) return true;
+  if (p->NT3c == 33) return false;
+  const int esz = p->cfg.precision == VAENMF_PREC_BF16X3 ? 4 : 2;
+  const size_t xb = ((size_t)Rs * esz + 63) / 64 * 64;
+  return wc_lds_plan(p, m2, xb).total <= (size_t)VN_LDS_LIMIT;
+}
 bool vn_wchain_fits(const vaenmf_plan* p, const VnChainCall& cc) {
   return vaenmf_wchain_addressable(p->NT, cc.Rcap, cc.nsamples + cc.burnin, p->Fs, p->Kp, p->n_utt, cc.eps != nullptr) != 0;
 }
@@ -805,28 +902,28 @@
   a.NT3 = p->NT3c; a.Tm = split ? 0 : ((p->NT3c - 1) & ~1); a.F = p->cfg.F; a.Fs = p->Fs;
   a.X2 = cc.X2; a.W = cc.W; a.Ht = cc.Ht; a.g = cc.g; a.B1 = cc.B1; a.Vb = p->Vb_ext;
   a.Z = cc.Z; a.Zs = cc.Zs; a.acc_out = cc.acc_out;
-  a.VsS = cc.VsS; a.VsS_bytes = (unsigned)cc.VsS_bytes; a.src = cc.src; a.Rs = cc.Rs;
+  a.VsS = cc.VsS; a.VsS_bytes = (unsigned)cc.VsS_bytes; a.src = cc.src; a.Rs = cc.Rs; a.lay = cc.lay;
   a.wt_utt = p->d_wt_utt; a.wt_n0 = p->d_wt_n0; a.wt_cnt = p->d_wt_cnt; a.n_wtiles = p->n_wtiles;
   a.frame_off = p->d_frame_off; a.utt_seed = p->d_utt_seed; a.eps = cc.eps; a.u = cc.u;
   a.Kp = p->Kp; a.NT = p->NT; a.n_utts = p->n_utt; a.Rcap = cc.Rcap; a.nsamples = cc.nsamples; a.burnin = cc.burnin;
   a.rng_mode = cc.rng_mode; a.update_Z = cc.update_Z; a.call = cc.call; a.sd = cc.sd; a.sd_hi = cc.sd_hi; a.one_hidden = cc.one_hidden;
   a.n_hi_lds = p->NT3c;
-  const size_t fixed = split ? WcLds<true>::fixed_bytes : WcLds<false>::fixed_bytes;
-  constexpr int GT33 = 4;
-  const size_t w3hi = (size_t)(p->NT3c == 33 ? p->NT3c - GT33 : p->NT3c) * NK_H * 1024;
-  const bool lol = split && p->NT3c <= 5;
+  constexpr int GT33 = WC_GT33;
   constexpr int NW_BF16 = 8, NW_X3 = 4;
-  const int nwaves = (split || p->NT3c == 33) ? 4 : NW_BF16;
-  a.b1_lds = (int)(fixed + w3hi * (lol ? 2 : 1));
-  const size_t lds = (size_t)a.b1_lds + ((cc.B1 && nwaves == 8) ? (size_t)nwaves * NT_H * 512 : 0);
-  VN_REQUIRE(lds <= (size_t)VN_LDS_LIMIT, "wave chain: %zu bytes of LDS needed", lds);
-  if (!split && (p->NT3c == 17 || p->NT3c == 33) && p->n_wtiles <= p->n_sms && vn_switches().wchain4) {
+  if (wc_runs_wchain4(p)) {
     const int rc4 = p->NT3c == 17 ? wc_launch4<17>(a, st) : wc_launch4<33>(a, st);
     if (rc4) return rc4;
     VN_CHECK_HIP(hipGetLastError());
     p->last_chain_kernel = 2;
     return 0;
   }
+  const bool aln = cc.VsS && cc.lay.aligned;
+  const WcLdsPlan lp = wc_lds_plan(p, cc.B1 != nullptr, aln ? (size_t)cc.lay.xframe * (split ? 4 : 2) : 0);
+  a.b1_lds = (int)lp.b1_lds;
+  a.park_lds = (int)lp.park_lds;
+  const size_t lds = lp.total;
+  VN_REQUIRE(lds <= (size_t)VN_LDS_LIMIT, "wave chain: %zu bytes of LDS needed", lds);
+  VN_REQUIRE(!aln || p->NT3c == 17, "wave chain: no line-aligned store layout at %d bin tiles", p->NT3c);
   int rc;
   if (p->NT3c == 33)     rc = wc_launch_s<33, true, false, 4, false, GT33>(a, p->n_wtiles, p->n_sms, lds, st);
   else if (p->NT3c == 17) rc = split ? wc_launch_s<17, true, true, NW_X3, false>(a, p->n_wtiles, p->n_sms, lds, st) : wc_launch_s<17, true, false, NW_BF16, false>(a, p->n_wtiles, p->n_sms, lds, st);
diff --git a/guided-vae-nmf_amd/csrc/common.h b/guided-vae-nmf_amd/csrc/common.h
--- a/guided-vae-nmf_amd/csrc/common.h
+++ b/guided-vae-nmf_amd/csrc/common.h
@@ -52,6 +52,28 @@
   Graph* insert(const Key& key, hipGraphExec_t exec, int chain_kernel, int w_fused);
   void release();
 };
+
+struct VnStoreLayout {
+  uint32_t row, frame;
+  uint32_t xslot, xframe;
+  uint64_t xbase;
+  int32_t aligned;
+};
+inline VnStoreLayout vn_store_layout_of(int F, int Fs, int esz, int Rs, size_t frames, bool aligned) {
+  VnStoreLayout l;
+  if (aligned && (F == 257 || F == 513)) {
+    l.row = (uint32_t)(F - 1); l.frame = (uint32_t)Rs * l.row;
+    l.xslot = 1; l.xframe = (uint32_t)(((size_t)Rs * esz + 63) / 64 * 64 / esz);
+    l.xbase = (uint64_t)frames * l.frame; l.aligned = 1;
+  } else {
+    l.row = l.xslot = (uint32_t)Fs; l.frame = l.xframe = (uint32_t)Rs * (uint32_t)Fs;
+    l.xbase = (uint64_t)(F - 1); l.aligned = 0;
+  }
+  return l;
+}
+inline size_t vn_store_bytes(const VnStoreLayout& l, size_t frames, int esz) {
+  return (l.aligned ? frames * ((size_t)l.frame + l.xframe) : frames * (size_t)l.frame) * esz;
+}
 
 struct vaenmf_plan {
   vaenmf_config cfg;
@@ -101,6 +123,7 @@
   int32_t* src;
   size_t VsS_cap, src_cap;
   int store_R, store_Rs;
+  VnStoreLayout store_lay;
   int n_sms;
   bool prof_on;
   std::vector<hipEvent_t> prof_ev;
@@ -119,6 +142,7 @@
   float *Z, *Zs, *acc_out;
   const float *eps, *u;
   void* VsS; size_t VsS_bytes; int32_t* src; int Rs;
+  VnStoreLayout lay;
   int Rcap, nsamples, burnin, rng_mode, update_Z;
   uint32_t call;
   float sd;
@@ -134,6 +158,7 @@
   int wfused_grid;
   int grid_cap;
   bool keep_zs;
+  bool store_aligned;
 };
 
 VnSwitches vn_switches();
@@ -141,6 +166,8 @@
 extern long long g_vn_dev_allocs;
 bool vn_wchain_supported(const vaenmf_plan* p);
 bool vn_wchain_fits(const vaenmf_plan* p, const VnChainCall& cc);
+bool vn_wchain_park_fits(const vaenmf_plan* p, int Rs, bool m2);
+VnStoreLayout vn_store_layout(const vaenmf_plan* p, int Rs, bool m2);
 int vn_launch_wchain(vaenmf_plan* p, const VnChainCall& cc, hipStream_t st);
 int vn_launch_tchain(vaenmf_plan* p, const VnChainCall& cc, hipStream_t st);
 int vn_launch_widechain(vaenmf_plan* p, const VnChainCall& cc, hipStream_t st);
diff --git a/guided-vae-nmf_amd/csrc/driver.hip b/guided-vae-nmf_amd/csrc/driver.hip
--- a/guided-vae-nmf_amd/csrc/driver.hip
+++ b/guided-vae-nmf_amd/csrc/driver.hip
@@ -1,5 +1,19 @@
 #include "common.h"
 #include <cstring>
+
+VnStoreLayout vn_store_layout(const vaenmf_plan* p, int Rs, bool m2) {
+  const int esz = p->cfg.precision == VAENMF_PREC_BF16X3 ? 4 : 2;
+  bool aligned = vn_switches().store_aligned;
+  if (aligned && !p->wide && vn_wchain_supported(p) && !vn_wchain_park_fits(p, Rs, m2)) aligned = false;
+  return vn_store_layout_of(p->cfg.F, p->Fs, esz, Rs, (size_t)(p->NT > 0 ? p->NT : p->cfg.max_frames) + 1, aligned);
+}
+extern "C" int vaenmf_store_layout(int32_t F, int32_t Fs, int32_t elt_bytes, int32_t Rs, int64_t frames, int32_t aligned, int64_t* out7) {
+  VN_REQUIRE(out7 != nullptr && F >= 1 && Fs >= F && (elt_bytes == 2 || elt_bytes == 4) && Rs >= 1 && frames >= 1, "vaenmf_store_layout: bad arguments");
+  const VnStoreLayout l = vn_store_layout_of(F, Fs, elt_bytes, Rs, (size_t)frames, aligned != 0);
+  out7[0] = l.row; out7[1] = l.frame; out7[2] = l.xslot; out7[3] = l.xframe; out7[4] = (int64_t)l.xbase; out7[5] = l.aligned;
+  out7[6] = (int64_t)vn_store_bytes(l, (size_t)frames, elt_bytes);
+  return 0;
+}
 
 extern "C" int vaenmf_mh_chain(vaenmf_plan* p, const float* X2, const float* W, const float* Ht, const float* g,
                                float* Z, int32_t update_Z, const float* B1, float* Zs, int32_t Rcap, int32_t nsamples,
@@ -18,13 +32,13 @@
   p->store_R = p->store_Rs = 0;
   if (p->store_on) {
     const int Rs = nsamples + 1;
-    const size_t esz = split ? sizeof(float) : sizeof(__bf16);
-    const size_t need_v = (size_t)(p->NT + 1) * Rs * p->Fs * esz, need_s = (size_t)p->NT * Rs;
+    const VnStoreLayout lay = vn_store_layout(p, Rs, B1 != nullptr);
+    const size_t need_v = vn_store_bytes(lay, (size_t)p->NT + 1, split ? 4 : 2), need_s = (size_t)p->NT * Rs;
     VN_REQUIRE(need_v < 0xE0000000ull, "sample store: %d frames x %d slots x %d bins exceeds the 32-bit byte offsets of "
                "the chain kernel; bind a smaller batch or switch the store off", p->NT, Rs, p->Fs);
     VN_REQUIRE(need_v <= p->VsS_cap && need_s <= p->src_cap, "sample store too small for %d frames x %d samples: call "
                "vaenmf_sample_store(plan, max_samples) after vaenmf_bind_batch (no allocation happens in vaenmf_mh_chain)", p->NT, nsamples);
-    cc.VsS = p->VsS; cc.VsS_bytes = need_v; cc.src = p->src; cc.Rs = Rs;
+    cc.VsS = p->VsS; cc.VsS_bytes = need_v; cc.src = p->src; cc.Rs = Rs; cc.lay = lay;
   }
   const bool use_wchain = !p->wide && vn_wchain_supported(p) && vn_wchain_fits(p, cc);
   VN_REQUIRE(p->wide || use_wchain || Zs != nullptr, "vaenmf_mh_chain: Zs may be NULL only where the wave-private chain kernels run (vaenmf_wchain_addressable)");
@@ -32,7 +46,7 @@
     ProfScope ps(p, VN_K_CHAIN, st);
     if (int e = p->wide ? vn_launch_widechain(p, cc, st) : use_wchain ? vn_launch_wchain(p, cc, st) : vn_launch_tchain(p, cc, st)) return e;
   }
-  if (p->store_on) { p->store_R = nsamples; p->store_Rs = nsamples + 1; }
+  if (p->store_on) { p->store_R = nsamples; p->store_Rs = nsamples + 1; p->store_lay = cc.lay; }
   return 0;
 }
 
@@ -44,7 +58,9 @@
   if (!p->store_on) return 0;
   const size_t esz = p->cfg.precision == VAENMF_PREC_BF16X3 ? sizeof(float) : sizeof(__bf16);
   const size_t frames = (size_t)(p->NT > 0 ? p->NT : p->cfg.max_frames) + 1, Rs = (size_t)max_samples + 1;
-  size_t need_v = frames * Rs * p->Fs * esz, need_s = frames * Rs;
+  const size_t need_pad = vn_store_bytes(vn_store_layout_of(p->cfg.F, p->Fs, (int)esz, (int)Rs, frames, false), frames, (int)esz);
+  const size_t need_aln = vn_store_bytes(vn_store_layout_of(p->cfg.F, p->Fs, (int)esz, (int)Rs, frames, true), frames, (int)esz);
+  size_t need_v = need_pad > need_aln ? need_pad : need_aln, need_s = frames * Rs;
   if (need_v >= 0xE0000000ull) need_v = 0xE0000000ull - 16;
   if (need_v > p->VsS_cap) {
     if (p->VsS) VN_CHECK_HIP(hipFree(p->VsS));
@@ -66,11 +82,14 @@
 
 namespace {
 template <typename ST>
-__global__ void store_gather_kernel(const ST* __restrict__ VsS, const int32_t* __restrict__ src, int NT, int R, int Rs, int Fs,
+__global__ void store_gather_kernel(const ST* __restrict__ VsS, const int32_t* __restrict__ src, int NT, int R, VnStoreLayout lay, int F, int Fs,
                                     float* __restrict__ out) {
   const int n = blockIdx.x / R, r = blockIdx.x - n * R;
-  const ST* row = VsS + ((size_t)n * Rs + src[(size_t)r * NT + n]) * Fs;
-  for (int f = threadIdx.x; f < Fs; f += blockDim.x) out[((size_t)n * R + r) * Fs + f] = (float)row[f];
+  const int sl = src[(size_t)r * NT + n];
+  const ST* row = VsS + (size_t)n * lay.frame + (size_t)sl * lay.row;
+  const ST* xp = VsS + lay.xbase + (size_t)n * lay.xframe + (size_t)sl * lay.xslot;
+  for (int f = threadIdx.x; f < Fs; f += blockDim.x)
+    out[((size_t)n * R + r) * Fs + f] = f < (int)lay.row ? (float)row[f] : (f == F - 1 ? (float)*xp : 0.f);
 }
 }
 
@@ -79,10 +98,10 @@
   VN_REQUIRE(Vs_out != nullptr, "null output");
   if (p->cfg.precision == VAENMF_PREC_BF16X3)
     hipLaunchKernelGGL(store_gather_kernel<float>, dim3((unsigned)(p->NT * p->store_R)), dim3(64), 0, (hipStream_t)stream,
-                       reinterpret_cast<const float*>(p->VsS), p->src, p->NT, p->store_R, p->store_Rs, p->Fs, Vs_out);
+                       reinterpret_cast<const float*>(p->VsS), p->src, p->NT, p->store_R, p->store_lay, p->cfg.F, p->Fs, Vs_out);
   else
     hipLaunchKernelGGL(store_gather_kernel<__bf16>, dim3((unsigned)(p->NT * p->store_R)), dim3(64), 0, (hipStream_t)stream,
-                       reinterpret_cast<const __bf16*>(p->VsS), p->src, p->NT, p->store_R, p->store_Rs, p->Fs, Vs_out);
+                       reinterpret_cast<const __bf16*>(p->VsS), p->src, p->NT, p->store_R, p->store_lay, p->cfg.F, p->Fs, Vs_out);
   VN_CHECK_HIP(hipGetLastError());
   return 0;
 }
@@ -119,7 +138,7 @@
       (uint64_t)p->cfg.precision, (uint64_t)p->cfg.K, (uint64_t)p->cfg.F,
       (uint64_t)sw.wchain4, (uint64_t)sw.team_chain, (uint64_t)sw.wfused, (uint64_t)sw.wgroup, (uint64_t)(uint32_t)sw.wfused_grid,
       (uint64_t)(uint32_t)sw.grid_cap,
-      (uint64_t)sw.keep_zs};
+      (uint64_t)sw.keep_zs, (uint64_t)sw.store_aligned};
 }
 }
 
@@ -181,7 +200,7 @@
 static int em_graph_launch(vaenmf_plan* p, VnEmGraphs::Graph& gph, const EmCall& c, bool stored, hipStream_t st) {
   VN_CHECK_HIP(hipGraphLaunch(gph.exec, st));
   gph.used = ++p->graphs.tick;
-  if (stored) { p->store_R = c.nsWF; p->store_Rs = c.nsWF + 1; }
+  if (stored) { p->store_R = c.nsWF; p->store_Rs = c.nsWF + 1; p->store_lay = vn_store_layout(p, c.nsWF + 1, c.B1 != nullptr); }
   p->last_chain_kernel = gph.chain_kernel;
   p->last_w_fused = gph.w_fused;
   p->graphs.last = 1;
@@ -208,8 +227,8 @@
   if (int e = check_bound(p)) return e;
   VN_REQUIRE(nsE <= Rcap && nsWF <= Rcap, "Rcap=%d too small for nsE=%d / nsWF=%d", Rcap, nsE, nsWF);
   const EmCall c = {X2, W, Ht, g, Z, B1, Zs, Rcap, niter, nsE, biE, nsWF, biWF, var_rw, X, S_hat, N_hat, cost};
-  const size_t esz = p->cfg.precision == VAENMF_PREC_BF16X3 ? sizeof(float) : sizeof(__bf16);
-  auto fits = [&](int ns) { return (size_t)(p->NT + 1) * (ns + 1) * p->Fs * esz < 0xE0000000ull; };
+  const int esz = p->cfg.precision == VAENMF_PREC_BF16X3 ? 4 : 2;
+  auto fits = [&](int ns) { return vn_store_bytes(vn_store_layout(p, ns + 1, B1 != nullptr), (size_t)p->NT + 1, esz) < 0xE0000000ull; };
   const bool want = p->store_on, stored = want && fits(nsE) && fits(nsWF);
   VN_REQUIRE(!p->wide || want, "vaenmf_em_run on a wide decoder plan streams the sample store: switch it on with vaenmf_sample_store first");
   VN_REQUIRE(!p->wide || stored, "vaenmf_em_run on a wide decoder plan: the sample store of %d frames passes the 32-bit offsets of the "
diff --git a/guided-vae-nmf_amd/csrc/engine.hip b/guided-vae-nmf_amd/csrc/engine.hip
--- a/guided-vae-nmf_amd/csrc/engine.hip
+++ b/guided-vae-nmf_amd/csrc/engine.hip
@@ -307,6 +307,7 @@
   const float* Vb;
   float *Z, *Zs, *acc_out;
   void* VsS;
+  VnStoreLayout lay;
   int32_t* src;
   int Rs;
   const int32_t *tile_utt, *tile_n0, *tile_cnt, *frame_off;
@@ -417,7 +418,7 @@
   if (STORE) {
 #pragma unroll
     for (int fg = 0; fg < 2; ++fg)
-      voff[fg] = ((uint32_t)(fvalid[fg] ? nrow[fg] : a.NT) * (uint32_t)(a.Rs * a.Fs) + 4u * q) * (uint32_t)sizeof(store_t);
+      voff[fg] = ((uint32_t)(fvalid[fg] ? nrow[fg] : a.NT) * a.lay.frame + 4u * q) * (uint32_t)sizeof(store_t);
   }
   const int sid = threadIdx.x - d.team * NW * 64, sfr = sid >> 3, squad = sid & 7;
   const bool srng = sid < TEAM_COLS * 8;
@@ -450,7 +451,7 @@
   const int S = a.nsamples + a.burnin;
   auto energy = [&](const float (&zz)[2][8], double (&E)[2], int next_step, int slot, auto dost) {
     constexpr bool DOST = STORE && decltype(dost)::value;
-    char* const vbase = reinterpret_cast<char*>(a.VsS) + (DOST ? (size_t)slot * a.Fs * sizeof(store_t) : 0);
+    char* const vbase = reinterpret_cast<char*>(a.VsS) + (DOST ? (size_t)slot * a.lay.row * sizeof(store_t) : 0);
     bf16x8 zhi[2], zlo[2];
     split8<SPLIT>(zz[0], zhi[0], zlo[0]);
     split8<SPLIT>(zz[1], zhi[1], zlo[1]);
@@ -494,6 +495,9 @@
         const float vx = gn[fg] * vs + vbn[fg];
         const float term = fast_log(vx) + x2n[fg] * fast_rcp(vx);
         e[fg] += (w == 0 && q == 0) ? (double)term : 0.0;
+        if (DOST && w == 2 && q == 0 && a.lay.aligned) {
+          reinterpret_cast<store_t*>(a.VsS)[a.lay.xbase + (size_t)(fvalid[fg] ? nrow[fg] : a.NT) * a.lay.xframe + (size_t)slot * a.lay.xslot] = (store_t)vs;
+        } else
         if (DOST && w == 2 && q == 0) {
           store_t* dst = reinterpret_cast<store_t*>(vbase + (size_t)dw.Fm * sizeof(store_t) + voff[fg]);
           if (SPLIT) {
@@ -1264,7 +1268,7 @@
   ChainArgs a = {};
   a.dw = make_decw(p);
   a.X2 = cc.X2; a.W = cc.W; a.Ht = cc.Ht; a.g = cc.g; a.B1 = cc.B1; a.Z = cc.Z; a.Zs = cc.Zs; a.acc_out = cc.acc_out; a.Vb = p->Vb_ext;
-  a.VsS = cc.VsS; a.src = cc.src; a.Rs = cc.Rs;
+  a.VsS = cc.VsS; a.src = cc.src; a.Rs = cc.Rs; a.lay = cc.lay;
   a.tile_utt = p->d_tile_utt; a.tile_n0 = p->d_tile_n0; a.tile_cnt = p->d_tile_cnt; a.frame_off = p->d_frame_off;
   a.utt_seed = p->d_utt_seed; a.eps = cc.eps; a.u = cc.u;
   a.Fs = p->Fs; a.Kp = p->Kp; a.NT = p->NT; a.Rcap = cc.Rcap; a.nsamples = cc.nsamples; a.burnin = cc.burnin;
diff --git a/guided-vae-nmf_amd/csrc/plan.hip b/guided-vae-nmf_amd/csrc/plan.hip
--- a/guided-vae-nmf_amd/csrc/plan.hip
+++ b/guided-vae-nmf_amd/csrc/plan.hip
@@ -33,6 +33,7 @@
   s.wfused_grid = atoi(env("VAENMF_WFUSED_GRID"));
   s.grid_cap = atoi(env("VAENMF_GRID_CAP"));
   s.keep_zs = env("VAENMF_KEEP_ZS")[0] == '1';
+  s.store_aligned = env("VAENMF_STORE_ALIGNED")[0] != '0';
   return s;
 }
 
@@ -133,7 +134,7 @@
   const size_t nk1 = p->Lp / 32, nt3 = p->wide ? p->Fs / 16 : p->NT3;
   p->have_weights = false;
   p->Vb_ext = nullptr;
-  p->store_on = false; p->VsS = nullptr; p->src = nullptr; p->VsS_cap = p->src_cap = 0; p->store_R = p->store_Rs = 0;
+  p->store_on = false; p->VsS = nullptr; p->src = nullptr; p->VsS_cap = p->src_cap = 0; p->store_R = p->store_Rs = 0; p->store_lay = {};
   p->n_utt = p->NT = p->n_tiles = 0;
   p->prof_on = false;
   p->prof_used = 0;
@@ -215,6 +216,7 @@
     case VAENMF_Q_W_FUSED: return p->last_w_fused;
     case VAENMF_Q_CHAIN_KERNEL: return p->last_chain_kernel;
     case VAENMF_Q_LP: return p->Lp;
+    case VAENMF_Q_STORE_ALIGNED: return p->store_lay.aligned;
     default: return -1;
   }
 }
diff --git a/guided-vae-nmf_amd/csrc/stream.hip b/guided-vae-nmf_amd/csrc/stream.hip
--- a/guided-vae-nmf_amd/csrc/stream.hip
+++ b/guided-vae-nmf_amd/csrc/stream.hip
@@ -10,6 +10,8 @@
 
 struct StreamArgs {
   const void* VsS;
+  VnStoreLayout lay;
+  unsigned store_bytes;
   const int32_t* src;
   const float *X2, *W, *normW, *Vb, *X;
   float *Ht, *g, *A1, *P, *S_hat, *N_hat, *WFs, *WFn;
@@ -59,6 +61,16 @@
     nw = 1.f;
     in_lds = false;
   }
+  __device__ __forceinline__ VnStoreLayout lay_here() const {
+#if defined(__HIP_DEVICE_COMPILE__)
+    typedef const __attribute__((address_space(4))) char* kptr;
+    kptr kp = (kptr)__builtin_amdgcn_kernarg_segment_ptr();
+    asm volatile("" : "+s"(kp));
+    return *(const __attribute__((address_space(4))) VnStoreLayout*)(kp + offsetof(StreamArgs, lay));
+#else
+    return a.lay;
+#endif
+  }
   __device__ __forceinline__ bool ok(int c, int t) const { return TAIL ? t < nb[c] : cv[c]; }
   __device__ __forceinline__ void pad_bins(f32x4 (&v)[NCH], float pad) const {
     if constexpr (TAIL) {
@@ -244,30 +256,35 @@
     return *reinterpret_cast<const int32_t*>(reinterpret_cast<const char*>(scol) + (unsigned)(r0 + (fc.lane < nr_ ? fc.lane : 0)) * (unsigned)fc.a.NT * 4u);
   }
   template <typename FC>
-  __device__ __forceinline__ void load_rows(const FC& fc, const ST* base, int sl, int r0, int R) {
+  __device__ __forceinline__ void load_rows(const FC& fc, int n, int sl, int r0, int R) {
+    const VnStoreLayout lay = fc.lay_here();
+    const ST* base = reinterpret_cast<const ST*>(fc.a.VsS) + (size_t)n * lay.frame;
     nr = RT > 0 ? RT : (R - r0 < RB ? R - r0 : RB);
 #pragma unroll
     for (int r = 0; r < RB; ++r)
       if (r == 0 || on(r)) {
-        const ST* row = base + (size_t)__builtin_amdgcn_readlane(sl, r) * fc.a.Fs;
+        const ST* row = base + (size_t)__builtin_amdgcn_readlane(sl, r) * lay.row;
 #pragma unroll
         for (int c = 0; c < NCH; ++c) raw[r][c] = __builtin_nontemporal_load(reinterpret_cast<const raw_t*>(row + fc.fo[c]));
       }
     if (fc.has_x) {
-      if constexpr (sizeof(ST) == 2) xbits = reinterpret_cast<const unsigned short*>(base)[(size_t)sl * fc.a.Fs + fc.a.F - 1];
-      else xbits = reinterpret_cast<const unsigned*>(base)[(size_t)sl * fc.a.Fs + fc.a.F - 1];
+      const char* xrow = reinterpret_cast<const char*>(reinterpret_cast<const ST*>(fc.a.VsS) + lay.xbase + (size_t)n * lay.xframe);
+      const unsigned xo = (unsigned)sl * (lay.xslot * (unsigned)sizeof(ST));
+      if constexpr (sizeof(ST) == 2) xbits = *reinterpret_cast<const unsigned short*>(xrow + xo);
+      else xbits = *reinterpret_cast<const unsigned*>(xrow + xo);
     } else xbits = 0u;
   }
   template <typename FC>
-  __device__ __forceinline__ void load(const FC& fc, const ST* base, const int32_t* scol, int r0, int R) {
-    load_rows(fc, base, load_slots(fc, scol, r0, R), r0, R);
+  __device__ __forceinline__ void load(const FC& fc, int n, const int32_t* scol, int r0, int R) {
+    load_rows(fc, n, load_slots(fc, scol, r0, R), r0, R);
   }
   template <typename FC>
-  __device__ __forceinline__ void load_rows_buf(const FC& fc, __amdgpu_buffer_rsrc_t rs, unsigned frame_off, int sl, int R, int r0 = 0) {
+  __device__ __forceinline__ void load_rows_buf(const FC& fc, __amdgpu_buffer_rsrc_t rs, int n, int sl, int R, int r0 = 0) {
     nr = RT > 0 ? RT : (R - r0 < RB ? R - r0 : RB);
-    const unsigned rowb = (unsigned)fc.a.Fs * (unsigned)sizeof(ST);
+    const unsigned frame_off = (unsigned)n * fc.a.lay.frame * (unsigned)sizeof(ST);
+    const unsigned rowb = fc.a.lay.row * (unsigned)sizeof(ST);
     if (fc.has_x) {
-      const unsigned o = frame_off + (unsigned)sl * rowb + (unsigned)(fc.a.F - 1) * (unsigned)sizeof(ST);
+      const unsigned o = ((unsigned)fc.a.lay.xbase + (unsigned)n * fc.a.lay.xframe + (unsigned)sl * fc.a.lay.xslot) * (unsigned)sizeof(ST);
       if constexpr (sizeof(ST) == 2) xbits = (unsigned)__builtin_amdgcn_raw_buffer_load_b16(rs, o, 0, 0);
       else xbits = (unsigned)__builtin_amdgcn_raw_buffer_load_b32(rs, o, 0, 0);
     } else xbits = 0u;
@@ -336,11 +353,10 @@
   constexpr int HB = Half::RB;
   if (a.R <= 2 * HB) {
     Half h0, h1;
-    auto base_of = [&](int n) { return reinterpret_cast<const ST*>(a.VsS) + (size_t)n * a.Rs * a.Fs; };
     const int R0 = a.R < HB ? a.R : HB;
     if (n_beg < n_end) {
-      h0.load(fc, base_of(n_beg), a.src + n_beg, 0, R0);
-      if (a.R > HB) h1.load(fc, base_of(n_beg), a.src + n_beg, HB, a.R); else h1.nr = 0, h1.xbits = 0u;
+      h0.load(fc, n_beg, a.src + n_beg, 0, R0);
+      if (a.R > HB) h1.load(fc, n_beg, a.src + n_beg, HB, a.R); else h1.nr = 0, h1.xbits = 0u;
     }
     for (int n = n_beg; n < n_end; ++n) {
       const int utt = a.frame_utt[n];
@@ -378,10 +394,10 @@
         a2x += wave_sum(q * q);
       };
       consume(h0);
-      if (n + 1 < n_end) h0.load(fc, base_of(n + 1), a.src + n + 1, 0, R0);
+      if (n + 1 < n_end) h0.load(fc, n + 1, a.src + n + 1, 0, R0);
       if (a.R > HB) {
         consume(h1);
-        if (n + 1 < n_end) h1.load(fc, base_of(n + 1), a.src + n + 1, HB, a.R);
+        if (n + 1 < n_end) h1.load(fc, n + 1, a.src + n + 1, HB, a.R);
       }
 #pragma unroll
       for (int c = 0; c < NCH; ++c)
@@ -393,10 +409,9 @@
     return;
   }
   for (int n = n_beg; n < n_end; ++n) {
-    const ST* base = reinterpret_cast<const ST*>(a.VsS) + (size_t)n * a.Rs * a.Fs;
     const int32_t* srow = a.src + n;
     RBt rb;
-    rb.load(fc, base, srow, 0, a.R);
+    rb.load(fc, n, srow, 0, a.R);
     const int utt = a.frame_utt[n];
     fc.set_utt(utt);
     const float gn = a.g[n];
@@ -414,7 +429,7 @@
 #pragma unroll
     for (int c = 0; c < NCH; ++c) a1[c] = a2[c] = f32x4{0.f, 0.f, 0.f, 0.f};
     for (int r0 = 0; r0 < a.R; r0 += RBt::RB) {
-      if (r0 > 0) rb.load(fc, base, srow, r0, a.R);
+      if (r0 > 0) rb.load(fc, n, srow, r0, a.R);
 #pragma unroll
       for (int r = 0; r < RBt::RB; ++r)
         if (r < rb.nr) {
@@ -451,7 +466,6 @@
   wave_frames(a.NT, n_beg, n_end);
   const bool one = a.R <= RBt::RB;
   for (int n = n_beg; n < n_end; ++n) {
-    const ST* base = reinterpret_cast<const ST*>(a.VsS) + (size_t)n * a.Rs * a.Fs;
     const int32_t* srow = a.src + n;
     RBt rb;
     const int utt = a.frame_utt[n];
@@ -472,7 +486,7 @@
       }
     }
     fc.set_utt(utt, a.gains_only ? nullptr : a.normW);
-    rb.load_rows(fc, base, sl, 0, a.R);
+    rb.load_rows(fc, n, sl, 0, a.R);
     const f32x2 gn2 = {gn, gn};
     if (!a.gains_only) {
 #pragma unroll
@@ -483,7 +497,7 @@
 #pragma unroll
       for (int c = 0; c < NCH; ++c) a1[c] = a2[c] = f32x4{0.f, 0.f, 0.f, 0.f};
       for (int r0 = 0; r0 < a.R; r0 += RBt::RB) {
-        if (r0 > 0) rb.load(fc, base, srow, r0, a.R);
+        if (r0 > 0) rb.load(fc, n, srow, r0, a.R);
         auto row1 = [&](int r) {
           f32x4 v[NCH];
           rb.get(r, v);
@@ -529,7 +543,7 @@
 #pragma unroll
       for (int c = 0; c < NCH; ++c) ng[c] = dg[c] = f32x4{0.f, 0.f, 0.f, 0.f};
       for (int r0 = 0; r0 < a.R; r0 += RBt::RB) {
-        if (!one) rb.load(fc, base, srow, r0, a.R);
+        if (!one) rb.load(fc, n, srow, r0, a.R);
         auto row2 = [&](int r) {
           f32x4 v[NCH];
           rb.get(r, v);
@@ -566,7 +580,7 @@
 #pragma unroll
     for (int c = 0; c < NCH; ++c) cl[c] = cx[c] = f32x4{0.f, 0.f, 0.f, 0.f};
     for (int r0 = 0; r0 < a.R; r0 += RBt::RB) {
-      if (!one) rb.load(fc, base, srow, r0, a.R);
+      if (!one) rb.load(fc, n, srow, r0, a.R);
 #pragma unroll
       for (int r = 0; r < RBt::RB; r += 2) {
         if (rb.on(r + 1)) {
@@ -620,10 +634,9 @@
   wave_frames(a.NT, n_beg, n_end);
   const float invR = 1.0f / (float)a.R;
   for (int n = n_beg; n < n_end; ++n) {
-    const ST* base = reinterpret_cast<const ST*>(a.VsS) + (size_t)n * a.Rs * a.Fs;
     const int32_t* srow = a.src + n;
     RBt rb;
-    rb.load(fc, base, srow, 0, a.R);
+    rb.load(fc, n, srow, 0, a.R);
     const int utt = a.frame_utt[n];
     fc.set_utt(utt);
     const float gn = a.g[n];
@@ -646,7 +659,7 @@
 #pragma unroll
     for (int c = 0; c < NCH; ++c) ws[c] = wn[c] = f32x4{0.f, 0.f, 0.f, 0.f};
     for (int r0 = 0; r0 < a.R; r0 += RBt::RB) {
-      if (r0 > 0) rb.load(fc, base, srow, r0, a.R);
+      if (r0 > 0) rb.load(fc, n, srow, r0, a.R);
 #pragma unroll
       for (int r = 0; r < RBt::RB; ++r)
         if (r < rb.nr) {
@@ -714,13 +727,13 @@
   int n_beg, n_end;
   wave_frames(a.NT, n_beg, n_end);
   if (n_beg >= n_end) return;
-  __amdgpu_buffer_rsrc_t vrs = __builtin_amdgcn_make_buffer_rsrc(const_cast<void*>(a.VsS), 0, (int)((unsigned)a.NT * (unsigned)(a.Rs * a.Fs) * (unsigned)sizeof(ST)), 0x00020000);
+  __amdgpu_buffer_rsrc_t vrs = __builtin_amdgcn_make_buffer_rsrc(const_cast<void*>(a.VsS), 0, (int)a.store_bytes, 0x00020000);
   auto request = [&](int n, RBt& rb, FS& s, int sl) {
     s.utt = a.frame_utt[n];
     s.g = a.g[n];
     s.hl = a.Ht[(size_t)n * KP + (fc.lane < KP ? fc.lane : 0)];
     fc.load_x2(n, s.x2, s.x2x);
-    rb.load_rows_buf(fc, vrs, (unsigned)n * (unsigned)(a.Rs * a.Fs) * (unsigned)sizeof(ST), sl, a.R);
+    rb.load_rows_buf(fc, vrs, n, sl, a.R);
   };
   auto compute = [&](int n, RBt& rb, const FS& s) {
     fc.set_utt(s.utt);
@@ -785,17 +798,18 @@
   const StreamArgs& a;
   const FC& fc;
   __amdgpu_buffer_rsrc_t vrs;
-  unsigned rowb, frameb, voff, xvoff;
+  unsigned rowb, frameb, voff;
+  unsigned xslotb, xframeb, xvoff;
   const char* pk_base;
   unsigned pk_stride;
   bf16x4 raw[2][RT];
   unsigned xb[2];
   __device__ RotCtx(const StreamArgs& a_, const FC& fc_) : a(a_), fc(fc_) {
-    vrs = __builtin_amdgcn_make_buffer_rsrc(const_cast<void*>(a.VsS), 0, (int)((unsigned)a.NT * (unsigned)(a.Rs * a.Fs) * 2u), 0x00020000);
-    rowb = (unsigned)a.Fs * 2u;
-    frameb = (unsigned)a.Rs * rowb;
+    vrs = __builtin_amdgcn_make_buffer_rsrc(const_cast<void*>(a.VsS), 0, (int)a.store_bytes, 0x00020000);
+    rowb = a.lay.row * 2u;
+    frameb = a.lay.frame * 2u;
     voff = (unsigned)(fc.cv[0] ? fc.f0[0] : 0) * 2u;
-    xvoff = (unsigned)(a.F - 1) * 2u;
+    xslotb = a.lay.xslot * 2u; xframeb = a.lay.xframe * 2u; xvoff = (unsigned)a.lay.xbase * 2u;
     xb[0] = xb[1] = 0u;
     const int l = fc.lane;
     if (l == KP) { pk_base = reinterpret_cast<const char*>(a.frame_utt); pk_stride = 4u; }
@@ -823,7 +837,7 @@
   }
   template <int S>
   __device__ __forceinline__ void req_x(int n, int sl, bool on) {
-    if (fc.has_x) xb[S] = (unsigned)__builtin_amdgcn_raw_buffer_load_b16(vrs, on ? (unsigned)sl * rowb + xvoff : 0xF0000000u, (unsigned)n * frameb, 0);
+    if (fc.has_x) xb[S] = (unsigned)__builtin_amdgcn_raw_buffer_load_b16(vrs, on ? (unsigned)sl * xslotb + xvoff : 0xF0000000u, (unsigned)n * xframeb, 0);
   }
   template <int S>
   __device__ __forceinline__ f32x4 row(int r) const {
@@ -988,7 +1002,6 @@
       a1xs[i] = pxs[i] = hls[i] = 0.f;
       const int n = n_beg + i;
       if (n < n_end) {
-        const ST* base = reinterpret_cast<const ST*>(a.VsS) + (size_t)n * a.Rs * a.Fs;
         const int sl = RBt::load_slots(fc, a.src + n, 0, RT);
         const float gn = a.g[n];
         f32x4 x2[1];
@@ -1004,7 +1017,7 @@
         hls[i] = fc.lane < KP ? a.Ht[(size_t)n * KP + (fc.lane < KP ? fc.lane : 0)] : 0.f;
         fc.set_utt(utt);
         RBt rb;
-        rb.load_rows(fc, base, sl, 0, RT);
+        rb.load_rows(fc, n, sl, 0, RT);
         f32x4 vb[1], a1, a2;
         float vbx;
         fc.noise_var(utt, h, vb, vbx);
@@ -1074,6 +1087,8 @@
   a.VsS = p->VsS; a.src = p->src; a.frame_utt = p->d_frame_utt; a.Vb = p->Vb_ext;
   a.store_f32 = p->cfg.precision == VAENMF_PREC_BF16X3;
   a.n_sms = p->n_sms;
+  a.lay = p->store_lay;
+  a.store_bytes = (unsigned)((a.lay.aligned ? a.lay.xbase + (uint64_t)p->NT * a.lay.xframe : (uint64_t)p->NT * a.lay.frame) * (a.store_f32 ? 4 : 2));
   a.NT = p->NT; a.R = p->store_R; a.Rs = p->store_Rs; a.F = p->cfg.F; a.Fm = p->Fm; a.Fs = p->Fs; a.K = p->cfg.K;
   return a;
 }
diff --git a/guided-vae-nmf_amd/csrc/wide.hip b/guided-vae-nmf_amd/csrc/wide.hip
--- a/guided-vae-nmf_amd/csrc/wide.hip
+++ b/guided-vae-nmf_amd/csrc/wide.hip
@@ -14,6 +14,7 @@
   const float *X2, *W, *Ht, *g, *B1, *Vb;
   float *Z, *Zs, *acc_out;
   void* VsS; int32_t* src; int Rs;
+  VnStoreLayout lay;
   const int32_t *wt_utt, *wt_n0, *wt_cnt, *frame_off;
   const uint64_t* utt_seed;
   const float *eps, *u;
@@ -173,7 +174,7 @@
       __syncthreads();
     }
     const char* last = a.NT2 > 0 ? act2 : act1;
-    char* const vrow = DOST ? reinterpret_cast<char*>(a.VsS) + ((size_t)nrow * a.Rs + slot) * a.Fs * sizeof(store_t) : nullptr;
+    char* const vrow = DOST ? reinterpret_cast<char*>(a.VsS) + ((size_t)nrow * a.lay.frame + (size_t)slot * a.lay.row) * sizeof(store_t) : nullptr;
     double e = 0.0;
 #pragma unroll
     for (int i = 0; i < WD_MAXT; ++i) {
@@ -195,7 +196,10 @@
           pl += fast_log2(vx);
           px += x2[i][k] * fast_rcp(vx);
         }
-        if (DOST && fvalid) {
+        if (DOST && fvalid && 16 * t + 4 * q >= (int)a.lay.row) {
+          if (16 * t + 4 * q == a.F - 1)
+            reinterpret_cast<store_t*>(a.VsS)[a.lay.xbase + (size_t)nrow * a.lay.xframe + (size_t)slot * a.lay.xslot] = (store_t)ev[0];
+        } else if (DOST && fvalid) {
           store_t* dst = reinterpret_cast<store_t*>(vrow) + 16 * t + 4 * q;
           if (SPLIT) *reinterpret_cast<f32x4*>(dst) = ev;
           else *reinterpret_cast<bf16x4*>(dst) = bf16x4{(__bf16)ev[0], (__bf16)ev[1], (__bf16)ev[2], (__bf16)ev[3]};
@@ -301,7 +305,7 @@
   a.F = p->cfg.F; a.Fs = p->Fs; a.Kp = p->Kp; a.NT = p->NT;
   a.X2 = cc.X2; a.W = cc.W; a.Ht = cc.Ht; a.g = cc.g; a.B1 = cc.B1; a.Vb = p->Vb_ext;
   a.Z = cc.Z; a.Zs = cc.Zs; a.acc_out = cc.acc_out;
-  a.VsS = cc.VsS; a.src = cc.src; a.Rs = cc.Rs;
+  a.VsS = cc.VsS; a.src = cc.src; a.Rs = cc.Rs; a.lay = cc.lay;
   a.wt_utt = p->d_wt_utt; a.wt_n0 = p->d_wt_n0; a.wt_cnt = p->d_wt_cnt; a.frame_off = p->d_frame_off;
   a.utt_seed = p->d_utt_seed; a.eps = cc.eps; a.u = cc.u;
   a.Rcap = cc.Rcap; a.nsamples = cc.nsamples; a.burnin = cc.burnin; a.rng_mode = cc.rng_mode; a.update_Z = cc.update_Z;
diff --git a/guided-vae-nmf_amd/vaenmf/_lib.py b/guided-vae-nmf_amd/vaenmf/_lib.py
--- a/guided-vae-nmf_amd/vaenmf/_lib.py
+++ b/guided-vae-nmf_amd/vaenmf/_lib.py
@@ -6,7 +6,7 @@
 
 PREC_BF16X3, PREC_BF16 = 0, 1
 RNG_REPLAY, RNG_DEVICE = 0, 1
-Q_FS, Q_KP, Q_TILES, Q_NT, Q_NUTT, Q_MSTEP_PATH, Q_WTILES, Q_EM_GRAPH, Q_DEV_ALLOCS, Q_W_FUSED, Q_CHAIN_KERNEL, Q_LP = 0, 1, 2, 3, 4, 5, 6, 7, 8, 9, 10, 11
+Q_FS, Q_KP, Q_TILES, Q_NT, Q_NUTT, Q_MSTEP_PATH, Q_WTILES, Q_EM_GRAPH, Q_DEV_ALLOCS, Q_W_FUSED, Q_CHAIN_KERNEL, Q_LP, Q_STORE_ALIGNED = 0, 1, 2, 3, 4, 5, 6, 7, 8, 9, 10, 11, 12
 ACT_NONE, ACT_TANH, ACT_RELU, ACT_SIGMOID, ACT_STEP = 0, 1, 2, 3, 4
 LABEL_IBM, LABEL_VAD = 0, 1
 
@@ -73,6 +73,7 @@
     "vaenmf_profile_enable": (_I, [_P, _I]),
     "vaenmf_profile_read": (_I, [_P, _P, _P]),
     "vaenmf_wchain_addressable": (_I, [_I64, _I, _I, _I, _I, _I, _I]),
+    "vaenmf_store_layout": (_I, [_I, _I, _I, _I, _I64, _I, _P]),
     "vaenmf_hbm_read_probe": (_I, [_P, _I64, _I, _P, C.POINTER(_D), _P]),
 }
 
diff --git a/include/vaenmf.h b/include/vaenmf.h
--- a/include/vaenmf.h
+++ b/include/vaenmf.h
@@ -22,6 +22,7 @@
        VAENMF_Q_W_FUSED = 9,
        VAENMF_Q_CHAIN_KERNEL = 10,
        VAENMF_Q_LP = 11,
+       VAENMF_Q_STORE_ALIGNED = 12,
        VAENMF_Q_DEV_ALLOCS = 8 };
 
 enum { VAENMF_ACT_NONE = 0, VAENMF_ACT_TANH = 1, VAENMF_ACT_RELU = 2, VAENMF_ACT_SIGMOID = 3,
@@ -94,6 +95,7 @@
 
 int vaenmf_sample_store(vaenmf_plan* plan, int32_t max_samples);
 int vaenmf_sample_store_gather(vaenmf_plan* plan, float* Vs_out, void* stream);
+int vaenmf_store_layout(int32_t F, int32_t Fs, int32_t elt_bytes, int32_t Rs, int64_t frames, int32_t aligned, int64_t* out7);
 int vaenmf_m_step_stored(vaenmf_plan* plan, const float* X2, float* W, float* Ht, float* g,
                          double* cost_frames, void* stream);
 int vaenmf_wiener_stored(vaenmf_plan* plan, const float* W, const float* Ht, const float* g,
```

Result: faster. 472,500 frames/s (median of 6 runs) (+3.3%).
